# vmware/splinterdb

Hardware: AMD Instinct MI355X
Metric: routing_filter build Mkeys/s + probe Mkeys/s, device-resident, 24B keys (higher is better)
Workload: dtype u32; 1 GPU; C2: 64M x 24B keys per GPU = 8 filters x 8,000,000, build + full probe; filters_total=8, filters_per_gpu=8, keys_per_filter=8000000, key_len=24, fingerprint_size=26, log_index_size=8, seed=42, parallelism=key-range shards, 1 rank(s), no data-path collective

## Files before the change

### include/rf_amd_diag.h

```cpp
#ifndef RF_AMD_DIAG_H
#define RF_AMD_DIAG_H

#include "rf_amd.h"

#ifdef __cplusplus
extern "C" {
#endif

int rf_amd_debug_read_lines(rf_amd_batch *b, uint8_t *h_lines, uint64_t bytes, uint64_t *num_lines);
int rf_amd_debug_rebuild_lines(rf_amd_batch *b);

int rf_amd_debug_probe_floor(rf_amd_batch *b, const void *d_in, uint32_t key_len, const uint64_t *h_counts,
                             uint64_t *d_out, void *stream);

int rf_amd_debug_phase_buffer(void *d_buf, uint32_t kernel);

int rf_amd_diag_lookup_stats(uint64_t *out, int reset);

int rf_amd_diag_lookup_paths(uint64_t *out, int reset);

int rf_amd_lookup_server_stats(rf_amd_engine *e, uint64_t *out);

int rf_amd_diag_lookup_ring(rf_amd_engine *e);

int rf_amd_diag_lookup_server_kill(rf_amd_engine *e, int err, uint32_t gap_us);

uint64_t rf_amd_diag_k4_bitmap_builds(void);

uint64_t rf_amd_diag_part16_builds(void);

int rf_amd_diag_fanout_max_blocks(uint32_t blocks);

uint32_t rf_amd_diag_range_tile(void);
uint32_t rf_amd_diag_range_lds_ranges(void);

const char *rf_amd_build_id(void);

#ifdef __cplusplus
}
#endif
#endif
```

### splinterdb_amd/csrc/rf_batch_plan.h

```cpp
#pragma once
#include <math.h>
#include <string.h>

#include <algorithm>
#include <string>
#include <vector>

#include "../../include/rf_amd.h"
#include "rf_plan.h"

namespace rf {

inline uint64_t max_fingerprints(const rf_amd_config& cfg) {
  const uint64_t addrs_per_extent = (uint64_t)cfg.page_size * cfg.pages_per_extent / 8;
  return 2ull * addrs_per_extent * (1ull << cfg.log_index_size) - 1;
}

inline uint32_t vsize_of(uint32_t value) { return value == 0 ? 0 : 32 - __builtin_clz(value); }

inline uint32_t log_buckets_of(uint64_t nfp, uint32_t lis) {
  const uint32_t lnb = 63 - __builtin_clzll(nfp);
  return lnb < lis ? lis : lnb;
}
inline uint32_t num_indices_of(uint64_t nfp, uint32_t lis) { return 1u << (log_buckets_of(nfp, lis) - lis); }

inline uint32_t line_log_group(uint32_t lis, uint32_t rvs, double lam, double sigma) {
  if (rvs > 32) return 0;
  for (int g = (int)(lis < 6 ? lis : 6); g >= 0; g--) {
    const double G = (double)(1u << g), mean = lam * G;
    const double cap = rvs ? std::min(128.0 - G, 384.0 / rvs) : 128.0 - G;
    if (mean + sigma * sqrt(mean) + 2.0 <= cap) return (uint32_t)g + 1;
  }
  return 0;
}

inline int lines_in_assembly(uint32_t lis, uint32_t lg_line, uint32_t page_size) {
  const uint32_t IS = 1u << lis, L = IS >> (lg_line - 1);
  const uint32_t min_block = 2 + (IS - 1) / 8 + 4 + 3;
  const uint32_t maxb = page_size / min_block + 1;
  if (maxb > ASM_MAXB || L + 1 > ASM_GT) return 0;
  return (uint64_t)maxb * (L + 1) <= ASM_GT ? 1 : 2;
}

struct PlanKnobs {
  bool wide64 = false;
  bool old_decode = false;
  bool old_resplit_off = false;
  uint32_t layout_seg = LAYOUT_SEG_MAX;
  double line_sigma = 3.5;
};

struct OldFilter {
  bool present = false;
  const FilterPlan* plan = nullptr;
  uint32_t fingerprint_size = 0, log_index_size = 0;
  bool has_entries = false;
  bool wide = false;
  bool built = false;
  bool same_device = false;
};

struct BatchInput {
  const rf_amd_config* cfg = nullptr;
  uint32_t num_filters = 0;
  const uint32_t* num_new = nullptr;
  const uint16_t* value = nullptr;
  const uint32_t* num_runs = nullptr;
  const uint32_t* run_len = nullptr;
  const uint16_t* run_value = nullptr;
  const OldFilter* olds = nullptr;
};

enum { PRE_TILE, PRE_OTILE, PRE_CB, PRE_PG, PRE_IDX, PRE_OIDX, NUM_PRE };

struct BatchPlan {
  uint32_t F = 0;
  std::vector<FilterPlan> plans;
  std::vector<uint32_t> pre;
  uint32_t* pre_of(int k) { return pre.data() + (size_t)k * (F + 1); }
  const uint32_t* pre_of(int k) const { return pre.data() + (size_t)k * (F + 1); }
  bool wide = false;
  bool flag32 = false;
  bool chained = false;
  uint64_t old_total = 0;
  uint32_t num_tiles = 0, num_old_tiles = 0, num_old_idx = 0;
  uint64_t E = 0, keys_total = 0;
  uint32_t CB = 0, I = 0, PS = 0, PF = 0;
  uint64_t NL = 0;
  bool plines_needed = false;
  uint32_t line_lmax = 0;
  uint32_t lay_seg = 0, lay_grid = 0;
  bool lay_whole = true;
  std::vector<uint32_t> lay_wg;
  bool k4_bitmap = false;
  std::vector<uint32_t> tile_filter, tile_start, tile_value, tile_end;
  std::vector<uint4> pplans;
};

inline int plan_fail(std::string* err, int rc, const std::string& msg) {
  if (err) *err = msg;
  return rc;
}

inline int check_config(const rf_amd_config* cfg, std::string* err) {
  if (!cfg) return plan_fail(err, RF_AMD_EINVAL, "null config");
  if (cfg->page_size != MAX_PAGE || cfg->pages_per_extent != 32)
    return plan_fail(err, RF_AMD_EINVAL, "engine supports 4 KiB pages in 32-page extents");
  if (cfg->fingerprint_size == 0 || cfg->fingerprint_size > 32 || cfg->log_index_size > MAX_LIS ||
      cfg->log_index_size < 3)
    return plan_fail(err, RF_AMD_EINVAL, "unsupported fingerprint_size / log_index_size");
  return 0;
}

inline void probe_geometry(FilterPlan& p, const rf_amd_config& cfg, double sigma, uint64_t* line_total,
                           uint32_t* line_lmax) {
  const uint32_t lis = cfg.log_index_size;
  p.rem = cfg.fingerprint_size - p.lnb;
  p.rvs = p.rem + p.vs;
  p.lg_line = line_log_group(lis, p.rvs, (double)p.num_fp / (double)(1ull << p.lnb), sigma);
  p.line_base = (uint32_t)*line_total;
  if (p.lg_line) {
    *line_total += (uint64_t)p.num_indices << (lis - (p.lg_line - 1));
    *line_lmax = std::max(*line_lmax, (1u << lis) >> (p.lg_line - 1));
  }
}

inline uint32_t pplan_word(const FilterPlan& p) { return p.vs | (p.rem << 8) | (p.rvs << 16) | (p.lg_line << 24); }
inline uint4 pack_pplan(const FilterPlan& p) { return make_uint4(pplan_word(p), p.line_base, p.idx_base, 0); }

inline int check_runs(const BatchInput& in, std::vector<uint32_t>* run_first, std::vector<uint32_t>* run_total,
                      std::string* err) {
  const rf_amd_config& cfg = *in.cfg;
  run_first->assign(in.num_filters + 1, 0u);
  run_total->assign(in.num_filters, 0u);
  for (uint32_t f = 0; f < in.num_filters; f++) {
    if (in.num_runs[f] == 0) return plan_fail(err, RF_AMD_EINVAL, "a filter without runs");
    const uint32_t r0 = (*run_first)[f], r1 = r0 + in.num_runs[f];
    (*run_first)[f + 1] = r1;
    uint64_t tot = 0;
    for (uint32_t r = r0; r < r1; r++) {
      if (in.run_len[r] == 0) return plan_fail(err, RF_AMD_EINVAL, "zero-length run");
      if (r > r0 && in.run_value[r] <= in.run_value[r - 1])
        return plan_fail(err, RF_AMD_EINVAL, "run values of a filter must be strictly increasing");
      tot += in.run_len[r];
    }
    if (tot > max_fingerprints(cfg))
      return plan_fail(err, RF_AMD_EINVAL, "num_fingerprints over routing_filter_max_fingerprints (reference: UB)");
    if (cfg.fingerprint_size + vsize_of(in.run_value[r1 - 1]) > 32)
      return plan_fail(err, RF_AMD_EINVAL, "fp_size + value_size > 32");
    const OldFilter* o = in.olds && in.olds[f].present ? &in.olds[f] : nullptr;
    if (o && o->plan && vsize_of(in.run_value[r0]) < o->plan->vs)
      return plan_fail(err, RF_AMD_EINVAL, "first run's value narrower than the old filter's value_size");
    (*run_total)[f] = (uint32_t)tot;
  }
  return 0;
}

inline int filter_geometry(const rf_amd_config& cfg, uint32_t num_new, uint32_t v, const FilterPlan* op,
                           FilterPlan* out, std::string* err) {
  FilterPlan& p = *out;
  const uint32_t lis = cfg.log_index_size, fps = cfg.fingerprint_size, IS = 1u << lis;
  p.num_new = num_new;
  p.old_region = op ? op->num_fp : 0;
  const uint64_t nfp = (uint64_t)p.num_new + p.old_region;
  if (nfp > max_fingerprints(cfg))
    return plan_fail(err, RF_AMD_EINVAL, "num_fingerprints over routing_filter_max_fingerprints (reference: UB)");
  p.num_fp = (uint32_t)nfp;
  if (p.num_fp == 0) return plan_fail(err, RF_AMD_EINVAL, "routing_filter_add with zero fingerprints (reference: UB)");
  const uint32_t lnb = log_buckets_of(nfp, lis);
  p.vs = vsize_of(v);
  if (lnb > fps || (1u << (lnb - lis)) > MAX_INDICES || fps + p.vs > 32 || (op && p.vs < op->vs))
    return plan_fail(err, RF_AMD_EINVAL, "filter geometry out of range (over routing_filter_max_fingerprints, "
                                         "fp_size + value_size > 32, or value narrower than old filter)");
  p.lnb = lnb;
  p.value = v;
  p.num_indices = 1u << (lnb - lis);
// ... 94 lines not shown
      first = end;
    }
  }
}

inline int plan_batch(const BatchInput& in0, const PlanKnobs& knobs, BatchPlan* out, std::string* err) {
  BatchInput in = in0;
  if (in.num_runs && in.run_len && in.run_value) {
    bool single = true;
    for (uint32_t f = 0; f < in.num_filters && single; f++) single = in.num_runs[f] == 1;
    if (single) {
      for (uint32_t f = 0; f < in.num_filters; f++)
        if (in.run_len[f] == 0) return plan_fail(err, RF_AMD_EINVAL, "zero-length run");
      in.num_new = in.run_len;
      in.value = in.run_value;
      in.num_runs = nullptr;
    }
  }
  if (int rc = check_config(in.cfg, err)) return rc;
  if (in.num_filters == 0 || !(in.num_runs ? (in.run_len && in.run_value) : in.num_new != nullptr))
    return plan_fail(err, RF_AMD_EINVAL, "empty batch");
  const rf_amd_config& cfg = *in.cfg;
  const uint32_t F = in.num_filters;
  std::vector<uint32_t> run_first, run_total;
  if (in.num_runs) {
    if (int rc = check_runs(in, &run_first, &run_total, err)) return rc;
    in.num_new = run_total.data();
  }
  BatchPlan& b = *out;
  b = BatchPlan();
  b.F = F;
  b.chained = in.num_runs != nullptr;
  b.plans.resize(F);
  b.pre.assign((size_t)NUM_PRE * (F + 1), 0u);
  const uint32_t lis = cfg.log_index_size;
  for (uint32_t f = 0; f < F; f++) {
    FilterPlan& p = b.plans[f];
    memset(&p, 0, sizeof(p));
    const FilterPlan* op = nullptr;
    if (in.olds && in.olds[f].present) {
      const OldFilter& o = in.olds[f];
      if (!o.plan || !o.built || !o.same_device) return plan_fail(err, RF_AMD_EINVAL, "bad old filter reference");
      op = o.plan;
      b.wide = true;
    }
    const uint32_t v = b.chained ? in.run_value[run_first[f + 1] - 1] : in.value ? in.value[f] : 0;
    if (int rc = filter_geometry(cfg, in.num_new[f], v, op, &p, err)) return rc;
    p.e_first = b.E;
    p.key_first = b.keys_total;
    p.cb_base = b.CB;
    p.idx_base = b.I;
    p.page_base = b.PS;
    p.pf_base = b.PF;
    probe_geometry(p, cfg, knobs.line_sigma, &b.NL, &b.line_lmax);
    const int la = p.lg_line ? lines_in_assembly(lis, p.lg_line, cfg.page_size) : 0;
    p.lines_asm = la != 0;
    p.lines_flag = la == 2;
    if (p.lg_line && la != 1) b.plines_needed = true;
    uint32_t ntiles = (p.num_new + TILE_KEYS - 1) / TILE_KEYS;
    if (b.chained) {
      const uint64_t prev_fp = (uint64_t)p.num_fp - in.run_len[run_first[f + 1] - 1];
      p.npo = prev_fp ? p.num_indices / num_indices_of(prev_fp, lis) : 1u;
      ntiles = 0;
      for (uint32_t r = run_first[f]; r < run_first[f + 1]; r++) ntiles += (in.run_len[r] + TILE_KEYS - 1) / TILE_KEYS;
    }
    auto pre = [&](int k, uint32_t count) { b.pre_of(k)[f + 1] = b.pre_of(k)[f] + count; };
    pre(PRE_TILE, ntiles);
    pre(PRE_OTILE, (p.old_region + TILE_KEYS - 1) / TILE_KEYS);
    pre(PRE_CB, 1u << p.cbits);
    pre(PRE_PG, p.page_cap);
    pre(PRE_IDX, p.num_indices);
    b.E += p.num_fp;
    b.keys_total += p.num_new;
    b.CB += 1u << p.cbits;
    b.I += p.num_indices;
    b.PS += p.page_cap;
    b.PF += p.page_cap + 1;
  }
  if (b.wide) {
    b.flag32 = !knobs.wide64;
    for (const auto& p : b.plans) b.flag32 = b.flag32 && cfg.fingerprint_size + p.vs <= 31;
  }
  if (!b.wide || b.flag32) {
    b.E = 0;
    for (auto& p : b.plans) {
      p.e_first = b.E;
      b.E += (uint64_t)CB_REGION << p.cbits;
    }
  }
  if (b.wide) plan_old_filters(b, in, knobs);
  b.lay_seg = knobs.layout_seg;
  if (cfg.page_size > MAX_PAGE || F >= (1u << 26)) b.lay_seg = 0;
  assign_layout(b);
  b.k4_bitmap = k4_bitmap_batch(b, cfg);
  b.num_tiles = b.pre_of(PRE_TILE)[F];
  b.num_old_tiles = b.pre_of(PRE_OTILE)[F];
  if (b.NL > 0xffffffffull) return plan_fail(err, RF_AMD_EINVAL, "batch too large (probe lines > 2^32)");
  b.pplans.resize(F);
  for (uint32_t f = 0; f < F; f++) b.pplans[f] = pack_pplan(b.plans[f]);
  if (b.chained) cut_tiles(b, in, run_first);
  return 0;
}

inline int plan_import(const rf_amd_config* cfgp, uint32_t F, const rf_amd_filter_info* infos,
                       const PlanKnobs& knobs, BatchPlan* out, std::string* err) {
  if (int rc = check_config(cfgp, err)) return rc;
  if (F == 0 || !infos) return plan_fail(err, RF_AMD_EINVAL, "bad image");
  const rf_amd_config& cfg = *cfgp;
  const uint32_t lis = cfg.log_index_size;
  BatchPlan& b = *out;
  b = BatchPlan();
  b.F = F;
  b.plans.resize(F);
  b.pplans.resize(F);
  uint64_t pages_total = 0, idx_total = 0;
  for (uint32_t f = 0; f < F; f++) {
    const rf_amd_filter_info& in = infos[f];
    FilterPlan& p = b.plans[f];
    memset(&p, 0, sizeof(p));
    const uint32_t lnb = in.num_fingerprints ? log_buckets_of(in.num_fingerprints, lis) : lis;
    if (in.num_fingerprints == 0 || lnb > cfg.fingerprint_size || (1u << (lnb - lis)) > MAX_INDICES ||
        in.num_indices != (1u << (lnb - lis)) || in.value_size > 32 - cfg.fingerprint_size || in.error ||
        in.num_pages == 0)
      return plan_fail(err, RF_AMD_EINVAL, "image geometry out of range (filter " + std::to_string(f) + ")");
    p.num_fp = in.num_fingerprints;
    p.lnb = lnb;
    p.vs = in.value_size;
    p.num_indices = in.num_indices;
    p.page_cap = in.num_pages;
    p.page_base = (uint32_t)pages_total;
    p.idx_base = (uint32_t)idx_total;
    probe_geometry(p, cfg, knobs.line_sigma, &b.NL, &b.line_lmax);
    if (p.lg_line) b.plines_needed = true;
    b.pplans[f] = pack_pplan(p);
    pages_total += in.num_pages;
    idx_total += p.num_indices;
  }
  if (b.NL >= (1ull << 32) || pages_total >= (1ull << 32)) return plan_fail(err, RF_AMD_EINVAL, "import too large");
  b.PS = (uint32_t)pages_total;
  b.I = (uint32_t)idx_total;
  return 0;
}

}
```

### splinterdb_amd/csrc/rf_engine.cpp

```cpp
#include <hip/hip_runtime.h>
#include <hip/hip_ext.h>
#include <math.h>
#include <algorithm>
#include <stdio.h>
#include <stdlib.h>
#include <string.h>
#include <time.h>
#include <x86intrin.h>

#include <map>
#include <atomic>
#include <memory>
#include <mutex>
#include <string>
#include <vector>

#include "../../include/rf_amd.h"
#include "../../include/rf_amd_diag.h"
#include "rf_plan.h"
#include "rf_batch_plan.h"
#include "rf_set_plan.h"
#include "rf_launch.h"

using namespace rf;
// ... 223 lines not shown
}

#define RF_BATCH_DEVBUFS(X)                                                                        \
  X(d_runs) X(d_wave_tab)      \
  X(d_plans) X(d_outs) X(d_ent) X(d_part) X(d_sorted) X(d_cb_count) X(d_cb_start) X(d_cb_cursor)   \
  X(d_cb_filter) X(d_overflow) X(d_idx_cnt) X(d_idx_start) X(d_slots) X(d_page_first)              \
  X(d_pg_filter) X(d_pages) X(d_tile_filter) X(d_tile_start) X(d_old_tile_filter)                  \
  X(d_old_tile_start) X(d_old_cnt) X(d_old_pos) X(d_first_old) X(d_has_old) X(d_pplans) X(d_lines) \
  X(d_idx_filter) X(d_spill) X(d_old_idx_filter) X(d_old32) X(d_old_tot) X(d_ob_lo) X(d_ob_n)      \
  X(d_pg_noline) X(d_pre) X(d_cb_out) X(d_lay_wg) X(d_lay_hand)                                    \
  X(d_tile_value) X(d_tile_end)

struct rf_amd_batch : BatchPlan {
  rf_amd_engine* eng = nullptr;
  rf_amd_config cfg{};
#define X(name) DevBuf name;
  RF_BATCH_DEVBUFS(X)
#undef X
  std::vector<uint64_t> runs_host;
  uint32_t lay_seq = 0;
  bool counters_clean = false;
  bool built = false;
  bool has_entries = false;
  std::vector<uint32_t> err_host;
  std::atomic<bool> err_ready{false};
  std::mutex err_mu;
  hipEvent_t built_ev = nullptr;
  std::vector<hipEvent_t> events;
  uint32_t ev_sets = 0, ev_set = 0;
  uint32_t ev_mask = EV_MASK_ALL;
  ~rf_amd_batch() {
    if (built_ev) (void)hipEventDestroy(built_ev);
    for (auto ev : events) (void)hipEventDestroy(ev);
  }
  std::vector<DevBuf*> bufs() {
    return {
#define X(name) &name,
        RF_BATCH_DEVBUFS(X)
#undef X
    };
  }
};

static PlanKnobs plan_knobs_env() {
  PlanKnobs k;
  k.wide64 = getenv("RF_AMD_WIDE64") != nullptr;
  k.old_decode = getenv("RF_AMD_OLD_DECODE") != nullptr;
  k.old_resplit_off = getenv("RF_AMD_OLD_RESPLIT_OFF") != nullptr;
  if (const char* e = getenv("RF_AMD_LAYOUT_SEG"); e && *e) {
    const unsigned long v = strtoul(e, nullptr, 10);
    k.layout_seg = (v < LAYOUT_SEG_MIN || (v & (v - 1))) ? 0 : v > LAYOUT_SEG_MAX ? LAYOUT_SEG_MAX : (uint32_t)v;
  }
  if (const char* e = getenv("RF_AMD_LINE_SIGMA"); e && atof(e) > 0.0) k.line_sigma = atof(e);
  return k;
}

extern "C" const char* rf_amd_last_error(void) { return g_err.c_str(); }

static std::mutex g_live_mu;
static std::vector<rf_amd_engine*>* g_live = nullptr;
static bool engine_quiesce(rf_amd_engine* e, int budget_ms);
static void engine_destroy_now(rf_amd_engine* e, bool device_sync);
static void engines_at_exit() {
  std::vector<rf_amd_engine*> v;
  {
    std::lock_guard<std::mutex> g(g_live_mu);
    if (g_live) v.swap(*g_live);
  }
  for (rf_amd_engine* e : v) {
    if (engine_quiesce(e, 2000)) engine_destroy_now(e, false);
  }
}

extern "C" int rf_amd_engine_create(int device, rf_amd_engine** out) {
  int n = 0;
  if (hipGetDeviceCount(&n) != hipSuccess || n == 0)
    return fail(RF_AMD_ENODEV, "no HIP device: the routing-filter engine has no CPU fallback");
  if (device < 0 || device >= n) return fail(RF_AMD_EINVAL, "bad device ordinal");
  HIPCHK(hipSetDevice(device));
  auto* e = new rf_amd_engine();
  static std::atomic<uint64_t> next_uid{1};
  e->uid = next_uid.fetch_add(1);
  e->device = device;
  {
    const char* lim = getenv("RF_AMD_POOL_MIB");
    size_t free_b = 0, total_b = 0;
    (void)hipMemGetInfo(&free_b, &total_b);
    const size_t dflt = free_b / 4;
    e->pool.limit = lim ? (size_t)atoll(lim) << 20 : dflt;
  }
  if (hipStreamCreateWithFlags(&e->stream, hipStreamDefault) != hipSuccess) {
    delete e;
    return fail(RF_AMD_EINVAL, "hipStreamCreate failed");
  }
  {
    static std::once_flag at_exit_once;
    std::call_once(at_exit_once, [] { (void)atexit(engines_at_exit); });
    std::lock_guard<std::mutex> g(g_live_mu);
    if (!g_live) g_live = new std::vector<rf_amd_engine*>();
    g_live->push_back(e);
  }
  *out = e;
  return 0;
}

static void srv_stop(rf_amd_engine* e);
extern "C" void rf_amd_engine_destroy(rf_amd_engine* e) {
  if (!e) return;
  {
    std::lock_guard<std::mutex> g(g_live_mu);
// ... 439 lines not shown
  return rf_amd_engine_pool_trim(e, bytes);
}

extern "C" uint32_t rf_amd_batch_num_filters(const rf_amd_batch* b) { return b ? b->F : 0; }

static LaunchArgs make_args(rf_amd_batch* b, hipStream_t st) {
  LaunchArgs a;
  memset(&a, 0, sizeof(a));
  a.stream = st;
  a.wide = b->wide;
  a.plans = b->d_plans.as<FilterPlan>();
  a.pplans = b->d_pplans.as<uint4>();
  a.pplans_mut = b->d_pplans.as<uint4>();
  a.num_filters = b->F;
  a.tile_filter = b->d_tile_filter.as<uint32_t>();
  a.tile_start = b->d_tile_start.as<uint32_t>();
  a.num_tiles = b->num_tiles;
  a.tile_value = b->chained ? b->d_tile_value.as<uint32_t>() : nullptr;
  a.tile_end = b->chained ? b->d_tile_end.as<uint32_t>() : nullptr;
  a.old_tile_filter = b->d_old_tile_filter.as<uint32_t>();
  a.old_tile_start = b->d_old_tile_start.as<uint32_t>();
  a.num_old_tiles = b->num_old_tiles;
  a.old_idx_filter = b->d_old_idx_filter.as<uint32_t>();
  a.num_old_idx = b->num_old_idx;
  a.old_cnt = b->d_old_cnt.as<uint32_t>();
  a.old_pos = b->d_old_pos.as<uint32_t>();
  a.flag32 = b->flag32 ? 1u : 0u;
  a.old32 = b->d_old32.as<uint32_t>();
  a.old_tot = b->d_old_tot.as<uint32_t>();
  a.ob_lo = b->d_ob_lo.as<uint32_t>();
  a.ob_n = b->d_ob_n.as<uint32_t>();
  a.fp_size = b->cfg.fingerprint_size;
  a.seed = b->cfg.seed;
  a.lis = b->cfg.log_index_size;
  a.page_size = b->cfg.page_size;
  a.ent = b->d_ent.p;
  a.part = b->d_part.p;
  a.sorted32 = b->wide ? b->d_sorted.as<uint32_t>() : b->d_part.as<uint32_t>();
  a.cb_count = b->d_cb_count.as<uint32_t>();
  a.cb_start = b->d_cb_start.as<uint32_t>();
  a.cb_cursor = b->d_cb_cursor.as<uint32_t>();
  a.cb_filter = b->d_cb_filter.as<uint32_t>();
  a.num_cb = b->CB;
  a.overflow = b->d_overflow.as<uint32_t>();
  a.spill = b->d_spill.p ? b->d_spill.as<uint32_t>() : nullptr;
  a.cb_outs = b->d_cb_out.p ? b->d_cb_out.as<uint32_t>() : nullptr;
  a.idx_cnt = b->d_idx_cnt.as<uint32_t>();
  a.idx_start = b->d_idx_start.as<uint32_t>();
  a.first_old = b->d_first_old.as<uint32_t>();
  a.has_old = b->d_has_old.as<uint32_t>();
  a.slots = b->d_slots.as<uint64_t>();
  a.lines = b->d_lines.as<uint4>();
  a.line_lmax = b->line_lmax;
  a.plines_needed = b->plines_needed ? 1u : 0u;
  a.pg_noline = b->d_pg_noline.as<uint32_t>();
  a.idx_filter = b->d_idx_filter.as<uint32_t>();
  a.num_idx = b->I;
  a.page_first = b->d_page_first.as<uint32_t>();
  a.pg_filter = b->d_pg_filter.as<uint32_t>();
  a.num_page_slots = b->PS;
  a.pages = b->d_pages.as<uint8_t>();
  a.outs = b->d_outs.p ? b->d_outs.as<FilterOut>() : nullptr;
  a.lay_wg = b->d_lay_wg.as<uint32_t>();
  a.lay_grid = b->d_lay_wg.p && b->d_lay_hand.p ? b->lay_grid : 0;
  a.lay_hand = b->d_lay_hand.as<uint64_t>();
  a.lay_seq = b->lay_seq;
  a.lay_seg = b->lay_seg;
  a.lay_whole = b->lay_whole ? 1u : 0u;
  a.k4_bitmap = b->k4_bitmap ? 1u : 0u;
  a.events = b->events.empty() ? nullptr : reinterpret_cast<void**>(b->events.data() + (size_t)b->ev_set * NUM_EVENTS);
  a.ev_mask = b->ev_mask;
  return a;
}

static int do_probe(rf_amd_batch* b, int kind, const void* in0, const uint64_t* offs, uint32_t key_len,
                    const uint32_t* fid, uint64_t n, uint64_t* found, void* stream,
                    const uint64_t* d_runs = nullptr);

static int note_built(rf_amd_batch* b, hipStream_t st) {
  if (!b->built_ev) HIPCHK(hipEventCreateWithFlags(&b->built_ev, hipEventDisableTiming));
  HIPCHK(hipEventRecord(b->built_ev, st));
  return 0;
}
static int wait_built(rf_amd_batch* b) {
  if (b->built_ev) HIPCHK(hipEventSynchronize(b->built_ev));
  return 0;
}

static int do_build(rf_amd_batch* b, int kind, const void* in0, const uint64_t* offs, uint32_t key_len,
                    void* stream) {
  if (!b) return fail(RF_AMD_EINVAL, "null batch");
  if (b->keys_total && !in0) return fail(RF_AMD_EINVAL, "null input");
  HIPCHK(hipSetDevice(b->eng->device));
  hipStream_t st = stream_of(b->eng, stream);
  (void)hipGetLastError();
  if (b->ev_sets) b->ev_set = (b->ev_set + 1) % b->ev_sets;
  if (++b->lay_seq == 0) b->lay_seq = 1;
  LaunchArgs a = make_args(b, st);
  a.kind = kind;
  a.in0 = in0;
  a.offs = offs;
  a.key_len = key_len;
  if (a.events && (a.ev_mask >> EV_B_START & 1u)) HIPCHK(hipEventRecord(((hipEvent_t*)a.events)[EV_B_START], st));
  const char* sc = getenv("RF_AMD_SELF_CLEAN");
  a.self_clean = (!b->wide && !b->plines_needed && b->num_tiles && !(sc && sc[0] == '0') &&
                  !getenv("RF_AMD_DIAG_OVERFLOW")) ? 1u : 0u;
  a.zero_outs = (a.self_clean && b->counters_clean) ? 1u : 0u;
  b->counters_clean = false;
  if (!a.zero_outs &&
      rf_launch_build_init(st, b->d_cb_count.as<uint32_t>(), (b->wide && !b->flag32) ? nullptr : b->d_cb_cursor.as<uint32_t>(),
                           b->CB, b->d_outs.as<uint32_t>(), (uint32_t)(sizeof(FilterOut) / 4 * b->F),
                           b->d_overflow.as<uint32_t>(), (b->wide && !b->flag32) ? nullptr : b->d_spill.as<uint32_t>(),
                           b->d_pg_noline.as<uint32_t>()))
    return fail(RF_AMD_EINVAL, "init kernel launch failed");
  if (b->wide) {
    if (int rc = launch_rc("old decode", rf_launch_old_decode(&a))) return rc;
  }
  b->err_ready.store(false, std::memory_order_release);
  int rc = rf_launch_build(&a);
  if (st == b->eng->stream) b->eng->builds_issued.fetch_add(1, std::memory_order_acq_rel);
  if (rc) return launch_rc("build", rc);
  b->counters_clean = a.self_clean != 0;
  if (getenv("RF_AMD_DIAG_OVERFLOW") && b->d_overflow.p) {
    uint32_t nov = 0;
    if (hipMemcpyAsync(&nov, b->d_overflow.p, 4, hipMemcpyDeviceToHost, st) == hipSuccess &&
        hipStreamSynchronize(st) == hipSuccess)
      fprintf(stderr, "rf_amd: %u of %u coarse buckets handed back (K4b / list mode)\n", nov, b->CB);
  }
  if (int erc = note_built(b, st)) return erc;
  b->built = true;
  b->has_entries = true;
  return 0;
}

extern "C" int rf_amd_batch_build_keys(rf_amd_batch* b, const void* d_keys, uint32_t key_len, void* stream) {
  if (key_len == 0) return fail(RF_AMD_EINVAL, "key_len 0");
  return do_build(b, fixed_kind(d_keys, key_len), d_keys, nullptr, key_len, stream);
}
extern "C" int rf_amd_batch_build_var_keys(rf_amd_batch* b, const uint8_t* d_bytes, const uint64_t* d_offsets,
                                           void* stream) {
  if (!d_offsets) return fail(RF_AMD_EINVAL, "null offsets");
  return do_build(b, IN_VAR, d_bytes, d_offsets, 0, stream);
}
extern "C" int rf_amd_batch_build_hashes(rf_amd_batch* b, const uint32_t* d_hashes, void* stream) {
  return do_build(b, IN_HASH, d_hashes, nullptr, 4, stream);
}

static int stage_reserve(rf_amd_engine* e, size_t bytes) {
  HostStage& s = e->stage;
  if (s.cap >= bytes) return 0;
  if (s.h) (void)hipHostFree(s.h);
  if (s.d) (void)hipFree(s.d);
  s.h = s.d = nullptr;
  s.cap = 0;
  const size_t c = std::max<size_t>(bytes, (size_t)1 << 20);
  if (hipHostMalloc(&s.h, c, hipHostMallocDefault) != hipSuccess) {
    s.h = nullptr;
    return fail(RF_AMD_ENOMEM, "pinned staging allocation failed");
  }
  if (hipMalloc(&s.d, c) != hipSuccess) {
    (void)hipHostFree(s.h);
    s.h = nullptr;
    return fail(RF_AMD_ENOMEM, "device staging allocation failed");
  }
  s.cap = c;
  return 0;
}

extern "C" int rf_amd_batch_stage_begin(rf_amd_batch* b, uint32_t** h_stage) {
  if (!b || !h_stage) return fail(RF_AMD_EINVAL, "null batch / out-param");
  rf_amd_engine* e = b->eng;
// ... 570 lines not shown
  int z = 0;
  e->srv.dead.compare_exchange_strong(z, err);
  return 0;
}

extern "C" int rf_amd_lookup_server_error(rf_amd_engine* e) { return e ? e->srv.dead.load() : RF_AMD_ENODEV; }

extern "C" int rf_amd_lookup_server_set_times(rf_amd_engine* e, uint64_t idle_us, uint64_t life_us) {
  if (!e || !idle_us || !life_us) return fail(RF_AMD_EINVAL, "bad server times");
  e->srv.idle_ticks = idle_us * 100;
  e->srv.life_ticks = life_us * 100;
  return 0;
}

extern "C" int rf_amd_diag_lookup_ring(rf_amd_engine* e) {
  if (!e || !e->srv.ready.load(std::memory_order_acquire)) return -1;
  return e->srv.ring_dev ? 1 : 0;
}

extern "C" int rf_amd_lookup_server_stats(rf_amd_engine* e, uint64_t* out) {
  if (!e || !out) return fail(RF_AMD_EINVAL, "null argument");
  out[0] = e->srv.tail.load();
  out[1] = e->srv.launches.load();
  out[2] = e->srv.ctl ? __atomic_load_n(&e->srv.ctl->exit_head, __ATOMIC_ACQUIRE) : 0;
  return 0;
}

static std::atomic<uint64_t> g_lk_calls{0}, g_lk_prep_ns{0}, g_lk_launch_ns{0}, g_lk_wait_ns{0};
static std::atomic<uint64_t> g_lk_small{0}, g_lk_mapped{0}, g_lk_copy{0}, g_lk_sync{0};
static inline uint64_t mono_ns() {
  timespec ts;
  clock_gettime(CLOCK_MONOTONIC, &ts);
  return (uint64_t)ts.tv_sec * 1000000000ull + (uint64_t)ts.tv_nsec;
}
struct LookupClock {
  uint64_t t0 = mono_ns(), t1 = 0, t2 = 0;
  void launching() { t1 = mono_ns(); }
  void launched() { t2 = mono_ns(); }
  ~LookupClock() {
    if (!t2) return;
    const uint64_t t3 = mono_ns();
    g_lk_calls.fetch_add(1, std::memory_order_relaxed);
    g_lk_prep_ns.fetch_add(t1 - t0, std::memory_order_relaxed);
    g_lk_launch_ns.fetch_add(t2 - t1, std::memory_order_relaxed);
    g_lk_wait_ns.fetch_add(t3 - t2, std::memory_order_relaxed);
  }
};
#ifndef RF_AMD_SRC_ID
#define RF_AMD_SRC_ID "unknown"
#endif
extern "C" const char* rf_amd_build_id(void) { return RF_AMD_SRC_ID; }

extern "C" uint64_t rf_amd_diag_k4_bitmap_builds(void) { return rf_k4_bitmap_builds(); }
extern "C" uint64_t rf_amd_diag_part16_builds(void) { return rf_part16_builds(); }

extern "C" int rf_amd_diag_lookup_stats(uint64_t* out, int reset) {
  if (!out) return fail(RF_AMD_EINVAL, "null output");
  std::atomic<uint64_t>* c[4] = {&g_lk_calls, &g_lk_prep_ns, &g_lk_launch_ns, &g_lk_wait_ns};
  for (int k = 0; k < 4; k++) out[k] = reset ? c[k]->exchange(0) : c[k]->load();
  return 0;
}

extern "C" int rf_amd_diag_lookup_paths(uint64_t* out, int reset) {
  if (!out) return fail(RF_AMD_EINVAL, "null output");
  std::atomic<uint64_t>* c[4] = {&g_lk_small, &g_lk_mapped, &g_lk_copy, &g_lk_sync};
  for (int k = 0; k < 4; k++) out[k] = reset ? c[k]->exchange(0) : c[k]->load();
  return 0;
}

static int probe_groups_host(rf_amd_engine* e, const std::vector<ProbeGroup>& groups,
                             const uint32_t* h_hashes, const uint32_t* h_group, uint64_t n, uint64_t* h_found) {
  if (n == 0) return 0;
  LookupClock clk;
  static const int mode = env_mode("RF_AMD_PROBE_MODE", "mapped", "copy");
  static const int wait = env_mode("RF_AMD_PROBE_WAIT", "flag", "sync");
  static const bool small_ok = !getenv("RF_AMD_PROBE_SMALL") || atoi(getenv("RF_AMD_PROBE_SMALL")) != 0;
  const uint32_t ng = (uint32_t)groups.size();
  const size_t o_g = (8 * n + 15) & ~15ull, o_f = (o_g + sizeof(ProbeGroup) * ng + 63) & ~63ull;
  const bool small = small_ok && wait != 2 && n <= SMALL_PROBES && ng <= SMALL_GROUPS;
  const bool mapped = mode == 1 || (mode == 0 && n <= MAPPED_MAX_PROBES);
  (small ? g_lk_small : mapped ? g_lk_mapped : g_lk_copy).fetch_add(1, std::memory_order_relaxed);
  if (!small && wait == 2) g_lk_sync.fetch_add(1, std::memory_order_relaxed);
  ProbeSlot* s = slot_take(e);
  if (!s) return RF_AMD_ENOMEM;
  struct Give {
    rf_amd_engine* e;
    ProbeSlot* s;
    ~Give() { slot_give(e, s); }
  } give{e, s};
  if (int rc = slot_reserve(s, small ? 8 * n : o_f + 8 * n, (small || mapped) ? 0 : o_f)) return rc;
  const uint64_t issued = e->builds_issued.load(std::memory_order_acquire);
  if (issued != e->builds_seen_idle.load(std::memory_order_acquire)) {
    if (hipStreamQuery(e->stream) == hipErrorNotReady) {
      hipEvent_t ev;
      HIPCHK(hipEventCreateWithFlags(&ev, hipEventDisableTiming));
      HIPCHK(hipEventRecord(ev, e->stream));
      HIPCHK(hipStreamWaitEvent(s->st, ev, 0));
      (void)hipEventDestroy(ev);
    } else {
      e->builds_seen_idle.store(issued, std::memory_order_release);
    }
  }
  const uint32_t seq = ++s->seq ? s->seq : ++s->seq;
  (void)hipGetLastError();
  if (small) {
    SmallProbe sp;
// ... 627 lines not shown
  if (h_pages) {
    if (pages_bytes < need) return fail(RF_AMD_EINVAL, "pages buffer too small");
    HIPCHK(hipMemcpyAsync(h_pages, b->d_pages.as<uint8_t>() + (uint64_t)p.page_base * b->cfg.page_size, need,
                          hipMemcpyDeviceToHost, st));
  }
  if (h_slots) {
    if (num_slots < p.num_indices) return fail(RF_AMD_EINVAL, "slots buffer too small");
    HIPCHK(hipMemcpyAsync(h_slots, b->d_slots.as<uint64_t>() + p.idx_base, 8ull * p.num_indices,
                          hipMemcpyDeviceToHost, st));
  }
  HIPCHK(hipStreamSynchronize(st));
  return 0;
}

extern "C" int rf_amd_batch_read_image_async(rf_amd_batch* b, uint32_t f, void* h_pages, uint64_t pages_bytes,
                                             void* h_slots, uint32_t num_slots, void* stream) {
  if (!b || f >= b->F) return fail(RF_AMD_EINVAL, "bad batch/filter");
  const FilterPlan& p = b->plans[f];
  if (pages_bytes > (uint64_t)p.page_cap * b->cfg.page_size || num_slots > p.num_indices)
    return fail(RF_AMD_EINVAL, "copy larger than the filter's reservation");
  HIPCHK(hipSetDevice(b->eng->device));
  hipStream_t st = stream_of(b->eng, stream);
  if (h_pages && pages_bytes)
    HIPCHK(hipMemcpyAsync(h_pages, b->d_pages.as<uint8_t>() + (uint64_t)p.page_base * b->cfg.page_size,
                          pages_bytes, hipMemcpyDeviceToHost, st));
  if (h_slots && num_slots)
    HIPCHK(hipMemcpyAsync(h_slots, b->d_slots.as<uint64_t>() + p.idx_base, 8ull * num_slots,
                          hipMemcpyDeviceToHost, st));
  return 0;
}

extern "C" int rf_amd_batch_image_ptrs(rf_amd_batch* b, uint32_t f, void** d_pages, void** d_slots) {
  if (!b || f >= b->F) return fail(RF_AMD_EINVAL, "bad batch/filter");
  const FilterPlan& p = b->plans[f];
  if (d_pages) *d_pages = b->d_pages.as<uint8_t>() + (uint64_t)p.page_base * b->cfg.page_size;
  if (d_slots) *d_slots = b->d_slots.as<uint64_t>() + p.idx_base;
  return 0;
}

static int import_enqueue(rf_amd_batch* b, const std::vector<FilterOut>& outs, const std::vector<uint32_t>& idx_filter,
                          const void* pages, const uint64_t* slots, hipMemcpyKind kind) {
  const uint32_t F = b->F;
  const size_t page_bytes = (size_t)b->PS * b->cfg.page_size;
  hipStream_t st = b->eng->stream;
  HIPCHK(hipMemcpyAsync(b->d_outs.p, outs.data(), sizeof(FilterOut) * F, hipMemcpyHostToDevice, st));
  HIPCHK(hipMemsetAsync(b->d_pages.as<uint8_t>() + page_bytes, 0, 256, st));
  HIPCHK(hipMemcpyAsync(b->d_pages.p, pages, page_bytes, kind, st));
  HIPCHK(hipMemcpyAsync(b->d_slots.p, slots, 8ull * b->I, kind, st));
  HIPCHK(hipMemcpyAsync(b->d_idx_filter.p, idx_filter.data(), 4ull * b->I, hipMemcpyHostToDevice, st));
  HIPCHK(hipMemcpyAsync(b->d_plans.p, b->plans.data(), sizeof(FilterPlan) * F, hipMemcpyHostToDevice, st));
  HIPCHK(hipMemcpyAsync(b->d_pplans.p, b->pplans.data(), 16ull * F, hipMemcpyHostToDevice, st));
  {
    LaunchArgs a = make_args(b, st);
    if (int lrc = launch_rc("probe-line", rf_launch_plines(&a))) return lrc;
  }
  HIPCHK(hipStreamSynchronize(st));
  return note_built(b, st);
}

static int batch_import(rf_amd_engine* e, const rf_amd_config* cfg, uint32_t F, const rf_amd_filter_info* infos,
                        const void* pages, const uint64_t* slots, hipMemcpyKind kind, rf_amd_batch** out) {
  if (int rc = check_cfg(cfg)) return rc;
  if (F == 0 || !infos || !pages || !slots) return fail(RF_AMD_EINVAL, "bad image");
  auto b = std::make_unique<rf_amd_batch>();
  std::string msg;
  if (int rc = plan_import(cfg, F, infos, plan_knobs_env(), b.get(), &msg)) return fail(rc, msg);
  b->eng = e;
  b->cfg = *cfg;

  HIPCHK(hipSetDevice(e->device));
  DevPool* pool = &e->pool;
  int rc = b->d_plans.alloc(sizeof(FilterPlan) * F, pool);
  rc |= b->d_pplans.alloc(16ull * F, pool);
  rc |= b->d_pages.alloc((size_t)b->PS * cfg->page_size + 256, pool);
  rc |= b->d_slots.alloc(8ull * b->I, pool);
  rc |= b->d_lines.alloc(64ull * b->NL + 64, pool);
  rc |= b->d_idx_filter.alloc(4ull * b->I, pool);
  rc |= b->d_outs.alloc(sizeof(FilterOut) * F, pool);
  if (rc) return fail(RF_AMD_ENOMEM, "device allocation failed");

  std::vector<FilterOut> outs(F);
  std::vector<uint32_t> idx_filter;
  idx_filter.reserve(b->I);
  for (uint32_t f = 0; f < F; f++) {
    outs[f] = FilterOut{infos[f].num_unique, infos[f].num_pages, 0u, 0u};
    idx_filter.insert(idx_filter.end(), b->plans[f].num_indices, f);
  }
  if (int erc = import_enqueue(b.get(), outs, idx_filter, pages, slots, kind)) {
    (void)hipStreamSynchronize(e->stream);
    return erc;
  }
  b->err_host.assign(F, 0u);
  b->err_ready.store(true, std::memory_order_release);
  b->built = true;
  *out = b.release();
  return 0;
}

static int batch_from_image(rf_amd_engine* e, const rf_amd_config* cfg, const rf_amd_image* img,
                            rf_amd_batch** out) {
  if (!img || !img->pages || !img->slots || img->info.num_fingerprints == 0)
    return fail(RF_AMD_EINVAL, "bad image");
  return batch_import(e, cfg, 1, &img->info, img->pages, img->slots, hipMemcpyHostToDevice, out);
}

extern "C" int rf_amd_batch_export(rf_amd_batch* b, void* d_pages, uint64_t pages_bytes, uint64_t* d_slots,
// ... 611 lines not shown
```

### splinterdb_amd/csrc/rf_kernels.hip

```cpp
#include <hip/hip_runtime.h>
#include <stdint.h>

#include <atomic>

#include "rf_device.h"
#include "rf_plan.h"
#include "rf_launch.h"

using namespace rf;

typedef unsigned int v4u __attribute__((ext_vector_type(4)));
typedef unsigned int v2u __attribute__((ext_vector_type(2)));

template <int KIND, bool NT = false>
__device__ __forceinline__ uint32_t hash_key(const void* __restrict__ in0, const uint64_t* __restrict__ offs,
                                             uint32_t key_len, uint32_t seed, uint64_t k) {
  if constexpr (KIND == IN_KEYS24) {
    const v2u* kp = reinterpret_cast<const v2u*>(static_cast<const uint8_t*>(in0) + k * 24);
    v2u a, b, c;
    if constexpr (NT) {
      a = __builtin_nontemporal_load(kp);
      b = __builtin_nontemporal_load(kp + 1);
      c = __builtin_nontemporal_load(kp + 2);
    } else {
// ... 2052 lines not shown
  const uint64_t v = (uint64_t)(nbits >= 32 ? val : (val & ((1u << nbits) - 1))) << sh;
  if ((uint32_t)v) atomicOr(&s[w], (uint32_t)v);
  if ((uint32_t)(v >> 32)) atomicOr(&s[w + 1], (uint32_t)(v >> 32));
}

__device__ __forceinline__ void assemble_atomic(const FilterPlan& P, uint32_t p, uint32_t slot, uint32_t b0,
                                                uint32_t b1, const uint32_t* __restrict__ idx_cnt,
                                                const uint32_t* __restrict__ idx_start,
                                                const uint32_t* __restrict__ sorted32,
                                                const uint64_t* __restrict__ slots, uint8_t* __restrict__ pages,
                                                uint32_t lis, uint32_t page_size, uint32_t* s_pg) {
  const uint32_t nwords = page_size / 4;
  for (uint32_t i = threadIdx.x; i < nwords + 4; i += ASM_NT) s_pg[i] = 0;
  const uint32_t index_size = 1u << lis;
  __syncthreads();
  for (uint32_t b = b0; b < b1; b++) {
    const uint32_t g = P.idx_base + b;
    const uint32_t off = (uint32_t)(slots[g] - (uint64_t)p * page_size);
    const uint32_t c = idx_cnt[g];
    const uint32_t enc = (c + index_size - 1) / 8 + 4;
    if (threadIdx.x == 0) lds_or_bits(s_pg, (uint64_t)off * 8, c & 0xffffu, 16);
    const uint32_t e0 = off + 2, e1 = off + 2 + enc;
    for (uint32_t w = (e0 >> 2) + threadIdx.x; w <= ((e1 - 1) >> 2); w += ASM_NT) {
      const uint32_t lo = max(e0, w * 4), hi = min(e1, w * 4 + 4);
      const uint32_t m = (hi - lo == 4) ? 0xffffffffu : (((1u << ((hi - lo) * 8)) - 1) << ((lo & 3) * 8));
      atomicOr(&s_pg[w], m);
    }
  }
  __syncthreads();
  const uint32_t remmask = P.rem >= 32 ? 0xffffffffu : ((1u << P.rem) - 1);
  for (uint32_t b = b0; b < b1; b++) {
    const uint32_t g = P.idx_base + b;
    const uint32_t off = (uint32_t)(slots[g] - (uint64_t)p * page_size);
    const uint32_t c = idx_cnt[g];
    const uint32_t enc = (c + index_size - 1) / 8 + 4;
    const uint32_t* ent = sorted32 + P.e_first + idx_start[g];
    const uint64_t ebit = (uint64_t)(off + 2) * 8;
    const uint64_t rbit = (uint64_t)(off + 2 + enc) * 8;
    for (uint32_t k = threadIdx.x; k < c; k += ASM_NT) {
      const uint32_t e = ent[k];
      const uint32_t fp = e >> P.vs;
      const uint32_t bucket_off = (P.rem >= 32 ? 0u : (fp >> P.rem)) & (index_size - 1);
      const uint64_t hb = ebit + k + bucket_off;
      atomicAnd(&s_pg[hb >> 5], ~(1u << (hb & 31)));
      const uint32_t rv = ((fp & remmask) << P.vs) | (e & ((1u << P.vs) - 1));
      lds_or_bits(s_pg, rbit + (uint64_t)k * P.rvs, rv, P.rvs);
    }
  }
}

constexpr uint32_t ASM_RUN = 16;
constexpr uint32_t ASM_MAXE = 16384;

__device__ __forceinline__ uint64_t lds_bits64(const uint32_t* s_pg, uint32_t bitpos) {
  const uint32_t w = bitpos >> 5, sh = bitpos & 31;
  const uint64_t lo = ((uint64_t)s_pg[w + 1] << 32) | s_pg[w];
  return (lo >> sh) | (sh ? (uint64_t)s_pg[w + 2] << (64 - sh) : 0ull);
}

__global__ __launch_bounds__(ASM_NT) __attribute__((amdgpu_waves_per_eu(8))) void k_assemble(const FilterPlan* __restrict__ plans,
                                                     const uint32_t* __restrict__ pg_filter,
                                                     const uint32_t* __restrict__ idx_cnt,
                                                     const uint32_t* __restrict__ idx_start,
                                                     const uint32_t* __restrict__ sorted32,
                                                     const uint64_t* __restrict__ slots,
                                                     const uint32_t* __restrict__ page_first,
                                                     const FilterOut* __restrict__ outs,
                                                     uint8_t* __restrict__ pages, uint4* __restrict__ lines,
                                                     uint32_t* __restrict__ pg_noline,
                                                     uint32_t lis, uint32_t page_size) {
  __shared__ __attribute__((aligned(16))) uint32_t s_pg[MAX_PAGE / 4 + 4];
  __shared__ uint32_t s_wpre[ASM_MAXB];
  __shared__ uint32_t s_off[ASM_MAXB + 1];
  __shared__ uint32_t s_c[ASM_MAXB];
  __shared__ uint32_t s_est[ASM_MAXB + 1];
  __shared__ uint32_t s_src[ASM_MAXB];
  __shared__ uint8_t s_rblk[ASM_MAXE / ASM_RUN + ASM_MAXB];
  __shared__ __attribute__((aligned(16))) uint32_t s_wmgs[MAX_PAGE / 16 > ASM_GT / 2 ? MAX_PAGE / 16 : ASM_GT / 2];
  uint32_t* const s_wm = s_wmgs;
  uint16_t* const s_gs = reinterpret_cast<uint16_t*>(s_wmgs);
  __shared__ uint32_t s_tmp[ASM_NT / WAVE + 1];
  DBG_PHASE_K(3, 15);
  const uint32_t slot = xcd_chunk(blockIdx.x, gridDim.x);
  const uint32_t f = pg_filter[slot];
  const FilterPlan& P = plans[f];
  const uint32_t p = slot - P.page_base;
  if (outs[f].error || p >= outs[f].num_pages) return;
  if (!P.lines_asm && P.lg_line && threadIdx.x == 0) pg_noline[1 + atomicAdd(&pg_noline[0], 1u)] = slot;
  const uint32_t* pf = page_first + P.pf_base;
  const uint32_t b0 = pf[p], b1 = pf[p + 1], nb = b1 - b0;
  uint4* dst = reinterpret_cast<uint4*>(pages + (uint64_t)slot * page_size);
  if (nb > ASM_MAXB) {
    assemble_atomic(P, p, slot, b0, b1, idx_cnt, idx_start, sorted32, slots, pages, lis, page_size, s_pg);
    __syncthreads();
    for (uint32_t i = threadIdx.x; i < page_size / 16; i += ASM_NT) dst[i] = reinterpret_cast<const uint4*>(s_pg)[i];
    return;
  }
  const uint32_t IS = 1u << lis, rvs = P.rvs;
  const uint32_t lgG = P.lines_asm ? P.lg_line - 1 : 0u, G = 1u << lgG, L = IS >> lgG;
  const bool cut = P.lines_asm && !(P.lines_flag && nb * (L + 1) > ASM_GT);
  uint32_t cj[2], oj[2], sj[2], sum = 0;
  uint64_t sl[2];
#pragma unroll
  for (int q = 0; q < 2; q++) {
    const uint32_t g = P.idx_base + b0 + min(threadIdx.x * 2 + q, nb - 1);
    cj[q] = idx_cnt[g];
    sl[q] = slots[g];
    sj[q] = idx_start[g];
  }
  for (uint32_t i = threadIdx.x; i < MAX_PAGE / 16; i += ASM_NT) s_wm[i] = 0;
#pragma unroll
  for (int q = 0; q < 2; q++) {
    const uint32_t j = threadIdx.x * 2 + q;
    oj[q] = 0;
    if (j < nb) {
      oj[q] = (uint32_t)(sl[q] - (uint64_t)p * page_size);
      s_off[j] = oj[q];
      s_c[j] = cj[q];
      s_src[j] = sj[q];
    } else {
      cj[q] = 0;
    }
    sum += cj[q];
  }
  uint32_t tot;
  uint32_t run = block_excl_scan<ASM_NT>(sum + (((cj[0] + ASM_RUN - 1) / ASM_RUN + (cj[1] + ASM_RUN - 1) / ASM_RUN) << 20),
                                         s_tmp, &tot);
  const uint32_t ne = tot & 0xfffffu, nruns = tot >> 20;
#pragma unroll
  for (int q = 0; q < 2; q++) {
    const uint32_t j = threadIdx.x * 2 + q;
    if (j < nb) s_est[j] = run >> 20;
    run += cj[q] + (((cj[q] + ASM_RUN - 1) / ASM_RUN) << 20);
  }
  if (threadIdx.x == 0) { s_est[nb] = nruns; s_off[nb] = page_size; }
  DBG_PHASE_K(3, 0);
  if (ne > ASM_MAXE) {
    __syncthreads();
    assemble_atomic(P, p, slot, b0, b1, idx_cnt, idx_start, sorted32, slots, pages, lis, page_size, s_pg);
  } else {
  __syncthreads();
#pragma unroll
  for (int q = 0; q < 2; q++) {
    const uint32_t j = threadIdx.x * 2 + q;
    if (j < nb) {
      for (uint32_t r = s_est[j]; r < s_est[j + 1]; r++) s_rblk[r] = (uint8_t)j;
    }
    if (j < nb && j > 0) reinterpret_cast<uint8_t*>(s_wm)[(oj[q] + 3) / 4] = 1;
  }
  __syncthreads();
  const uint32_t nwp = page_size / 4;
  constexpr uint32_t QPT = (MAX_PAGE / 16 + ASM_NT - 1) / ASM_NT;
// ... 24 lines not shown
#pragma unroll
      for (uint32_t i = 0; i < ASM_RUN; i++) ev[i] = src[min(i, last)];
    }
  };
  uint32_t ev0[ASM_RUN], pv0 = 0;
  if (threadIdx.x < nruns) load_run(threadIdx.x, ev0, pv0);
  uint32_t jw = jw0;
#pragma unroll
  for (uint32_t q = 0; q < QPT; q++) {
  const uint32_t qd = threadIdx.x * QPT + q;
  const uint32_t mw = mwq[q];
  if (4 * qd < nwp) {
    const uint32_t ja = jw + (mw & 0xffu);
    jw += (mw & 0xffu) + ((mw >> 8) & 0xffu) + ((mw >> 16) & 0xffu) + (mw >> 24);
    const uint32_t jb = min(ja + 1, nb - 1), jc = min(ja + 2, nb - 1);
    const uint32_t o0 = s_off[ja], c0 = s_c[ja];
    const uint32_t o1 = ja + 1 < nb ? s_off[jb] : 0xffffffffu, c1 = s_c[jb];
    const uint32_t o2 = ja + 2 < nb ? s_off[jc] : 0xffffffffu, c2 = s_c[jc];
    const uint32_t n0 = o0 + 2 + (c0 + IS - 1) / 8 + 4;
    const uint32_t n1 = o1 + 2 + (c1 + IS - 1) / 8 + 4;
    const uint32_t n2 = o2 + 2 + (c2 + IS - 1) / 8 + 4;
    uint32_t x4[4];
#pragma unroll
    for (int k = 0; k < 4; k++) {
      uint32_t x = 0;
#pragma unroll
      for (int i = 0; i < 4; i++) {
        const uint32_t B = 16 * qd + 4 * k + i;
        const bool s2 = B >= o2, s1 = B >= o1;
        const uint32_t o = s2 ? o2 : (s1 ? o1 : o0), c = s2 ? c2 : (s1 ? c1 : c0);
        const uint32_t en = s2 ? n2 : (s1 ? n1 : n0);
        const uint32_t rel = B - o;
        const uint32_t byte = rel < 2 ? ((c >> (8 * rel)) & 0xffu) : (B < en ? 0xffu : 0u);
        x |= byte << (8 * i);
      }
      x4[k] = x;
    }
    reinterpret_cast<v4u*>(s_pg)[qd] = v4u{x4[0], x4[1], x4[2], x4[3]};
  }
  }
  if (threadIdx.x < 4) s_pg[page_size / 4 + threadIdx.x] = 0;
  __syncthreads();
  DBG_PHASE_K(3, 1);
  const uint32_t rmask = rvs >= 32 ? 0xffffffffu : ((1u << rvs) - 1);
  const uint32_t bsh = rvs >= 32 ? 0u : rvs, bmask = rvs >= 32 ? 0u : IS - 1;
  for (uint32_t r = threadIdx.x; r < nruns; r += ASM_NT) {
    const uint32_t j = s_rblk[r], k0 = (r - s_est[j]) * ASM_RUN, c = s_c[j];
    const uint32_t len = min((uint32_t)ASM_RUN, c - k0);
    uint32_t (&ev)[ASM_RUN] = ev0;
    uint32_t& pv = pv0;
    if (r != threadIdx.x) load_run(r, ev, pv);
    if (cut) {
      const uint32_t gb = j * (L + 1);
      const uint32_t gp = k0 ? ((pv >> bsh) & bmask) >> lgG : 0u;
      uint32_t last = ev[0];
#pragma unroll
      for (uint32_t i = 1; i < ASM_RUN; i++) last = i < len ? ev[i] : last;
      const uint32_t gl = ((last >> bsh) & bmask) >> lgG;
      const uint32_t hi = bsh + lis >= 32 ? 0u : ev[0] & ~((IS << bsh) - 1u);
#pragma unroll 1
      for (uint32_t g = gp + 1; g <= gl; g++) {
        const uint32_t lim = hi | ((g * G) << bsh);
        uint32_t before = 0;
#pragma unroll
        for (uint32_t i = 0; i < ASM_RUN; i++) before += (i < len && ev[i] < lim) ? 1u : 0u;
        s_gs[gb + g] = (uint16_t)(g * G + k0 + before);
      }
      if (k0 + len == c)
#pragma unroll 1
        for (uint32_t g = gl + 1; g < L; g++) s_gs[gb + g] = (uint16_t)(g * G + c);
    }
    const uint32_t eb0 = (s_off[j] + 2) * 8 + k0;
    const uint32_t rb0 = (s_off[j] + 2 + (c + IS - 1) / 8 + 4) * 8 + k0 * rvs;
    uint32_t wb = (eb0 + ((ev[0] >> bsh) & bmask)) & ~31u;
    uint64_t m = 0;
#pragma unroll
    for (uint32_t i = 0; i < ASM_RUN; i++) {
      const uint32_t hb = eb0 + i + ((ev[i] >> bsh) & bmask);
      const bool live = i < len;
      if (live && hb - wb >= 64) {
        if ((uint32_t)m) atomicAnd(&s_pg[wb >> 5], ~(uint32_t)m);
        if ((uint32_t)(m >> 32)) atomicAnd(&s_pg[(wb >> 5) + 1], ~(uint32_t)(m >> 32));
        m = 0;
        wb = hb & ~31u;
      }
      m |= (uint64_t)(live ? 1u : 0u) << ((hb - wb) & 63);
    }
    if ((uint32_t)m) atomicAnd(&s_pg[wb >> 5], ~(uint32_t)m);
    if ((uint32_t)(m >> 32)) atomicAnd(&s_pg[(wb >> 5) + 1], ~(uint32_t)(m >> 32));
    if (rvs >= 32) {
#pragma unroll
      for (uint32_t i = 0; i < ASM_RUN; i++)
        if (i < len) lds_or_bits(s_pg, rb0 + i * rvs, ev[i], rvs);
    } else if (rvs) {
      const uint32_t per = 32u / rvs;
      uint32_t w = rb0 >> 5, nbit = rb0 & 31, since = 0;
      uint64_t acc = 0;
#pragma unroll
      for (uint32_t i = 0; i < ASM_RUN; i++) {
        const bool live = i < len;
        acc |= (uint64_t)(live ? ev[i] & rmask : 0u) << nbit;
        nbit += live ? rvs : 0u;
        if (++since == per) {
          since = 0;
          if (nbit >= 32) {
            atomicOr(&s_pg[w], (uint32_t)acc);
            acc >>= 32;
            nbit -= 32;
            w++;
          }
        }
// ... 28 lines not shown
        s_gs[j * (L + 1) + L] = (uint16_t)(c + IS);
        if (c == 0)
          for (uint32_t g = 1; g < L; g++) s_gs[j * (L + 1) + g] = (uint16_t)(g * G);
      }
    }
    __syncthreads();
  } else {
  uint32_t wc[2], wsum = 0;
#pragma unroll
  for (int q = 0; q < 2; q++) {
    const uint32_t j = threadIdx.x * 2 + q;
    wc[q] = j < nb ? (s_c[j] + IS + 63) / 64 : 0u;
    wsum += wc[q];
  }
  uint32_t nw;
  uint32_t wrun = block_excl_scan<ASM_NT>(wsum, s_tmp, &nw);
#pragma unroll
  for (int q = 0; q < 2; q++) {
    const uint32_t j = threadIdx.x * 2 + q;
    if (j < nb) {
      s_est[j] = wrun;
      s_gs[j * (L + 1)] = 0;
      s_gs[j * (L + 1) + L] = (uint16_t)(s_c[j] + IS);
    }
    wrun += wc[q];
  }
  if (threadIdx.x == 0) s_est[nb] = nw;
  __syncthreads();
  uint32_t carry = 0;
  for (uint32_t base = 0; base < nw; base += ASM_NT) {
    const uint32_t it = base + threadIdx.x;
    uint32_t j = 0, w = 0, ones = 0;
    uint64_t x = 0;
    if (it < nw) {
      uint32_t lo = 0, hi = nb;
      while (hi - lo > 1) {
        const uint32_t mid = (lo + hi) >> 1;
        if (s_est[mid] <= it) lo = mid; else hi = mid;
      }
      j = lo;
      w = it - s_est[j];
      const uint32_t nbits = s_c[j] + IS, b = w * 64;
      x = lds_bits64(s_pg, (s_off[j] + 2) * 8 + b);
      if (nbits - b < 64) x &= (1ull << (nbits - b)) - 1;
      ones = __popcll(x);
    }
    uint32_t tot;
    const uint32_t ex_all = block_excl_scan<ASM_NT>(ones, s_tmp, &tot) + carry;
    carry += tot;
    if (it < nw && w == 0) s_wpre[j] = ex_all;
    __syncthreads();
    if (it < nw) {
      const uint32_t ex = ex_all - s_wpre[j];
      for (uint32_t k = (ex + G) >> lgG; k < L && k * G - 1 < ex + ones; k++)
        s_gs[j * (L + 1) + k] = (uint16_t)(w * 64 + select64_fast(x, k * G - 1 - ex) + 1);
    }
    __syncthreads();
  }
  }
  DBG_PHASE_K(3, 4);
  const uint32_t nt = nb * L * 4;
  for (uint32_t u = threadIdx.x; u < nt; u += ASM_NT) {
    const uint32_t j = u >> (lis - lgG + 2), rest = u & (4 * L - 1), gl = rest >> 2, qq = rest & 3;
    const uint32_t c = s_c[j];
    const uint32_t ebit = (s_off[j] + 2) * 8, rbit = (s_off[j] + 2 + (c + IS - 1) / 8 + 4) * 8;
    const uint32_t a = s_gs[j * (L + 1) + gl], ne2 = s_gs[j * (L + 1) + gl + 1] - a;
    const uint32_t n = ne2 - G, E = a - gl * G;
    const bool ovf = ne2 > 128 || n * rvs > 384;
    uint64_t wv[2];
#pragma unroll
    for (int h = 0; h < 2; h++) {
      const uint32_t o = qq * 128 + h * 64;
      uint64_t x = 0;
      if (ovf) {
        x = o < 128 ? ~0ull : 0ull;
      } else if (o < 128) {
        const uint32_t hi = min(o + 64, ne2);
        if (o < hi) x = lds_bits64(s_pg, ebit + a + o) & lowmask64(hi - o);
      } else {
        const uint32_t ro = o - 128, hi = min(ro + 64, n * rvs);
        if (ro < hi) x = lds_bits64(s_pg, rbit + E * rvs + ro) & lowmask64(hi - ro);
      }
      wv[h] = x;
    }
    const uint64_t line = (uint64_t)P.line_base + (uint64_t)(b0 + j) * L + gl;
    lines[line * 4 + qq] = make_uint4((uint32_t)wv[0], (uint32_t)(wv[0] >> 32), (uint32_t)wv[1], (uint32_t)(wv[1] >> 32));
  }
  DBG_PHASE_K(3, 8);
}

__global__ void k_old_counts(const FilterPlan* __restrict__ plans, const uint32_t* __restrict__ old_idx_filter,
                             uint32_t num_old_idx, uint32_t* __restrict__ cnt) {
  const uint32_t g = blockIdx.x * blockDim.x + threadIdx.x;
  if (g >= num_old_idx) return;
  const FilterPlan& P = plans[old_idx_filter[g]];
  if (old_error(P)) {
    cnt[g] = 0;
    return;
  }
  const uint64_t s = P.old_slots[g - P.old_idx_base];
  cnt[g] = (uint32_t)P.old_pages[s] | ((uint32_t)P.old_pages[s + 1] << 8);
}

__global__ __launch_bounds__(LAYOUT_NT) void k_old_scan(const FilterPlan* __restrict__ plans,
                                                        const uint32_t* __restrict__ cnt,
                                                        uint32_t* __restrict__ pos, uint64_t* __restrict__ ent,
                                                        uint32_t* __restrict__ old_tot) {
  __shared__ uint32_t s_tmp[LAYOUT_NT / WAVE + 1];
  const FilterPlan& P = plans[blockIdx.x];
  const uint32_t n = P.old_direct ? 0u : P.old_num_indices;
  if (n == 0) return;
  constexpr int PER = MAX_INDICES / LAYOUT_NT;
  uint32_t v[PER], sum = 0;
#pragma unroll
  for (int k = 0; k < PER; k++) {
    const uint32_t i = threadIdx.x * PER + k;
    v[k] = i < n ? cnt[P.old_idx_base + i] : 0u;
    sum += v[k];
  }
  uint32_t total;
  uint32_t run = block_excl_scan<LAYOUT_NT>(sum, s_tmp, &total);
#pragma unroll
  for (int k = 0; k < PER; k++) {
    const uint32_t i = threadIdx.x * PER + k;
    if (i < n) pos[P.old_idx_base + i] = run;
    run += v[k];
  }
  if (old_tot && threadIdx.x == 0) old_tot[blockIdx.x] = total;
  if (!ent) return;
  uint64_t* tail = ent + P.e_first + P.num_new;
  for (uint32_t j = total + threadIdx.x; j < P.old_region; j += LAYOUT_NT) tail[j] = ~0ull;
}

__global__ __launch_bounds__(256) void k_old_decode(const FilterPlan* __restrict__ plans,
                                                    const uint32_t* __restrict__ old_idx_filter,
                                                    uint32_t num_old_idx, const uint32_t* __restrict__ pos,
                                                    uint64_t* __restrict__ ent, uint32_t* __restrict__ old32,
// ... 432 lines not shown
__device__ __forceinline__ uint64_t probe_stream(uint32_t bo, uint32_t remainder, uint32_t vs, uint32_t rvs,
                                                 const uint8_t* pg, uint64_t hdr, uint32_t lis) {
  const uint32_t index_size = 1u << lis;
  const uint32_t c = (uint32_t)pg[hdr] | ((uint32_t)pg[hdr + 1] << 8);
  const uint32_t enc = (c + index_size - 1) / 8 + 4;
  const uint64_t a0 = (hdr + 2) & ~15ull;
  const uint32_t e0 = (uint32_t)((hdr + 2 - a0) * 8);
  const uint32_t target_lo = bo ? bo - 1 : 0;
  uint32_t start = 0, end = 0, cum = 0;
  bool have_start = (bo == 0);
  const uint32_t nwin = (e0 + c + index_size + 127) / 128 + 1;
  for (uint32_t k = 0;; k++) {
    if (k > nwin) return 0;
    uint64_t lo, hi;
    ld_win(pg, a0 + 16ull * k, lo, hi);
    if (k == 0 && e0) {
      if (e0 >= 64) { lo = 0; hi = (hi >> (e0 - 64)) << (e0 - 64); }
      else { lo = (lo >> e0) << e0; }
    }
    const uint32_t pc = __popcll(lo) + __popcll(hi);
    const uint32_t base = 128u * k - e0;
    if (!have_start && cum + pc > target_lo) {
      start = base + select128(lo, hi, target_lo - cum) + 1 - bo;
      have_start = true;
    }
    if (cum + pc > bo) {
      end = base + select128(lo, hi, bo - cum) - bo;
      break;
    }
    cum += pc;
  }
  if (start >= end) return 0;
  const uint64_t rbit0 = (hdr + 2 + enc) * 8;
  const uint32_t vmask = (uint32_t)((1ull << vs) - 1);
  uint64_t found = 0;
  for (uint32_t pos = start; pos < end; pos++) {
    const uint32_t rv = ld_bits(pg, rbit0 + (uint64_t)pos * rvs, rvs);
    if ((rv >> vs) == remainder) {
      const uint32_t v = rv & vmask;
      if (v < 64) found |= 1ull << v;
    }
  }
  return found;
}

__device__ __forceinline__ uint64_t bits64_at(const uint8_t* pg, uint64_t bitpos) {
  const uint64_t by = bitpos >> 3;
  const uint32_t sh = (uint32_t)(bitpos & 7);
  uint64_t x = ld_u64_unaligned(pg, by) >> sh;
  if (sh) x |= (uint64_t)pg[by + 8] << (64 - sh);
  return x;
}

__device__ __forceinline__ void plines_index(const FilterPlan& P, uint32_t g, const uint64_t* __restrict__ slots,
                                             const uint8_t* __restrict__ pages, uint4* __restrict__ lines,
                                             uint8_t* blk, uint32_t* s_a, uint32_t lane, uint32_t lis,
                                             uint32_t page_size) {
  constexpr uint32_t SLICE = MAX_PAGE + 64;
  const uint32_t IS = 1u << lis;
  const uint32_t lgG = P.lg_line - 1, G = 1u << lgG, L = IS >> lgG;
  const uint8_t* pg = blk;
  const uint8_t* gp = pages + (uint64_t)P.page_base * page_size;
  const uint64_t rel_g = slots[g];
  const uint32_t c = (uint32_t)gp[rel_g] | ((uint32_t)gp[rel_g + 1] << 8);
  const uint64_t a0 = rel_g & ~15ull;
  const uint32_t used = (uint32_t)(rel_g - a0) + 2 + (c + IS - 1) / 8 + 4 +
                        (uint32_t)(((uint64_t)c * P.rvs + 7) / 8) + 12;
  const uint32_t nq = min((used + 15) / 16, SLICE / 16);
  for (uint32_t q = lane; q < nq; q += WAVE)
    reinterpret_cast<v4u*>(blk)[q] = *reinterpret_cast<const v4u*>(gp + a0 + 16ull * q);
  __builtin_amdgcn_fence(__ATOMIC_RELEASE, "wavefront");
  __builtin_amdgcn_wave_barrier();
  __builtin_amdgcn_fence(__ATOMIC_ACQUIRE, "wavefront");
  const uint64_t rel = rel_g - a0;
  {
    const uint64_t ebit = (rel + 2) * 8;
    const uint32_t nbits = c + IS;
    if (lane == 0) { s_a[0] = 0; s_a[L] = nbits; }
    uint32_t ones_before = 0;
    for (uint32_t base = 0; base < nbits; base += 64 * WAVE) {
      const uint32_t b0 = base + lane * 64;
      uint64_t x = 0;
      if (b0 < nbits) {
        x = bits64_at(pg, ebit + b0);
        const uint32_t nb = min(64u, nbits - b0);
        x &= lowmask64(nb);
      }
      const uint32_t ones = __popcll(x);
      const uint32_t ex = wave_incl_scan(ones) - ones + ones_before;
      for (uint32_t k = (ex + G) >> lgG; k < L && k * G - 1 < ex + ones; k++)
        s_a[k] = b0 + select64_fast(x, k * G - 1 - ex) + 1;
      ones_before = __shfl(ex + ones, WAVE - 1, WAVE);
    }
  }
  __builtin_amdgcn_fence(__ATOMIC_RELEASE, "wavefront");
  __builtin_amdgcn_wave_barrier();
  __builtin_amdgcn_fence(__ATOMIC_ACQUIRE, "wavefront");
  const uint32_t rvs = P.rvs;
  const uint64_t ebit = (rel + 2) * 8;
  const uint32_t enc = (c + IS - 1) / 8 + 4;
  const uint64_t rbit0 = (rel + 2 + enc) * 8;
  const uint64_t line0 = (uint64_t)P.line_base + (uint64_t)(g - P.idx_base) * L;
  for (uint32_t u = lane; u < 4 * L; u += WAVE) {
    const uint32_t gl = u >> 2, qq = u & 3;
    const uint32_t a = s_a[gl], ne = s_a[gl + 1] - a;
    const uint32_t n = ne - G, E = a - gl * G;
    const bool ovf = ne > 128 || (uint64_t)n * rvs > 384;
    uint64_t w[2];
#pragma unroll
    for (int h = 0; h < 2; h++) {
      const uint32_t o = qq * 128 + h * 64;
      uint64_t x = 0;
      if (ovf) {
        x = o < 128 ? ~0ull : 0ull;
      } else if (o < 128) {
        const uint32_t hi = min(o + 64, ne);
        if (o < hi) x = bits64_at(pg, ebit + a + o) & lowmask64(hi - o);
      } else {
        const uint32_t ro = o - 128, hi = min(ro + 64, n * rvs);
        if (ro < hi) x = bits64_at(pg, rbit0 + (uint64_t)E * rvs + ro) & lowmask64(hi - ro);
      }
      w[h] = x;
    }
    lines[(line0 + gl) * 4 + qq] =
        make_uint4((uint32_t)w[0], (uint32_t)(w[0] >> 32), (uint32_t)w[1], (uint32_t)(w[1] >> 32));
  }
}


__global__ __launch_bounds__(256) void k_plines(const FilterPlan* __restrict__ plans,
                                                const uint32_t* __restrict__ idx_filter,
                                                const uint64_t* __restrict__ slots,
                                                const uint8_t* __restrict__ pages,
                                                const FilterOut* __restrict__ outs,
                                                uint4* __restrict__ lines, uint32_t num_idx,
                                                uint32_t lmax, uint32_t lis, uint32_t page_size,
                                                uint32_t force) {
  constexpr uint32_t SLICE = MAX_PAGE + 64;
  __shared__ __attribute__((aligned(16))) uint8_t s_blk[256 / WAVE][SLICE];
  extern __shared__ uint32_t s_dyn[];
  const uint32_t wv = threadIdx.x / WAVE, lane = threadIdx.x & (WAVE - 1);
  const uint32_t g = blockIdx.x * (blockDim.x / WAVE) + wv;
  if (g >= num_idx) return;
  const uint32_t f = idx_filter[g];
  const FilterPlan& P = plans[f];
  if (P.lg_line == 0 || (outs && outs[f].error) || g - P.idx_base >= P.num_indices) return;
  if (!force && P.lines_asm) return;
  plines_index(P, g, slots, pages, lines, s_blk[wv], s_dyn + wv * (lmax + 1), lane, lis, page_size);
}

__global__ __launch_bounds__(256) void k_plines_list(const FilterPlan* __restrict__ plans,
                                                     const uint32_t* __restrict__ pg_filter,
                                                     const uint32_t* __restrict__ page_first,
                                                     const uint64_t* __restrict__ slots,
                                                     const uint8_t* __restrict__ pages,
                                                     const uint32_t* __restrict__ plist,
                                                     uint4* __restrict__ lines, uint32_t lmax, uint32_t lis,
                                                     uint32_t page_size) {
  constexpr uint32_t SLICE = MAX_PAGE + 64;
  __shared__ __attribute__((aligned(16))) uint8_t s_blk[256 / WAVE][SLICE];
  extern __shared__ uint32_t s_dyn[];
  const uint32_t wv = threadIdx.x / WAVE, lane = threadIdx.x & (WAVE - 1);
  const uint32_t n = plist[0];
  for (uint32_t e = blockIdx.x; e < n; e += gridDim.x) {
    const uint32_t slot = plist[1 + e];
    const FilterPlan& P = plans[pg_filter[slot]];
    const uint32_t* pf = page_first + P.pf_base;
    const uint32_t p = slot - P.page_base, b1 = pf[p + 1];
    for (uint32_t b = pf[p] + wv; b < b1; b += 256 / WAVE)
      plines_index(P, P.idx_base + b, slots, pages, lines, s_blk[wv], s_dyn + wv * (lmax + 1), lane, lis,
                   page_size);
  }
}

__device__ __forceinline__ uint32_t select32(uint32_t x, uint32_t r) {
  uint32_t pos = 0;
#pragma unroll
  for (uint32_t w = 16; w >= 1; w >>= 1) {
    const uint32_t c = __popc(x & ((1u << w) - 1));
    const bool up = r >= c;
    r = up ? r - c : r;
    x = up ? x >> w : x;
    pos = up ? pos + w : pos;
  }
  return pos;
}

__device__ __forceinline__ uint64_t field_ones64(uint32_t rvs) {
  uint64_t L = 1;
  uint32_t w = rvs;
#pragma unroll
  for (int i = 0; i < 6; i++) {
    if (w < 64) {
      L |= L << w;
      w <<= 1;
    }
  }
  return L;
}

__device__ __forceinline__ bool line_bounds(const v4u& E, uint32_t j, uint32_t& p1, uint32_t& c) {
  const uint32_t d0 = E.x, d1 = E.y, d2 = E.z, d3 = E.w;
  if ((d0 & d1 & d2 & d3) == 0xffffffffu) return false;
  p1 = 0;
  if (j) {
    const uint32_t r = j - 1, c0 = __popc(d0), c1 = c0 + __popc(d1), c2 = c1 + __popc(d2);
    const uint32_t x = r >= c2 ? d3 : (r >= c1 ? d2 : (r >= c0 ? d1 : d0));
    const uint32_t base = r >= c2 ? 96u : (r >= c1 ? 64u : (r >= c0 ? 32u : 0u));
    const uint32_t rr = r - (r >= c2 ? c2 : (r >= c1 ? c1 : (r >= c0 ? c0 : 0u)));
    p1 = base + select32(x, rr) + 1;
  }
  const uint64_t e0 = (uint64_t)d1 << 32 | d0, e1 = (uint64_t)d3 << 32 | d2;
  const uint64_t y = p1 >= 128 ? 0ull
                     : (p1 >= 64 ? e1 >> (p1 - 64) : (e0 >> p1) | (p1 ? e1 << (64 - p1) : 0ull));
  if (y == 0) return false;
  c = (uint32_t)__builtin_ctzll(y);
  return true;
}

__device__ __forceinline__ uint64_t emit_matches(uint64_t Z, uint64_t W, uint32_t rvs, uint32_t vs) {
  if (vs == 0) return Z ? 1ull : 0ull;
  const uint32_t vmask = (1u << vs) - 1;
  uint64_t found = 0;
  while (Z) {
    const uint32_t p = (uint32_t)__builtin_ctzll(Z) + 1 - rvs;
    const uint32_t val = (uint32_t)(W >> p) & vmask;
    if (val < 64) found |= 1ull << val;
    Z &= Z - 1;
  }
  return found;
}

template <typename Win>
__device__ __forceinline__ bool line_decode_w(const v4u& E, Win win, uint32_t j, uint32_t remainder, uint32_t vs,
                                              uint32_t rvs, uint64_t& found) {
  uint32_t p1, c;
  if (!line_bounds(E, j, p1, c)) return false;
  const uint32_t s = p1 - j;
  found = 0;
  if (c == 0 || rvs == 0) {
    if (c && remainder == 0) found = 1;
    return true;
  }
  const uint32_t b = s * rvs, wi = b >> 5, off = b & 31;
  if (off + c * rvs > 96 || b + c * rvs > 384) return false;
  uint32_t w0, w1, w2;
  win(wi, w0, w1, w2);
  const uint64_t wl = (uint64_t)w1 << 32 | w0;
  const uint32_t vmask = (uint32_t)((1ull << vs) - 1);
  const uint32_t nb = c * rvs, rem = rvs - vs;
  if (nb <= 64 && rem > 0) {
    const uint64_t W = off ? (wl >> off) | ((uint64_t)w2 << (64 - off)) : wl;
    const uint64_t L = field_ones64(rvs);
    const uint64_t valid = nb == 64 ? ~0ull : (1ull << nb) - 1;
    const uint64_t M = ((L << rvs) - (L << vs)) & valid;
    const uint64_t H = (L << (rvs - 1)) & valid;
    const uint64_t MH = M & ~H;
    const uint64_t Y = (W ^ ((uint64_t)(remainder << vs) * L)) & M;
    const uint64_t Z = H & ~((((Y & MH) + MH) | Y) & H);
    found = emit_matches(Z, W, rvs, vs);
    return true;
  }
  const uint32_t rvmask = rvs >= 32 ? 0xffffffffu : ((1u << rvs) - 1);
  for (uint32_t k = 0; k < c; k++) {
    const uint32_t qb = off + k * rvs;
    const uint64_t v = qb < 64 ? ((wl >> qb) | (qb ? (uint64_t)w2 << (64 - qb) : 0ull)) : (uint64_t)(w2 >> (qb - 64));
    const uint32_t rv = (uint32_t)v & rvmask;
    if ((rv >> vs) == remainder) {
      const uint32_t val = rv & vmask;
      if (val < 64) found |= 1ull << val;
    }
  }
  return true;
}

__device__ __forceinline__ bool line_decode(const v4u (&Q)[4], uint32_t j, uint32_t remainder, uint32_t vs,
                                            uint32_t rvs, uint64_t& found) {
  auto win = [&](uint32_t wi, uint32_t& w0, uint32_t& w1, uint32_t& w2) {
    const uint32_t R[14] = {Q[1].x, Q[1].y, Q[1].z, Q[1].w, Q[2].x, Q[2].y, Q[2].z,
                            Q[2].w, Q[3].x, Q[3].y, Q[3].z, Q[3].w, 0u, 0u};
    const uint32_t g = wi >> 2, o = wi & 3;
    uint32_t W[6];
#pragma unroll
    for (int k = 0; k < 6; k++) W[k] = g == 0 ? R[k] : (g == 1 ? R[4 + k] : R[8 + k]);
    w0 = o == 0 ? W[0] : (o == 1 ? W[1] : (o == 2 ? W[2] : W[3]));
    w1 = o == 0 ? W[1] : (o == 1 ? W[2] : (o == 2 ? W[3] : W[4]));
    w2 = o == 0 ? W[2] : (o == 1 ? W[3] : (o == 2 ? W[4] : W[5]));
  };
  return line_decode_w(Q[0], win, j, remainder, vs, rvs, found);
}

#ifndef RF_PROBE_NT
#define RF_PROBE_NT 1024
#endif
constexpr int PROBE_NT = RF_PROBE_NT;
constexpr int PROBE_NT_VAR = 256;
__host__ __device__ constexpr int probe_nt(int kind) { return kind == IN_VAR ? PROBE_NT_VAR : PROBE_NT; }

__global__ __launch_bounds__(256) void k_wave_tab(const uint64_t* __restrict__ runs, uint32_t nf, uint64_t n,
                                                  uint32_t* __restrict__ tab) {
  const uint64_t w = (uint64_t)blockIdx.x * blockDim.x + threadIdx.x;
  const uint64_t i = w * WAVE;
  if (i >= n) return;
  uint32_t lo = 0, hi = nf;
  while (hi - lo > 1) {
    const uint32_t mid = (lo + hi) >> 1;
    if (runs[mid] <= i) lo = mid; else hi = mid;
  }
  const uint64_t left = runs[lo + 1] - i;
  tab[w] = lo << 7 | (uint32_t)min<uint64_t>(left, WAVE);
}

__device__ __forceinline__ uint32_t tab_filter(const uint32_t* __restrict__ tab, const uint64_t* __restrict__ runs,
                                               uint32_t nf, uint64_t i) {
  const uint64_t w = i / WAVE;
  const uint64_t wu = ((uint64_t)__builtin_amdgcn_readfirstlane((uint32_t)(w >> 32)) << 32) |
                      __builtin_amdgcn_readfirstlane((uint32_t)w);
  const uint32_t t = tab[wu];
  uint32_t lo = t >> 7;
  if ((uint32_t)(i & (WAVE - 1)) >= (t & 127u))
    while (lo + 1 < nf && runs[lo + 1] <= i) lo++;
  return lo;
}

__device__ __forceinline__ uint4 load_pplan(const uint4* __restrict__ pplans, uint32_t fid, uint32_t nf) {
  const uint32_t fs = __builtin_amdgcn_readfirstlane(fid);
  if (__builtin_amdgcn_ballot_w64(fid != fs) == 0) {
    if (fs >= nf) return make_uint4(0, 0, 0, 1);
#if __HIP_DEVICE_COMPILE__
    typedef __attribute__((address_space(4))) const uint32_t cu32;
    const cu32* c = reinterpret_cast<const cu32*>(reinterpret_cast<uintptr_t>(pplans + fs));
    return make_uint4(c[0], c[1], c[2], c[3]);
#else
    return pplans[fs];
#endif
  }
  return fid < nf ? pplans[fid] : make_uint4(0, 0, 0, 1);
}

__device__ __forceinline__ void split_fp(uint32_t h, uint32_t fp_size, uint32_t rem, uint32_t& bucket,
                                         uint32_t& remainder) {
  const uint32_t fp = h >> (32 - fp_size);
  bucket = rem >= 32 ? 0u : fp >> rem;
  remainder = fp & (rem >= 32 ? 0xffffffffu : ((1u << rem) - 1));
}

__device__ __forceinline__ bool probe_line(const uint4 P, uint32_t h, const uint4* __restrict__ lines,
                                           uint32_t fp_size, uint64_t& r) {
  const uint32_t vs = P.x & 0xff, rem = (P.x >> 8) & 0xff, rvs = (P.x >> 16) & 0xff, lgl = P.x >> 24;
  r = 0;
  if (P.w) return true;
  if (!lgl) return false;
  uint32_t bucket, remainder;
  split_fp(h, fp_size, rem, bucket, remainder);
  const v4u* lp = reinterpret_cast<const v4u*>(lines + ((uint64_t)P.y + (bucket >> (lgl - 1))) * 4);
  v4u Q[4];
#pragma unroll
  for (int k = 0; k < 4; k++) Q[k] = lp[k];
  return line_decode(Q, bucket & ((1u << (lgl - 1)) - 1), remainder, vs, rvs, r);
}

__device__ __forceinline__ uint64_t probe_walk(const uint4 P, uint32_t h, uint32_t fid,
                                               const FilterPlan* __restrict__ plans,
                                               const uint8_t* __restrict__ pages, const uint64_t* __restrict__ slots,
                                               uint32_t fp_size, uint32_t lis, uint32_t page_size) {
  const uint32_t vs = P.x & 0xff, rem = (P.x >> 8) & 0xff, rvs = (P.x >> 16) & 0xff;
  uint32_t bucket, remainder;
  split_fp(h, fp_size, rem, bucket, remainder);
  const uint64_t hdr = slots[P.z + (bucket >> lis)];
  const uint8_t* pg = pages + (uint64_t)plans[fid].page_base * page_size;
  return probe_stream(bucket & ((1u << lis) - 1), remainder, vs, rvs, pg, hdr, lis);
}

struct FieldOnes {
  uint64_t v[33];
  constexpr FieldOnes() : v() {
    for (uint32_t r = 1; r <= 32; r++) {
      uint64_t L = 0;
      for (uint32_t k = 0; k < 64; k += r) L |= 1ull << k;
      v[r] = L;
    }
  }
};
__constant__ FieldOnes c_field_ones = FieldOnes();

__device__ __forceinline__ uint32_t sload32(const void* p) {
#if __HIP_DEVICE_COMPILE__
  typedef __attribute__((address_space(4))) const uint32_t cu32;
  return *reinterpret_cast<const cu32*>(reinterpret_cast<uintptr_t>(p));
#else
  return *static_cast<const uint32_t*>(p);
#endif
}
__device__ __forceinline__ uint64_t sload64(const void* p) {
  return (uint64_t)sload32(p) | (uint64_t)sload32(static_cast<const uint32_t*>(p) + 1) << 32;
}

__device__ __forceinline__ bool line_decode_u(const uint32_t* Lw, uint32_t j, uint32_t remainder, uint32_t vs,
                                              uint32_t rvs, uint64_t L, uint64_t& found) {
  uint32_t p1, c;
  if (!line_bounds(*reinterpret_cast<const v4u*>(Lw), j, p1, c)) return false;
  found = 0;
  if (c == 0) return true;
  const uint32_t b = (p1 - j) * rvs, nb = c * rvs, wi = b >> 5, off = b & 31;
  if (off + nb > 96 || b + nb > 384 || nb > 64) return false;
  const uint64_t M = (L << rvs) - (L << vs);
  const uint64_t H = L << (rvs - 1);
  const uint64_t MH = M & ~H;
  const uint32_t w0 = Lw[4 + wi], w1 = Lw[5 + wi], w2 = Lw[6 + wi];
  const uint64_t W = (uint64_t)__builtin_amdgcn_alignbit(w2, w1, off) << 32 | __builtin_amdgcn_alignbit(w1, w0, off);
  const uint64_t Y = W ^ ((uint64_t)(remainder << vs) * L);
  const uint64_t valid = nb == 64 ? ~0ull : (1ull << nb) - 1;
  const uint64_t Z = H & valid & ~(((Y & MH) + MH) | Y);
  found = emit_matches(Z, W, rvs, vs);
  return true;
}

#ifndef RF_FAST_KSTRIDE
#define RF_FAST_KSTRIDE 1040
#endif
constexpr uint32_t FAST_KSTRIDE = RF_FAST_KSTRIDE;
constexpr int FAST_WBUF = (3 * FAST_KSTRIDE + 1024) / 16 + 1;

__device__ __forceinline__ void keys24_issue_dma(const uint8_t* kb, v4u* sw, uint32_t lane) {
  __builtin_amdgcn_global_load_lds((const __attribute__((address_space(1))) void*)(kb + lane * 16),
                                   (__attribute__((address_space(3))) void*)sw, 16, 0, 2);
  if (lane < 32)
    __builtin_amdgcn_global_load_lds((const __attribute__((address_space(1))) void*)(kb + 1024 + lane * 16),
                                     (__attribute__((address_space(3))) void*)(sw + WAVE), 16, 0, 2);
}
__device__ __forceinline__ void keys24_stage_partial(const uint8_t* kb, uint32_t bytes, v4u* sw, uint32_t lane) {
  const v4u* src = reinterpret_cast<const v4u*>(kb);
#pragma unroll
  for (uint32_t j = lane; j < 96; j += WAVE) {
    if ((j + 1) * 16 <= bytes) {
      sw[j] = __builtin_nontemporal_load(src + j);
    } else if (j * 16 < bytes) {
      const uint64_t t = __builtin_nontemporal_load(reinterpret_cast<const uint64_t*>(src + j));
      sw[j] = v4u{(uint32_t)t, (uint32_t)(t >> 32), 0u, 0u};
    }
  }
}
__device__ __forceinline__ uint32_t keys24_hash_lds(const v4u* sw, uint32_t lane, uint32_t seed) {
  const uint2* k2 = reinterpret_cast<const uint2*>(sw) + 3 * lane;
  const uint2 a = k2[0], b = k2[1], c = k2[2];
  const uint32_t w[6] = {a.x, a.y, b.x, b.y, c.x, c.y};
  return xxh32_24(w, seed);
}

template <int K, uint32_t STRIDE, bool ROT>
__device__ __forceinline__ void quad_gather_k(const uint8_t* fb, uint32_t lo, uint32_t q, uint32_t q16, uint8_t* sb) {
  const uint32_t lk = (uint32_t)__builtin_amdgcn_mov_dpp((int)lo, K * 0x55, 0xf, 0xf, false);
  const uint8_t* src;
  if constexpr (ROT) src = fb + lk + (((q + K) & 3u) << 4);
  else src = fb + (lk + q16);
  __builtin_amdgcn_global_load_lds((const __attribute__((address_space(1))) void*)src,
                                   (__attribute__((address_space(3))) void*)(sb + K * STRIDE), 16, 0, 0);
}
template <uint32_t STRIDE, bool ROT>
__device__ __forceinline__ void quad_gather(const uint8_t* fb, uint32_t lo, uint32_t q, uint8_t* sb) {
  const uint32_t q16 = q << 4;
  quad_gather_k<0, STRIDE, ROT>(fb, lo, q, q16, sb);
  quad_gather_k<1, STRIDE, ROT>(fb, lo, q, q16, sb);
  quad_gather_k<2, STRIDE, ROT>(fb, lo, q, q16, sb);
  quad_gather_k<3, STRIDE, ROT>(fb, lo, q, q16, sb);
}

template <int KIND>
__device__ __forceinline__ bool probe_fast(const uint4* __restrict__ pplans, const FilterPlan* __restrict__ plans,
                                           const uint8_t* __restrict__ pages, const uint64_t* __restrict__ slots,
                                           const uint4* __restrict__ lines, const void* __restrict__ in0,
                                           const uint32_t* __restrict__ wave_tab, uint64_t n,
                                           uint64_t* __restrict__ found, uint32_t fp_size, uint32_t seed, uint32_t lis,
                                           uint32_t page_size, uint32_t nf, uint64_t wf, v4u* sw) {
  if (wf + WAVE > n) return false;
  if (KIND == IN_KEYS24 && ((uintptr_t)in0 & 15)) return false;
  const uint32_t lane = threadIdx.x & (WAVE - 1);
  uint32_t h = 0;
  if constexpr (KIND == IN_KEYS24) {
    keys24_issue_dma(static_cast<const uint8_t*>(in0) + wf * 24, sw, lane);
  } else {
    h = __builtin_nontemporal_load(static_cast<const uint32_t*>(in0) + wf + lane);
  }
  const uint32_t t = sload32(wave_tab + wf / WAVE);
  if ((t & 127u) != WAVE) return false;
  const uint32_t fs = t >> 7;
  if (fs >= nf) return false;
  const uint4 U = make_uint4(sload32(&pplans[fs].x), sload32(&pplans[fs].y), sload32(&pplans[fs].z),
                             sload32(&pplans[fs].w));
  const uint32_t vs = U.x & 0xff, rem = (U.x >> 8) & 0xff, rvs = (U.x >> 16) & 0xff, lgl = U.x >> 24;
  if (U.w || !lgl || rem == 0 || rem >= 32 || rvs > 32) return false;
  if constexpr (KIND == IN_KEYS24) {
    asm volatile("s_waitcnt vmcnt(0)" ::: "memory");
    wave_sync_lds();
    h = keys24_hash_lds(sw, lane, seed);
  }
  const uint32_t lgG = lgl - 1;
  const uint32_t fp = h >> (32 - fp_size);
  const uint32_t bucket = fp >> rem;
  const uint32_t remainder = fp & ((1u << rem) - 1);
  const uint8_t* fb = reinterpret_cast<const uint8_t*>(lines) + ((uint64_t)U.y << 6);
  uint8_t* sb = reinterpret_cast<uint8_t*>(sw);
  quad_gather<FAST_KSTRIDE, false>(fb, (bucket >> lgG) << 6, lane & 3, sb);
  asm volatile("s_waitcnt vmcnt(0)" ::: "memory");
  wave_sync_lds();
  const uint32_t* Lw = reinterpret_cast<const uint32_t*>(sb + (lane & 3) * FAST_KSTRIDE + (lane >> 2) * 64);
  const uint64_t L = sload64(&c_field_ones.v[rvs]);
  uint64_t r;
  if (!line_decode_u(Lw, bucket & ((1u << lgG) - 1), remainder, vs, rvs, L, r))
    r = probe_walk(U, h, fs, plans, pages, slots, fp_size, lis, page_size);
  __builtin_nontemporal_store(r, found + wf + lane);
  return true;
}

template <int KIND>
__global__ __launch_bounds__(probe_nt(KIND)) void k_probe(const uint4* __restrict__ pplans,
                                                    const FilterPlan* __restrict__ plans,
                                                    const uint8_t* __restrict__ pages,
                                                    const uint64_t* __restrict__ slots,
                                                    const uint4* __restrict__ lines,
                                                    const void* __restrict__ in0,
                                                    const uint64_t* __restrict__ offs, uint32_t key_len,
                                                    const uint32_t* __restrict__ filter_id,
                                                    const uint64_t* __restrict__ runs,
                                                    const uint32_t* __restrict__ wave_tab, uint64_t n,
                                                    uint64_t* __restrict__ found, uint32_t fp_size,
                                                    uint32_t seed, uint32_t lis, uint32_t page_size,
                                                    uint32_t num_filters) {
  constexpr int NT = probe_nt(KIND);
  const uint64_t i0 = (uint64_t)xcd_chunk(blockIdx.x, gridDim.x) * NT + threadIdx.x;
  uint32_t h = 0, fid = 0xffffffffu;
  uint4 pp = make_uint4(0, 0, 0, 1);
  constexpr bool WAVE_KEYS = KIND == IN_KEYS24;
  constexpr bool WAVE_VAR = KIND == IN_VAR;
  constexpr int WBUF = WAVE_VAR ? 1 : FAST_WBUF;
  __shared__ v4u s_wbuf[NT / WAVE][WBUF];
  constexpr uint32_t VCAP = 4096;
  __shared__ __attribute__((aligned(16))) uint32_t s_vk[WAVE_VAR ? NT / WAVE : 1][WAVE_VAR ? VCAP / 4 + 4 : 1];
  const uint32_t lane = threadIdx.x & (WAVE - 1);
  const uint64_t wf = i0 - lane;
  if constexpr (KIND == IN_KEYS24 || KIND == IN_HASH) {
    if (runs) {
      const uint32_t wv = __builtin_amdgcn_readfirstlane(threadIdx.x) / WAVE;
      const uint64_t wfs = (uint64_t)xcd_chunk(blockIdx.x, gridDim.x) * NT + wv * WAVE;
      if (wfs < n && probe_fast<KIND>(pplans, plans, pages, slots, lines, in0, wave_tab, n, found, fp_size, seed,
                                      lis, page_size, num_filters, wfs, s_wbuf[wv]))
        return;
    }
  }
  if constexpr (WAVE_KEYS) {
    if (wf < n) {
      if (i0 < n) fid = runs ? tab_filter(wave_tab, runs, num_filters, i0) : __builtin_nontemporal_load(filter_id + i0);
      pp = load_pplan(pplans, fid, num_filters);
      if (((uintptr_t)in0 & 15) == 0) {
        v4u* sw = s_wbuf[threadIdx.x / WAVE];
        const uint32_t bytes = (uint32_t)min<uint64_t>(WAVE, n - wf) * 24;
        const uint8_t* kb = static_cast<const uint8_t*>(in0) + wf * 24;
        if (bytes == WAVE * 24) {
          keys24_issue_dma(kb, sw, lane);
          asm volatile("s_waitcnt vmcnt(0)" ::: "memory");
        } else {
          keys24_stage_partial(kb, bytes, sw, lane);
        }
        wave_sync_lds();
        if (i0 < n) h = keys24_hash_lds(sw, lane, seed);
      } else if (i0 < n) {
        h = hash_key<KIND, true>(in0, offs, key_len, seed, i0);
      }
    }
  } else if constexpr (WAVE_VAR) {
    uint64_t o0 = 0, o1 = 0;
    if (i0 < n) {
      fid = runs ? tab_filter(wave_tab, runs, num_filters, i0) : __builtin_nontemporal_load(filter_id + i0);
      o0 = offs[i0];
      o1 = offs[i0 + 1];
    }
    pp = load_pplan(pplans, fid, num_filters);
    uint64_t w0 = 0, w1 = 0;
    h = wave_hash_var<VCAP, true>(static_cast<const uint8_t*>(in0), o0, o1, i0 < n, s_vk[threadIdx.x / WAVE], seed,
                                  &w0, &w1);
  } else {
    if (i0 < n) {
      if constexpr (KIND == IN_PAIR) {
        const uint64_t pr = __builtin_nontemporal_load(static_cast<const uint64_t*>(in0) + i0);
        fid = (uint32_t)(pr >> 32);
        h = (uint32_t)pr;
      } else {
        fid = runs ? tab_filter(wave_tab, runs, num_filters, i0) : __builtin_nontemporal_load(filter_id + i0);
        h = hash_key<KIND, true>(in0, offs, key_len, seed, i0);
      }
    }
    pp = load_pplan(pplans, fid, num_filters);
  }
  const uint32_t fs = __builtin_amdgcn_readfirstlane(fid);
  const bool uniform = __builtin_amdgcn_ballot_w64(fid != fs) == 0;
  if (wf + WAVE <= n && uniform) {
    const uint4 U = make_uint4(__builtin_amdgcn_readfirstlane(pp.x), __builtin_amdgcn_readfirstlane(pp.y),
                               __builtin_amdgcn_readfirstlane(pp.z), __builtin_amdgcn_readfirstlane(pp.w));
    const uint32_t vs = U.x & 0xff, rem = (U.x >> 8) & 0xff, rvs = (U.x >> 16) & 0xff, lgl = U.x >> 24;
    if (!U.w && lgl) {
      uint32_t bucket, remainder;
      split_fp(h, fp_size, rem, bucket, remainder);
      const uint8_t* fb = reinterpret_cast<const uint8_t*>(lines) + ((uint64_t)U.y << 6);
      const uint32_t lo = (bucket >> (lgl - 1)) << 6;
      v4u* sw;
      if constexpr (WAVE_VAR) sw = reinterpret_cast<v4u*>(s_vk[threadIdx.x / WAVE]);
      else sw = s_wbuf[threadIdx.x / WAVE];
      quad_gather<WAVE * 16, true>(fb, lo, lane & 3, reinterpret_cast<uint8_t*>(sw));
      asm volatile("s_waitcnt vmcnt(0)" ::: "memory");
      wave_sync_lds();
      const uint32_t* L32 = reinterpret_cast<const uint32_t*>(sw + (lane & 3) * WAVE + (lane >> 2) * 4);
      const v4u E = *reinterpret_cast<const v4u*>(L32 + ((0u - lane) & 3u) * 4);
      auto win = [&](uint32_t wi, uint32_t& w0, uint32_t& w1, uint32_t& w2) {
        auto dw = [&](uint32_t d) -> uint32_t { d &= 15u; return L32[(((d >> 2) - lane) & 3u) * 4 + (d & 3u)]; };
        w0 = dw(4 + wi);
        w1 = dw(5 + wi);
        w2 = dw(6 + wi);
      };
      uint64_t r;
      if (!line_decode_w(E, win, bucket & ((1u << (lgl - 1)) - 1), remainder, vs, rvs, r))
        r = probe_walk(U, h, fs, plans, pages, slots, fp_size, lis, page_size);
      __builtin_nontemporal_store(r, found + i0);
      return;
    }
  }
  if (i0 >= n) return;
  uint64_t r;
  bool ok;
  if (uniform) {
    const uint4 U = make_uint4(__builtin_amdgcn_readfirstlane(pp.x), __builtin_amdgcn_readfirstlane(pp.y),
                               __builtin_amdgcn_readfirstlane(pp.z), __builtin_amdgcn_readfirstlane(pp.w));
    ok = probe_line(U, h, lines, fp_size, r);
  } else {
    ok = probe_line(pp, h, lines, fp_size, r);
  }
  if (!ok) r = probe_walk(pp, h, fid, plans, pages, slots, fp_size, lis, page_size);
  __builtin_nontemporal_store(r, found + i0);
}

template <int KIND>
__global__ __launch_bounds__(probe_nt(KIND)) void k_probe_floor(const uint4* __restrict__ pplans,
                                                          const uint4* __restrict__ lines,
                                                          const void* __restrict__ in0,
                                                          const uint32_t* __restrict__ wave_tab, uint64_t n,
                                                          uint64_t* __restrict__ found, uint32_t fp_size,
                                                          uint32_t nf) {
  constexpr int NT = probe_nt(KIND);
  __shared__ v4u s_wbuf[NT / WAVE][FAST_WBUF];
  const uint32_t wv = __builtin_amdgcn_readfirstlane(threadIdx.x) / WAVE;
  const uint64_t wf = (uint64_t)xcd_chunk(blockIdx.x, gridDim.x) * NT + wv * WAVE;
  const uint32_t lane = threadIdx.x & (WAVE - 1);
  if (wf >= n) return;
  v4u* sw = s_wbuf[wv];
  uint32_t h = 0;
  const bool full = wf + WAVE <= n;
  if constexpr (KIND == IN_KEYS24) {
    if (full) keys24_issue_dma(static_cast<const uint8_t*>(in0) + wf * 24, sw, lane);
  } else {
    if (full) h = __builtin_nontemporal_load(static_cast<const uint32_t*>(in0) + wf + lane);
  }
  const uint32_t t = sload32(wave_tab + wf / WAVE);
  const uint32_t fs = t >> 7;
  uint32_t lgl = 0, rem = 0, base = 0;
  if ((t & 127u) == WAVE && fs < nf && full) {
    const uint32_t x = sload32(&pplans[fs].x);
    lgl = x >> 24;
    rem = (x >> 8) & 0xff;
    base = sload32(&pplans[fs].y);
  }
  if (!lgl || rem == 0 || rem >= 32) {
    asm volatile("s_waitcnt vmcnt(0)" ::: "memory");
    if (wf + lane < n) found[wf + lane] = 0;
    return;
  }
  if constexpr (KIND == IN_KEYS24) {
    asm volatile("s_waitcnt vmcnt(0)" ::: "memory");
    wave_sync_lds();
    const uint2* k2 = reinterpret_cast<const uint2*>(sw) + 3 * lane;
    const uint2 a = k2[0], b = k2[1], c = k2[2];
    h = (a.x ^ a.y ^ b.x ^ b.y ^ c.x ^ c.y) * 0x9e3779b1u;
    h ^= h >> 15;
    h *= 0x85ebca77u;
  }
  const uint32_t bucket = (h >> (32 - fp_size)) >> rem;
  const uint8_t* fb = reinterpret_cast<const uint8_t*>(lines) + ((uint64_t)base << 6);
  uint8_t* sb = reinterpret_cast<uint8_t*>(sw);
  quad_gather<FAST_KSTRIDE, false>(fb, (bucket >> (lgl - 1)) << 6, lane & 3, sb);
  asm volatile("s_waitcnt vmcnt(0)" ::: "memory");
  wave_sync_lds();
  const v4u E = *reinterpret_cast<const v4u*>(sb + (lane & 3) * FAST_KSTRIDE + (lane >> 2) * 64);
  __builtin_nontemporal_store((uint64_t)(E[0] ^ E[1] ^ E[2] ^ E[3]), found + wf + lane);
}

__device__ __forceinline__ uint64_t probe_group(const ProbeGroup& G, uint32_t h) {
  const uint32_t fp_size = G.fpl & 0xff, lis = (G.fpl >> 8) & 0xff;
  const uint4 P = make_uint4(G.x, 0u, 0u, G.err);
  uint64_t r = 0;
  if (!probe_line(P, h, G.lines, fp_size, r)) {
    const uint32_t vs = G.x & 0xff, rem = (G.x >> 8) & 0xff, rvs = (G.x >> 16) & 0xff;
    uint32_t bucket, remainder;
    split_fp(h, fp_size, rem, bucket, remainder);
    r = probe_stream(bucket & ((1u << lis) - 1), remainder, vs, rvs, G.pages, G.slots[bucket >> lis], lis);
  }
  return r;
}

__global__ __launch_bounds__(256) void k_probe_groups(const uint32_t* __restrict__ in,
                                                      const ProbeGroup* __restrict__ groups, uint32_t ng,
                                                      uint64_t n, uint64_t* __restrict__ found,
                                                      uint32_t* __restrict__ counter,
                                                      uint32_t* __restrict__ done_flag, uint32_t seq) {
  const uint64_t i = (uint64_t)blockIdx.x * 256 + threadIdx.x;
  if (i < n) {
    const uint32_t h = in[i], g = in[n + i];
    uint64_t r = 0;
    if (g < ng) r = probe_group(groups[g], h);
    found[i] = r;
  }
  if (done_flag) {
    asm volatile("s_waitcnt vmcnt(0)" ::: "memory");
    __syncthreads();
    if (threadIdx.x == 0) {
      __threadfence_system();
      asm volatile("s_waitcnt vmcnt(0)" ::: "memory");
      const uint32_t last = gridDim.x - 1;
      if (last == 0 || __hip_atomic_fetch_add(counter, 1u, __ATOMIC_ACQ_REL, __HIP_MEMORY_SCOPE_AGENT) == last) {
        if (last) atomicExch(counter, 0u);
        __hip_atomic_store(done_flag, seq, __ATOMIC_RELEASE, __HIP_MEMORY_SCOPE_SYSTEM);
      }
    }
  }
}

__global__ __launch_bounds__(WAVE) void k_probe_small(SmallProbe a) {
  const uint32_t lane = threadIdx.x;
  if (lane < a.n) {
    const uint32_t h = a.h[lane], g = a.g[lane];
    uint64_t r = 0;
    if (g < a.ng) r = probe_group(a.groups[g], h);
    a.found[lane] = r;
  }
  asm volatile("s_waitcnt vmcnt(0)" ::: "memory");
  __builtin_amdgcn_wave_barrier();
  if (lane == 0) {
    __threadfence_system();
    asm volatile("s_waitcnt vmcnt(0)" ::: "memory");
    __hip_atomic_store(a.done_flag, a.seq, __ATOMIC_RELEASE, __HIP_MEMORY_SCOPE_SYSTEM);
  }
}

constexpr int FAN_NT = 256;
#ifndef RF_FAN_U
#define RF_FAN_U 2
#endif
constexpr int FAN_U = RF_FAN_U;
#ifndef RF_FAN_VCAP
#define RF_FAN_VCAP 4096
#endif
constexpr uint32_t FAN_VCAP = RF_FAN_VCAP;

template <int KIND>
__device__ __forceinline__ uint32_t fan_hash_chunk(const void* __restrict__ in0, const uint64_t* __restrict__ offs,
                                                   uint32_t key_len, uint32_t seed, uint64_t wf, uint32_t nk,
                                                   uint32_t lane, v4u* sw, uint32_t* svk) {
  constexpr bool WAVE_KEYS = KIND == IN_KEYS24;
  constexpr bool WAVE_VAR = KIND == IN_VAR;
  uint32_t h = 0;
  if constexpr (WAVE_KEYS) {
    if (((uintptr_t)in0 & 15) == 0) {
      const uint8_t* kb = static_cast<const uint8_t*>(in0) + wf * 24;
      if (nk == WAVE) {
        keys24_issue_dma(kb, sw, lane);
        asm volatile("s_waitcnt vmcnt(0)" ::: "memory");
      } else {
        keys24_stage_partial(kb, nk * 24, sw, lane);
      }
      wave_sync_lds();
      if (lane < nk) h = keys24_hash_lds(sw, lane, seed);
    } else if (lane < nk) {
      h = hash_key<KIND, true>(in0, nullptr, key_len, seed, wf + lane);
    }
  } else if constexpr (WAVE_VAR) {
    uint64_t o0 = 0, o1 = 0;
    if (lane < nk) {
      o0 = offs[wf + lane];
      o1 = offs[wf + lane + 1];
    }
    uint64_t win0 = 0, win1 = 0;
    h = wave_hash_var<FAN_VCAP, true>(static_cast<const uint8_t*>(in0), o0, o1, lane < nk, svk, seed, &win0,
                                      &win1);
  } else {
    if (lane < nk) h = hash_key<KIND, true>(in0, nullptr, key_len, seed, wf + lane);
  }
  return h;
}

template <int KIND>
__global__ __launch_bounds__(FAN_NT) void k_probe_fanout(const void* __restrict__ in0,
                                                         const uint64_t* __restrict__ offs, uint32_t key_len,
                                                         uint32_t seed, const ProbeGroup* __restrict__ groups,
                                                         uint32_t ng, const uint32_t* __restrict__ member,
                                                         uint32_t K, uint64_t n, uint64_t* __restrict__ found) {
  constexpr bool WAVE_KEYS = KIND == IN_KEYS24;
  constexpr bool WAVE_VAR = KIND == IN_VAR;
  constexpr int NW = FAN_NT / WAVE;
  __shared__ v4u s_keys[NW][WAVE_KEYS ? 96 : 1];
  constexpr uint32_t VCAP = FAN_VCAP;
  __shared__ __attribute__((aligned(16))) uint32_t s_vk[WAVE_VAR ? NW : 1][WAVE_VAR ? VCAP / 4 + 4 : 1];
  __shared__ uint32_t s_h[NW][WAVE];
  const uint32_t lane = threadIdx.x & (WAVE - 1);
  const uint32_t wv = __builtin_amdgcn_readfirstlane(threadIdx.x) / WAVE;
  const uint64_t nwaves = (n + WAVE - 1) / WAVE;
  const uint32_t q64 = WAVE / K, r64 = WAVE % K;
  for (uint64_t wc = (uint64_t)blockIdx.x * NW + wv; wc < nwaves; wc += (uint64_t)gridDim.x * NW) {
    const uint64_t wf = wc * WAVE;
    const uint32_t nk = (uint32_t)min<uint64_t>(WAVE, n - wf);
    const uint32_t h = fan_hash_chunk<KIND>(in0, offs, key_len, seed, wf, nk, lane, s_keys[wv], s_vk[wv]);
    s_h[wv][lane] = h;
    wave_sync_lds();
    const uint64_t pbase = wf * K;
    const uint64_t np = (uint64_t)nk * K;
    uint32_t key = lane / K, slot = lane % K;
    for (uint64_t p0 = lane; p0 < np + lane; p0 += (uint64_t)WAVE * FAN_U) {
      uint32_t kk[FAN_U], g[FAN_U], st[FAN_U], px[FAN_U], pf[FAN_U], hh[FAN_U], pj[FAN_U], pr[FAN_U];
      v4u Q[FAN_U][4];
#pragma unroll
      for (int u = 0; u < FAN_U; u++) {
        kk[u] = key;
        g[u] = 0xffffffffu;
        if (key < nk) g[u] = member ? __builtin_nontemporal_load(member + pbase + p0 + (uint64_t)u * WAVE) : slot;
        const uint64_t s2 = (uint64_t)slot + r64;
        key += q64 + (s2 >= K ? 1u : 0u);
        slot = (uint32_t)(s2 >= K ? s2 - K : s2);
      }
      uint64_t pl[FAN_U];
#pragma unroll
      for (int u = 0; u < FAN_U; u++) {
        if (g[u] >= ng) g[u] = 0xffffffffu;
        const uint32_t gs = __builtin_amdgcn_readfirstlane(g[u]);
        uint32_t err = 1;
        px[u] = pf[u] = 0;
        pl[u] = 0;
        if (__builtin_amdgcn_ballot_w64(g[u] != gs) == 0) {
          if (gs != 0xffffffffu) {
            const ProbeGroup* G = groups + gs;
            px[u] = sload32(&G->x);
            err = sload32(&G->err);
            pf[u] = sload32(&G->fpl);
            pl[u] = sload64(&G->lines);
          }
        } else if (g[u] != 0xffffffffu) {
          const ProbeGroup* G = groups + g[u];
          px[u] = G->x;
          err = G->err;
          pf[u] = G->fpl;
          pl[u] = (uint64_t)(uintptr_t)G->lines;
        }
        st[u] = err ? 0u : ((px[u] >> 24) ? 1u : 2u);
      }
#pragma unroll
      for (int u = 0; u < FAN_U; u++) {
        hh[u] = s_h[wv][kk[u] & (WAVE - 1)];
        pj[u] = pr[u] = 0;
        if (st[u] == 1) {
          const uint32_t rem = (px[u] >> 8) & 0xff, lgl = px[u] >> 24, fp_size = pf[u] & 0xff;
          uint32_t bucket, remainder;
          split_fp(hh[u], fp_size, rem, bucket, remainder);
          pr[u] = remainder;
          pj[u] = bucket & ((1u << (lgl - 1)) - 1);
          const v4u* lp = reinterpret_cast<const v4u*>((uintptr_t)pl[u]) + (uint64_t)(bucket >> (lgl - 1)) * 4;
#pragma unroll
          for (int k = 0; k < 4; k++) Q[u][k] = lp[k];
        }
      }
#pragma unroll
      for (int u = 0; u < FAN_U; u++) {
        uint64_t r = 0;
        bool walk = st[u] == 2;
        if (st[u] == 1) walk = !line_decode(Q[u], pj[u], pr[u], px[u] & 0xff, (px[u] >> 16) & 0xff, r);
        if (walk) r = probe_group(groups[g[u]], hh[u]);
        if (kk[u] < nk) __builtin_nontemporal_store(r, found + pbase + p0 + (uint64_t)u * WAVE);
      }
    }
    wave_sync_lds();
  }
}

template <int KIND>
__global__ __launch_bounds__(FAN_NT) void k_probe_fanout_ragged(const void* __restrict__ in0,
                                                                const uint64_t* __restrict__ offs,
                                                                uint32_t key_len, uint32_t seed,
                                                                const ProbeGroup* __restrict__ groups, uint32_t ng,
                                                                const uint32_t* __restrict__ member,
                                                                const uint64_t* __restrict__ moff, uint64_t n,
                                                                uint64_t* __restrict__ found) {
  constexpr bool WAVE_KEYS = KIND == IN_KEYS24;
  constexpr bool WAVE_VAR = KIND == IN_VAR;
  constexpr int NW = FAN_NT / WAVE;
  __shared__ v4u s_keys[NW][WAVE_KEYS ? 96 : 1];
  __shared__ __attribute__((aligned(16))) uint32_t s_vk[WAVE_VAR ? NW : 1][WAVE_VAR ? FAN_VCAP / 4 + 4 : 1];
  __shared__ uint32_t s_h[NW][WAVE];
  __shared__ uint32_t s_off[NW][WAVE];
  const uint32_t lane = threadIdx.x & (WAVE - 1);
  const uint32_t wv = __builtin_amdgcn_readfirstlane(threadIdx.x) / WAVE;
  const uint64_t nwaves = (n + WAVE - 1) / WAVE;
  for (uint64_t wc = (uint64_t)blockIdx.x * NW + wv; wc < nwaves; wc += (uint64_t)gridDim.x * NW) {
    const uint64_t wf = wc * WAVE;
    const uint32_t nk = (uint32_t)min<uint64_t>(WAVE, n - wf);
    const uint64_t pbase = moff[wf];
    const uint32_t np = (uint32_t)(moff[wf + nk] - pbase);
    if (np == 0) continue;
    s_off[wv][lane] = lane < nk ? (uint32_t)(moff[wf + lane] - pbase) : np;
    const uint32_t h = fan_hash_chunk<KIND>(in0, offs, key_len, seed, wf, nk, lane, s_keys[wv], s_vk[wv]);
    s_h[wv][lane] = h;
    wave_sync_lds();
    for (uint32_t p0 = lane; p0 < np + lane; p0 += (uint32_t)WAVE * FAN_U) {
      uint32_t g[FAN_U], st[FAN_U], px[FAN_U], pf[FAN_U], hh[FAN_U], pj[FAN_U], pr[FAN_U];
      v4u Q[FAN_U][4];
#pragma unroll
      for (int u = 0; u < FAN_U; u++) {
        const uint32_t p = p0 + (uint32_t)u * WAVE;
        g[u] = 0xffffffffu;
        if (p < np) g[u] = __builtin_nontemporal_load(member + pbase + p);
      }
#pragma unroll
      for (int u = 0; u < FAN_U; u++) {
        hh[u] = s_h[wv][wave_owner_of(s_off[wv], p0 + (uint32_t)u * WAVE)];
      }
      uint64_t pl[FAN_U];
#pragma unroll
      for (int u = 0; u < FAN_U; u++) {
        if (g[u] >= ng) g[u] = 0xffffffffu;
        const uint32_t gs = __builtin_amdgcn_readfirstlane(g[u]);
        uint32_t err = 1;
        px[u] = pf[u] = 0;
        pl[u] = 0;
        if (__builtin_amdgcn_ballot_w64(g[u] != gs) == 0) {
          if (gs != 0xffffffffu) {
            const ProbeGroup* G = groups + gs;
            px[u] = sload32(&G->x);
            err = sload32(&G->err);
            pf[u] = sload32(&G->fpl);
            pl[u] = sload64(&G->lines);
          }
        } else if (g[u] != 0xffffffffu) {
          const ProbeGroup* G = groups + g[u];
          px[u] = G->x;
          err = G->err;
          pf[u] = G->fpl;
          pl[u] = (uint64_t)(uintptr_t)G->lines;
        }
        st[u] = err ? 0u : ((px[u] >> 24) ? 1u : 2u);
      }
#pragma unroll
      for (int u = 0; u < FAN_U; u++) {
        pj[u] = pr[u] = 0;
        if (st[u] == 1) {
          const uint32_t rem = (px[u] >> 8) & 0xff, lgl = px[u] >> 24, fp_size = pf[u] & 0xff;
          uint32_t bucket, remainder;
          split_fp(hh[u], fp_size, rem, bucket, remainder);
          pr[u] = remainder;
          pj[u] = bucket & ((1u << (lgl - 1)) - 1);
          const v4u* lp = reinterpret_cast<const v4u*>((uintptr_t)pl[u]) + (uint64_t)(bucket >> (lgl - 1)) * 4;
#pragma unroll
          for (int k = 0; k < 4; k++) Q[u][k] = lp[k];
        }
      }
#pragma unroll
      for (int u = 0; u < FAN_U; u++) {
        const uint32_t p = p0 + (uint32_t)u * WAVE;
        uint64_t r = 0;
        bool walk = st[u] == 2;
        if (st[u] == 1) walk = !line_decode(Q[u], pj[u], pr[u], px[u] & 0xff, (px[u] >> 16) & 0xff, r);
        if (walk) r = probe_group(groups[g[u]], hh[u]);
        if (p < np) __builtin_nontemporal_store(r, found + pbase + p);
      }
    }
    wave_sync_lds();
  }
}

constexpr int FC_NT = 256;
constexpr int FC_PER = 16;
constexpr uint32_t FC_TILE = FC_NT * FC_PER;
constexpr uint32_t FC_MAX_GRID = 1u << 20;

__global__ __launch_bounds__(FC_NT) void k_found_count(const uint64_t* __restrict__ found, uint64_t m,
                                                       uint64_t ntiles, uint32_t* __restrict__ cnt) {
  __shared__ uint32_t s_c[FC_NT / WAVE];
  for (uint64_t t = blockIdx.x; t < ntiles; t += gridDim.x) {
    const uint64_t t0 = t * FC_TILE;
    uint32_t c = 0;
#pragma unroll
    for (int k = 0; k < FC_PER; k++) {
      const uint64_t i = t0 + (uint64_t)k * FC_NT + threadIdx.x;
      if (i < m) c += (uint32_t)__popcll(found[i]);
    }
    const uint32_t s = block_sum<FC_NT>(c, s_c);
    if (threadIdx.x == 0) cnt[t] = s;
  }
}

__global__ __launch_bounds__(1024) void k_found_scan(const uint32_t* __restrict__ cnt, uint64_t ntiles,
                                                     uint64_t* __restrict__ off, uint64_t* __restrict__ count) {
  __shared__ uint32_t s_tmp[1024 / WAVE + 1];
// ... 335 lines not shown
  if (v < 0) {
    const char* e = getenv("RF_AMD_K4_BITMAP");
    v = (e && e[0] == '0') ? 0 : 1;
  }
  return v != 0;
}
static std::atomic<uint64_t> g_k4_bitmap_builds{0};
extern "C" uint64_t rf_k4_bitmap_builds(void) { return g_k4_bitmap_builds.load(std::memory_order_relaxed); }
static std::atomic<uint64_t> g_part16_builds{0};
extern "C" uint64_t rf_part16_builds(void) { return g_part16_builds.load(std::memory_order_relaxed); }

template <typename EntT, bool FL = (sizeof(EntT) == 8), bool DUAL = false, bool RUNS = false>
static int launch_sort_t(const LaunchArgs& a, EntT* ent, EntT* part, const uint32_t* spill, bool bitmap = false) {
  if constexpr (DUAL) {
    hipLaunchKernelGGL((k_cb_merge<RUNS>), dim3(a.num_cb), dim3(SORT_NT), 0, (hipStream_t)a.stream, a.plans, a.cb_filter,
                     a.cb_count, a.cb_start, (const uint32_t*)part, a.old32, a.ob_lo, a.ob_n, a.sorted32, a.idx_cnt,
                     a.idx_start, a.outs, a.overflow, a.lis, a.first_old, a.has_old, spill, a.cb_outs);
    CHECK_LAUNCH();
    hipLaunchKernelGGL((k_cb_sort<EntT, FL, true, true, RUNS>), dim3(a.num_cb), dim3(SORT_NT), 0, (hipStream_t)a.stream,
                       a.plans, a.cb_filter, a.cb_count, a.cb_start, part, a.old32, a.ob_lo, a.ob_n, a.sorted32,
                       a.idx_cnt, a.idx_start, a.outs, a.overflow, a.lis, a.first_old, a.has_old, spill, a.cb_outs,
                       a.overflow);
  } else {
    bool launched = false;
    if constexpr (sizeof(EntT) == 4 && !FL && !RUNS) {
      if (bitmap) {
        launched = true;
        hipLaunchKernelGGL(k_cb_bitmap, dim3(a.num_cb), dim3(SORT_NT), 0, (hipStream_t)a.stream, a.plans, a.cb_filter,
                           a.cb_count, a.cb_start, part, a.sorted32, a.idx_cnt, a.idx_start, a.outs, a.overflow, a.lis,
                           spill);
        g_k4_bitmap_builds.fetch_add(1, std::memory_order_relaxed);
      }
    }
    if (!launched) {
      hipLaunchKernelGGL((k_cb_sort<EntT, FL, false, false, RUNS>), dim3(a.num_cb), dim3(SORT_NT), 0, (hipStream_t)a.stream, a.plans,
                         a.cb_filter, a.cb_count, a.cb_start, part, a.old32, a.ob_lo, a.ob_n, a.sorted32, a.idx_cnt,
                         a.idx_start, a.outs, a.overflow, a.lis, a.first_old, a.has_old, spill, a.cb_outs, nullptr);
    }
  }
  CHECK_LAUNCH();
  REC(EV_B_SORT);
  hipLaunchKernelGGL((k_cb_sort_big<EntT, FL, DUAL, RUNS>), dim3(BIG_GRID), dim3(BIG_NT), 0, (hipStream_t)a.stream, a.plans,
                     a.cb_filter, a.cb_count, a.cb_start, part, a.old32, a.ob_lo, a.ob_n, ent, a.sorted32, a.idx_cnt, a.idx_start, a.outs,
                     a.overflow, a.lis, a.first_old, a.has_old, spill, a.cb_outs);
  CHECK_LAUNCH();
  REC(EV_B_SORT_BIG);
  return 0;
}

static int launch_plines_list(const LaunchArgs& a) {
  if (!a.line_lmax || !a.num_page_slots) return 0;
  const size_t lds = 4ull * (256 / WAVE) * (a.line_lmax + 1);
  const uint32_t grid = a.num_page_slots < 1024 ? a.num_page_slots : 1024;
  hipLaunchKernelGGL(k_plines_list, dim3(grid), dim3(256), lds, (hipStream_t)a.stream, a.plans, a.pg_filter,
                     a.page_first, a.slots, a.pages, a.pg_noline, a.lines, a.line_lmax, a.lis, a.page_size);
  CHECK_LAUNCH();
  return 0;
}

template <bool RUNS>
static int launch_build_t(const LaunchArgs& a) {
  const TileRuns runs{a.tile_value, a.tile_end};
  if (a.wide && a.flag32) {
    uint32_t* ent = (uint32_t*)a.ent;
    uint32_t* part = (uint32_t*)a.part;
    if (a.num_tiles) {
#define L(K) hipLaunchKernelGGL((k_hash_scatter<K, true, RUNS>), dim3(a.num_tiles), dim3(SCAT_NT), 0, (hipStream_t)a.stream, \
                                a.plans, a.tile_filter, a.tile_start, a.in0, a.offs, a.key_len, a.fp_size, a.seed, \
                                part, a.cb_count, a.spill, runs)
      KIND_SWITCH(a.kind, L);
#undef L
      CHECK_LAUNCH();
    }
    if (a.num_tiles) {
      const CountFold fold{nullptr, 0, a.spill + 1, a.cb_count, a.cb_start, a.num_filters};
      if (int rc = launch_hash_count_t<uint32_t, true, RUNS>(a, ent, a.cb_cursor, a.spill, fold)) return rc;
    }
    if (int rc = launch_scatter_t<uint32_t, true, RUNS>(a, ent, part, a.spill)) return rc;
    if (a.num_cb) {
      hipLaunchKernelGGL(k_old_cb_bounds, dim3((a.num_cb + 255) / 256), dim3(256), 0, (hipStream_t)a.stream, a.plans,
                         a.cb_filter, a.num_cb, a.old32, a.old_tot, a.fp_size, a.lis, a.ob_lo, a.ob_n, a.cb_count);
      CHECK_LAUNCH();
    }
    REC(EV_B_HASH);
    hipLaunchKernelGGL(k_cb_scan, dim3(a.num_filters), dim3(256), 0, (hipStream_t)a.stream, a.plans, a.cb_count,
                       a.cb_count, a.cb_outs, a.cb_outs, nullptr);
    CHECK_LAUNCH();
    REC(EV_B_SCAN);
    REC(EV_B_SCATTER);
    if (int rc = launch_sort_t<uint32_t, true, true, RUNS>(a, ent, part, a.spill)) return rc;
  } else if (a.wide) {
    uint64_t* ent = (uint64_t*)a.ent;
    uint64_t* part = (uint64_t*)a.part;
    if (a.num_old_tiles) {
      hipLaunchKernelGGL(k_old_count, dim3(a.num_old_tiles), dim3(TILE_NT), 0, (hipStream_t)a.stream, a.plans,
                         a.old_tile_filter, a.old_tile_start, a.fp_size, ent, a.cb_count);
      CHECK_LAUNCH();
    }
    if (a.num_tiles) { int rc = launch_hash_count_t<uint64_t, true, RUNS>(a, ent, a.cb_count, nullptr, CountFold{}); if (rc) return rc; }
    REC(EV_B_HASH);
    hipLaunchKernelGGL(k_cb_scan, dim3(a.num_filters), dim3(256), 0, (hipStream_t)a.stream, a.plans, a.cb_count,
                       a.cb_count, a.cb_start, a.cb_cursor, nullptr);
    CHECK_LAUNCH();
    REC(EV_B_SCAN);
    if (int rc = launch_scatter_t<uint64_t, true, RUNS>(a, ent, part, nullptr)) return rc;
    REC(EV_B_SCATTER);
    if (int rc = launch_sort_t<uint64_t, true, false, RUNS>(a, ent, part, nullptr)) return rc;
  } else {
    uint32_t* ent = (uint32_t*)a.ent;
    uint32_t* part = (uint32_t*)a.part;
    bool bitmap = false;
    if constexpr (!RUNS) bitmap = a.k4_bitmap && k4_bitmap_enabled();
    if (a.num_tiles) {
#define L(K) hipLaunchKernelGGL((k_hash_scatter<K, false, RUNS, P16>), dim3(a.num_tiles), dim3(SCAT_NT), 0, (hipStream_t)a.stream, \
                                a.plans, a.tile_filter, a.tile_start, a.in0, a.offs, a.key_len, a.fp_size, a.seed, \
                                part, a.cb_count, a.spill, runs)
      if constexpr (!RUNS) {
        if (bitmap) {
          constexpr bool P16 = true;
          KIND_SWITCH(a.kind, L);
        }
      }
      if (!bitmap) {
        constexpr bool P16 = false;
        KIND_SWITCH(a.kind, L);
      }
#undef L
      CHECK_LAUNCH();
    }
    if (bitmap) g_part16_builds.fetch_add(1, std::memory_order_relaxed);
    REC(EV_B_HASH);
    if (a.num_tiles) {
      const CountFold fold{a.zero_outs ? (uint32_t*)a.outs : nullptr, (uint32_t)(sizeof(FilterOut) / 4) * a.num_filters,
                           a.spill + 1, a.cb_count, a.cb_start, a.num_filters};
      if (int rc = launch_hash_count_t<uint32_t, false, RUNS>(a, ent, a.cb_cursor, a.spill, fold)) return rc;
    }
    REC(EV_B_SCAN);
    if (int rc = launch_scatter_t<uint32_t, false, RUNS>(a, ent, part, a.spill)) return rc;
    REC(EV_B_SCATTER);
    if (int rc = launch_sort_t<uint32_t, false, false, RUNS>(a, ent, part, a.spill, bitmap)) return rc;
  }
  const BuildClean clean = a.self_clean ? BuildClean{a.cb_count, a.cb_cursor, a.overflow, a.spill}
                                        : BuildClean{nullptr, nullptr, nullptr, nullptr};
  if (a.lay_whole || !a.lay_grid) {
    hipLaunchKernelGGL(k_layout, dim3(a.num_filters), dim3(LAYOUT_NT), 0, (hipStream_t)a.stream, a.plans, a.idx_cnt,
                       a.idx_start, a.sorted32, a.first_old, a.has_old, a.pplans_mut, a.slots, a.page_first, a.outs,
                       a.lis, a.page_size, a.lay_grid ? a.lay_seg : 0u, clean);
    CHECK_LAUNCH();
  }
  if (a.lay_grid) {
    hipLaunchKernelGGL(k_layout_seg, dim3(a.lay_grid), dim3(LAYOUT_NT), 0, (hipStream_t)a.stream, a.plans, a.lay_wg,
                       a.lay_hand, a.lay_seq, a.lay_seg, a.idx_cnt, a.idx_start, a.sorted32, a.first_old, a.has_old,
                       a.pplans_mut, a.slots, a.page_first, a.outs, a.lis, a.page_size, clean);
    CHECK_LAUNCH();
  }
  REC(EV_B_LAYOUT);
  hipLaunchKernelGGL(k_assemble, dim3(a.num_page_slots), dim3(ASM_NT), 0, (hipStream_t)a.stream, a.plans, a.pg_filter,
                     a.idx_cnt, a.idx_start, a.sorted32, a.slots, a.page_first, a.outs, a.pages, a.lines,
                     a.pg_noline, a.lis, a.page_size);
  CHECK_LAUNCH();
  if (a.plines_needed)
    if (int rc = launch_plines_list(a)) return rc;
  REC(EV_B_ASSEMBLE);
  return 0;
}

extern "C" int rf_launch_build(const LaunchArgs* pa) {
  return pa->tile_value ? launch_build_t<true>(*pa) : launch_build_t<false>(*pa);
}

extern "C" int rf_launch_plines(const LaunchArgs* pa) {
  const LaunchArgs& a = *pa;
  if (!a.line_lmax) return 0;
  const size_t lds = 4ull * (256 / WAVE) * (a.line_lmax + 1);
  hipLaunchKernelGGL(k_plines, dim3((a.num_idx + 3) / 4), dim3(256), lds, (hipStream_t)a.stream, a.plans,
                     a.idx_filter, a.slots, a.pages, a.outs, a.lines, a.num_idx, a.line_lmax, a.lis,
                     a.page_size, a.plines_force);
  CHECK_LAUNCH();
  return 0;
}

extern "C" int rf_launch_old_decode(const LaunchArgs* pa) {
  const LaunchArgs& a = *pa;
  if (a.num_old_idx == 0) return 0;
  hipLaunchKernelGGL(k_old_counts, dim3((a.num_old_idx + 255) / 256), dim3(256), 0, (hipStream_t)a.stream, a.plans,
                     a.old_idx_filter, a.num_old_idx, a.old_cnt);
  CHECK_LAUNCH();
  hipLaunchKernelGGL(k_old_scan, dim3(a.num_filters), dim3(LAYOUT_NT), 0, (hipStream_t)a.stream, a.plans, a.old_cnt,
                     a.old_pos, a.flag32 ? nullptr : (uint64_t*)a.ent, a.old_tot);
  CHECK_LAUNCH();
  const uint32_t waves_per_block = 256 / WAVE;
  hipLaunchKernelGGL(k_old_decode, dim3((a.num_old_idx + waves_per_block - 1) / waves_per_block), dim3(256), 0,
                     (hipStream_t)a.stream, a.plans, a.old_idx_filter, a.num_old_idx, a.old_pos,
                     a.flag32 ? nullptr : (uint64_t*)a.ent, a.flag32 ? a.old32 : nullptr, a.lis, a.fp_size);
  CHECK_LAUNCH();
  return 0;
}

__global__ __launch_bounds__(256) void k_seg_fill(const uint32_t* __restrict__ pre, uint32_t nf, uint32_t n,
                                                  uint32_t* __restrict__ fof, uint32_t* __restrict__ start,
                                                  uint32_t mul) {
  const uint32_t i = blockIdx.x * blockDim.x + threadIdx.x;
  if (i >= n) return;
  uint32_t lo = 0, hi = nf;
  while (hi - lo > 1) {
    const uint32_t mid = (lo + hi) >> 1;
    if (pre[mid] <= i) lo = mid; else hi = mid;
  }
  fof[i] = lo;
  if (start) start[i] = (i - pre[lo]) * mul;
}

extern "C" int rf_launch_seg_fill(void* stream, const uint32_t* pre, uint32_t nf, uint32_t n, uint32_t* fof,
                                  uint32_t* start, uint32_t mul) {
  if (n == 0) return 0;
  hipLaunchKernelGGL(k_seg_fill, dim3((n + 255) / 256), dim3(256), 0, (hipStream_t)stream, pre, nf, n, fof, start, mul);
  CHECK_LAUNCH();
  return 0;
}

extern "C" int rf_launch_wave_tab(void* stream, const uint64_t* runs, uint32_t nf, uint64_t n, uint32_t* tab) {
  const uint64_t nw = (n + WAVE - 1) / WAVE;
  if (nw == 0) return 0;
  hipLaunchKernelGGL(k_wave_tab, dim3((uint32_t)((nw + 255) / 256)), dim3(256), 0, (hipStream_t)stream, runs, nf, n, tab);
  CHECK_LAUNCH();
  return 0;
}

extern "C" int rf_launch_probe_floor(const LaunchArgs* pa, int kind, const void* in0, uint64_t n, uint64_t* found) {
  const LaunchArgs& a = *pa;
  if (n == 0) return 0;
  if (!a.wave_tab || (kind != IN_KEYS24 && kind != IN_HASH)) return (int)hipErrorInvalidValue;
  const int nt = probe_nt(kind);
  dim3 g((uint32_t)((n + nt - 1) / nt)), b(nt);
  if (kind == IN_KEYS24)
    hipLaunchKernelGGL((k_probe_floor<IN_KEYS24>), g, b, 0, (hipStream_t)a.stream, a.pplans, a.lines, in0, a.wave_tab, n,
                       found, a.fp_size, a.num_filters);
  else
    hipLaunchKernelGGL((k_probe_floor<IN_HASH>), g, b, 0, (hipStream_t)a.stream, a.pplans, a.lines, in0, a.wave_tab, n,
                       found, a.fp_size, a.num_filters);
  CHECK_LAUNCH();
  return 0;
}

extern "C" int rf_launch_probe(const LaunchArgs* pa, int kind, const void* in0, const uint64_t* offs,
                               uint32_t key_len, const uint32_t* filter_id, uint64_t n, uint64_t* found) {
  const LaunchArgs& a = *pa;
  if (n == 0) return 0;
  const int nt = probe_nt(kind);
  dim3 g((uint32_t)((n + nt - 1) / nt)), b(nt);
  REC(EV_P_START);
#define PK(K) hipLaunchKernelGGL((k_probe<K>), g, b, 0, (hipStream_t)a.stream, a.pplans, a.plans, a.pages, a.slots, a.lines, in0, offs, key_len, filter_id, a.probe_runs, a.wave_tab, n, found, a.fp_size, a.seed, a.lis, a.page_size, a.num_filters)
  switch (kind) {
    KEY_KIND_CASES(PK)
    case IN_PAIR: PK(IN_PAIR); break;
    default: PK(IN_HASH); break;
  }
#undef PK
  CHECK_LAUNCH();
  REC(EV_P_END);
  return 0;
}
```

### splinterdb_amd/csrc/rf_plan.h

```cpp
#pragma once
#include <hip/hip_runtime.h>
#include <stdint.h>

namespace rf {

constexpr uint32_t MAX_PAGE = 4096;
constexpr uint32_t MAX_INDICES = 16384;
constexpr uint32_t MAX_LIS = 12;
constexpr uint32_t CB_LOG_MEAN = 12;
constexpr uint32_t MAX_CB = 2048;
constexpr uint32_t MAX_BINS = 4096;
constexpr uint32_t MAX_IPC = 512;

constexpr int TILE_NT = 256;
#ifndef RF_TILE_KEYS
#define RF_TILE_KEYS 16384
#endif
constexpr int TILE_KEYS = RF_TILE_KEYS;
constexpr int SCAT_NT = 512;
constexpr int SORT_NT = 512;
constexpr int SORT_CAP = 9216;
#ifndef RF_REGION_PAD
#define RF_REGION_PAD 0
#endif
// ... 3 lines not shown
constexpr int BIG_NT = 1024;
constexpr int BIG_GRID = 64;
constexpr int LAYOUT_NT = 1024;
constexpr int ASM_NT = 128;
constexpr uint32_t ASM_MAXB = 128;
constexpr uint32_t ASM_GT = 1024;

enum InputKind { IN_KEYS24 = 0, IN_KEYS_W = 1, IN_KEYS_B = 2, IN_VAR = 3, IN_HASH = 4, IN_PAIR = 5 };

inline int fixed_kind(const void* p, uint32_t key_len) {
  const uintptr_t u = (uintptr_t)p;
  if (key_len == 24 && (u & 7) == 0) return IN_KEYS24;
  if ((key_len & 3) == 0 && (u & 3) == 0) return IN_KEYS_W;
  return IN_KEYS_B;
}

constexpr uint32_t ERR_INDEX_OVERFLOW = 1u, ERR_BLOCK_TOO_BIG = 2u, ERR_PAGE_CAP = 4u,
                   ERR_GEOMETRY = 8u;

struct FilterOut {
  uint32_t num_unique;
  uint32_t num_pages;
  uint32_t error;
  uint32_t pad;
};

struct FilterPlan {
  uint64_t e_first;
  uint64_t key_first;
  uint64_t old_first;
  uint32_t num_new;
  uint32_t old_region;
  uint32_t num_fp;
  uint32_t value;
  uint32_t vs, rem, rvs, lnb;
  uint32_t num_indices;
  uint32_t cbits, bbits;
  uint32_t binsh;
  uint32_t cb_base, idx_base, page_base, page_cap, pf_base;
  uint32_t lg_line, line_base;
  uint32_t lines_asm;
  uint32_t old_num_indices, old_vs, old_rvs, npo;
  uint32_t old_idx_base;
  uint32_t lines_flag;
  const uint8_t* old_pages;
  const uint64_t* old_slots;
  uint32_t old_direct;
  uint32_t old_cbits, old_bbits;
  const uint32_t* old_entries;
  const uint32_t* old_idx_start;
  const uint32_t* old_idx_cnt;
  const FilterOut* old_out;
};
__host__ __device__ inline uint32_t old_error(const FilterPlan& P) { return P.old_out ? P.old_out->error : 0u; }

constexpr uint32_t LAYOUT_SEG_MAX = 4096, LAYOUT_SEG_MIN = 256;
constexpr uint32_t LAYOUT_MAX_GROUPS = MAX_INDICES / LAYOUT_SEG_MIN;
__host__ __device__ inline uint32_t layout_groups(const FilterPlan& p, uint32_t seg) {
  return (seg && p.num_indices > seg && p.npo <= seg) ? p.num_indices / seg : 1u;
}

struct EstFilter {
  const uint8_t* pages;
  const uint64_t* slots;
  uint32_t vs, rvs;
  uint32_t num_idx;
  uint32_t idx_first;
};

struct ProbeGroup {
  uint32_t x;
  uint32_t err;
  uint32_t fpl;
  uint32_t pad;
  const uint4* lines;
  const uint8_t* pages;
  const uint64_t* slots;
};

constexpr uint32_t SRV_RING = 4096;
constexpr uint32_t SRV_REQ_WORDS = 16;
struct SrvReq {
  uint64_t w[SRV_REQ_WORDS];
};
static_assert(sizeof(SrvReq) == 128, "one request per two 64-byte lines");
struct SrvRes {
  uint64_t w[4];
};
static_assert(sizeof(SrvRes) == 32, "two answers per 64-byte line");
__host__ __device__ inline uint32_t srv_check(uint64_t t) { return (uint32_t)(t / SRV_RING) + 1u; }
struct SrvCtl {
  uint64_t unused;
  uint64_t exit_head;
  uint64_t exit_gen;
  uint64_t served;
  uint64_t prof[6];
};

constexpr uint32_t SMALL_PROBES = 64, SMALL_GROUPS = 8;
struct SmallProbe {
  uint32_t n, ng, seq;
  uint32_t h[SMALL_PROBES];
  uint8_t g[SMALL_PROBES];
  ProbeGroup groups[SMALL_GROUPS];
  uint64_t* found;
  uint32_t* done_flag;
// ... 13 lines not shown
  SetUpdEntry e[SET_UPD_PER_LAUNCH];
};
static_assert(sizeof(SetUpdEntry) == 56, "40 bytes of ProbeGroup, the id, the error word's address");
static_assert(sizeof(SetUpdate) == 16 + 56 * SET_UPD_PER_LAUNCH && sizeof(SetUpdate) <= 4096,
              "one launch's entries fit HIP's 4,096 bytes of kernel arguments");

struct LaunchArgs {
  void* stream;
  int kind;
  int wide;
  const FilterPlan* plans;
  const uint4* pplans;
  uint4* pplans_mut;
  uint32_t num_filters;
  const uint32_t* tile_filter;
  const uint32_t* tile_start;
  uint32_t num_tiles;
  const uint32_t* tile_value;
  const uint32_t* tile_end;
  const uint32_t* old_tile_filter;
  const uint32_t* old_tile_start;
  uint32_t num_old_tiles;
  const uint32_t* old_idx_filter;
  uint32_t num_old_idx;
  uint32_t* old_cnt;
  uint32_t* old_pos;
  uint32_t flag32;
  uint32_t* old32;
  uint32_t* old_tot;
  uint32_t* ob_lo;
  uint32_t* ob_n;
  const void* in0;
  const uint64_t* offs;
  uint32_t key_len, fp_size, seed, lis, page_size;
  void* ent;
  void* part;
  uint32_t* sorted32;
  uint32_t* cb_count;
  uint32_t* cb_start;
  uint32_t* cb_cursor;
  const uint32_t* cb_filter;
  uint32_t num_cb;
  uint32_t* overflow;
  uint32_t* spill;
  uint32_t* idx_cnt;
  uint32_t* idx_start;
  uint32_t* first_old;
  uint32_t* has_old;
  uint64_t* slots;
  uint4* lines;
  uint32_t line_lmax;
  uint32_t plines_needed;
  uint32_t plines_force;
  const uint32_t* idx_filter;
  uint32_t num_idx;
  uint32_t* page_first;
  uint32_t* pg_noline;
  uint32_t* cb_outs;
  const uint32_t* pg_filter;
  uint32_t num_page_slots;
  uint8_t* pages;
  FilterOut* outs;
  const uint32_t* lay_wg;
  uint32_t lay_grid;
  uint64_t* lay_hand;
  uint32_t lay_seq;
  uint32_t lay_seg;
  uint32_t lay_whole;
  uint32_t k4_bitmap;
  uint32_t self_clean;
  uint32_t zero_outs;
  const uint64_t* probe_runs;
  const uint32_t* wave_tab;
  void** events;
  uint32_t ev_mask;
};

enum EventSlot { EV_B_START = 0, EV_B_HASH, EV_B_SCAN, EV_B_SCATTER, EV_B_SORT, EV_B_SORT_BIG,
                 EV_B_LAYOUT, EV_B_ASSEMBLE, EV_P_START, EV_P_END, NUM_EVENTS };
constexpr uint32_t EV_MASK_ALL = (1u << NUM_EVENTS) - 1;
constexpr uint32_t EV_MASK_PROBE = 1u << EV_P_START | 1u << EV_P_END;

}
```

### splinterdb_amd/engine.py

```python
import ctypes
import os
from dataclasses import dataclass

import numpy as np

HERE = os.path.dirname(os.path.abspath(__file__))
LIB_PATH = os.path.join(HERE, "librf_amd.so")

STATUS_OK = 0
STATUS_NO_MEMORY = 12
STATUS_NO_DEVICE = 19
STATUS_BAD_PARAM = 22
MAX_FILTERS = 32
ROUTING_NOT_FOUND = 0xFFFF

EXPORTED = [
    "rf_amd_engine_create", "rf_amd_engine_destroy", "rf_amd_last_error",
    "rf_amd_batch_create", "rf_amd_batch_destroy", "rf_amd_batch_build_keys",
    "rf_amd_batch_build_var_keys", "rf_amd_batch_build_hashes", "rf_amd_batch_probe_keys",
    "rf_amd_batch_probe_var_keys", "rf_amd_batch_probe_hashes", "rf_amd_batch_info",
    "rf_amd_batch_probe_keys_runs", "rf_amd_batch_probe_hashes_runs",
    "rf_amd_batch_read_image", "rf_amd_batch_read_image_async", "rf_amd_batch_image_ptrs", "rf_amd_batch_num_filters",
    "rf_amd_batch_set_timing", "rf_amd_batch_timings", "rf_amd_batch_timings_back", 
    "rf_amd_debug_read_lines", "rf_amd_debug_rebuild_lines", "rf_amd_debug_phase_buffer", "rf_amd_diag_lookup_stats",
    "rf_amd_debug_probe_floor",
    "rf_amd_host_alloc", "rf_amd_host_free", "rf_amd_engine_fence", "rf_amd_engine_fence_wait",
    "rf_amd_host_register", "rf_amd_host_unregister", "rf_amd_batch_place_image", "rf_amd_engine_set_pool_limit",
    "rf_amd_lookup_submit", "rf_amd_lookup_wait", "rf_amd_lookup_reap", "rf_amd_lookup_server_stats",
    "rf_amd_build_id",
    "rf_amd_filter_add", "rf_amd_filter_lookup_hashes", "rf_amd_filter_lookup_keys",
    "rf_amd_image_free",
    "rf_amd_max_fingerprints", "rf_amd_estimate_unique_keys_from_count",
    "rf_amd_space_use_bytes",
    "rf_amd_estimate_unique_fp", "rf_amd_batch_estimate_unique_fp", "rf_amd_estimate_unique_keys",
    "rf_amd_lookup_async", "rf_amd_lookup_async_poll", "rf_amd_lookup_async_wait",
    "rf_amd_lookup_async_free", "rf_amd_filter_verify", "rf_amd_filter_print",
    "rf_amd_hash_keys", "rf_amd_hash_var_keys",
    "rf_amd_batch_export", "rf_amd_batch_import", "rf_amd_route_scratch_bytes", "rf_amd_route_probes", "rf_amd_batch_probe_pairs", "rf_amd_unroute_found",
    "rf_amd_batch_build_hashes_host", "rf_amd_batch_probe_hashes_host", "rf_amd_engine_pool_stats",
    "rf_amd_filter_print_abs", "rf_amd_batch_infos", "rf_amd_batch_destroy_on", "rf_amd_probe_many_hashes_host",
    "rf_amd_probe_filters_host", "rf_amd_engine_pool_trim", "rf_amd_engine_stream", "rf_amd_engine_sync",
    "rf_amd_batch_device_bytes", "rf_amd_batch_trim", "rf_amd_batch_stage_begin", "rf_amd_batch_stage_build",
    "rf_amd_batch_stage_abort", "rf_amd_lookup_server_error", "rf_amd_lookup_server_failed",
    "rf_amd_lookup_server_set_times", "rf_amd_diag_lookup_server_kill", "rf_amd_diag_lookup_ring",
    "rf_amd_batch_create_runs", "rf_amd_filter_add_runs", "rf_amd_diag_k4_bitmap_builds",
    "rf_amd_filter_set_create", "rf_amd_filter_set_destroy", "rf_amd_filter_set_num_members",
    "rf_amd_filter_set_probe_keys", "rf_amd_filter_set_probe_hashes",
    "rf_amd_found_compact_scratch_bytes", "rf_amd_found_compact",
    "rf_amd_filter_set_probe_var_keys", "rf_amd_batch_probe_var_keys_runs", "rf_amd_filter_lookup_var_keys",
    "rf_amd_diag_fanout_max_blocks", "rf_amd_diag_lookup_paths", "rf_amd_diag_part16_builds",
    "rf_amd_filter_set_probe_keys_ragged", "rf_amd_filter_set_probe_var_keys_ragged",
    "rf_amd_filter_set_probe_hashes_ragged",
    "rf_amd_filter_set_create_cap", "rf_amd_filter_set_capacity", "rf_amd_filter_set_update",
    "rf_amd_filter_set_destroy_on",
    "rf_amd_range_map_create", "rf_amd_range_map_destroy", "rf_amd_range_map_destroy_on",
    "rf_amd_range_map_num_ranges", "rf_amd_range_map_max_list", "rf_amd_range_route_scratch_bytes",
    "rf_amd_range_map_route_keys", "rf_amd_range_map_route_var_keys",
    "rf_amd_diag_range_tile", "rf_amd_diag_range_lds_ranges",
]
ROUTE_MAX_WORLD = 16
FOUND_COMPACT_TILE = 4096
ASYNC_STATUS_RUNNING = 0
ASYNC_STATUS_DONE = 1
CALLBACK_FN = ctypes.CFUNCTYPE(None, ctypes.c_void_p)


class PlatformStatusError(RuntimeError):
    def __init__(self, code, msg):
        super().__init__(f"platform_status {code}: {msg}")
        self.code = code


class RfConfig(ctypes.Structure):
    _fields_ = [("fingerprint_size", ctypes.c_uint32), ("log_index_size", ctypes.c_uint32),
                ("seed", ctypes.c_uint32), ("page_size", ctypes.c_uint32),
                ("pages_per_extent", ctypes.c_uint32)]


class RfFilterInfo(ctypes.Structure):
    _fields_ = [("num_fingerprints", ctypes.c_uint32), ("num_unique", ctypes.c_uint32),
                ("value_size", ctypes.c_uint32), ("num_indices", ctypes.c_uint32),
                ("num_pages", ctypes.c_uint32), ("error", ctypes.c_uint32)]


class RfImage(ctypes.Structure):
    _fields_ = [("info", RfFilterInfo), ("pages", ctypes.POINTER(ctypes.c_uint8)),
                ("slots", ctypes.POINTER(ctypes.c_uint64))]


_lib = None


def check_build_id(L, path):
    from . import build as _b
    L.rf_amd_build_id.restype = ctypes.c_char_p
    got = L.rf_amd_build_id().decode()
    try:
        want = _b.source_id()
    except OSError:
        return
    if got != want:
        raise RuntimeError(f"{path} was built from other sources (build id {got}, tree {want}): "
                           "rebuild it (python -c 'import __graft_entry__ as g; g.build()')")
# ... 6 lines not shown
    path = os.environ.get("RF_AMD_LIB", LIB_PATH)
    if not os.path.exists(path):
        if not build_if_missing or path != LIB_PATH:
            raise PlatformStatusError(STATUS_NO_DEVICE, f"{path} missing (run build)")
        from . import build as _b
        _b.build()
    L = ctypes.CDLL(path)
    check_build_id(L, path)
    vp, u32, u64, i32 = ctypes.c_void_p, ctypes.c_uint32, ctypes.c_uint64, ctypes.c_int
    L.rf_amd_last_error.restype = ctypes.c_char_p
    L.rf_amd_engine_create.argtypes = [i32, ctypes.POINTER(vp)]
    L.rf_amd_engine_destroy.argtypes = [vp]
    L.rf_amd_engine_destroy.restype = None
    L.rf_amd_batch_create.argtypes = [vp, ctypes.POINTER(RfConfig), u32, vp, vp, vp, vp,
                                      ctypes.POINTER(vp)]
    L.rf_amd_batch_create_runs.argtypes = [vp, ctypes.POINTER(RfConfig), u32, vp, vp, vp, vp, vp,
                                           ctypes.POINTER(vp)]
    L.rf_amd_batch_destroy.argtypes = [vp]
    L.rf_amd_batch_destroy.restype = None
    L.rf_amd_batch_build_keys.argtypes = [vp, vp, u32, vp]
    L.rf_amd_batch_build_var_keys.argtypes = [vp, vp, vp, vp]
    L.rf_amd_batch_build_hashes.argtypes = [vp, vp, vp]
    L.rf_amd_batch_probe_keys.argtypes = [vp, vp, u32, vp, u64, vp, vp]
    L.rf_amd_batch_probe_var_keys.argtypes = [vp, vp, vp, vp, u64, vp, vp]
    L.rf_amd_batch_probe_hashes.argtypes = [vp, vp, vp, u64, vp, vp]
    L.rf_amd_batch_probe_keys_runs.argtypes = [vp, vp, u32, ctypes.POINTER(u64), vp, vp]
    L.rf_amd_batch_probe_hashes_runs.argtypes = [vp, vp, ctypes.POINTER(u64), vp, vp]
    L.rf_amd_batch_info.argtypes = [vp, u32, ctypes.POINTER(RfFilterInfo)]
    L.rf_amd_batch_read_image.argtypes = [vp, u32, vp, u64, vp, u32]
    L.rf_amd_batch_read_image_async.argtypes = [vp, u32, vp, u64, vp, u32, vp]
    L.rf_amd_batch_image_ptrs.argtypes = [vp, u32, ctypes.POINTER(vp), ctypes.POINTER(vp)]
    L.rf_amd_batch_set_timing.argtypes = [vp, i32]
    L.rf_amd_batch_timings.argtypes = [vp, ctypes.POINTER(ctypes.c_float), u32]
    L.rf_amd_batch_timings_back.argtypes = [vp, u32, ctypes.POINTER(ctypes.c_float), u32]
    L.rf_amd_debug_read_lines.argtypes = [vp, vp, u64, ctypes.POINTER(u64)]
    L.rf_amd_debug_rebuild_lines.argtypes = [vp]
    L.rf_amd_debug_phase_buffer.argtypes = [vp, u32]
    L.rf_amd_debug_probe_floor.argtypes = [vp, vp, u32, vp, vp, vp]
    L.rf_amd_diag_lookup_stats.argtypes = [vp, ctypes.c_int]
    L.rf_amd_diag_lookup_paths.argtypes = [vp, ctypes.c_int]
    L.rf_amd_lookup_submit.argtypes = [vp, vp, u32, u32, vp, ctypes.POINTER(u64)]
    L.rf_amd_lookup_wait.argtypes = [vp, u64, ctypes.POINTER(u64)]
    L.rf_amd_lookup_reap.argtypes = [vp, vp, vp, u64]
    L.rf_amd_lookup_reap.restype = u64
    L.rf_amd_lookup_server_stats.argtypes = [vp, vp]
    L.rf_amd_lookup_server_error.argtypes = [vp]
    L.rf_amd_lookup_server_failed.argtypes = [vp, vp, u64]
    L.rf_amd_lookup_server_failed.restype = u64
    L.rf_amd_lookup_server_set_times.argtypes = [vp, u64, u64]
    L.rf_amd_diag_lookup_server_kill.argtypes = [vp, i32, u32]
    L.rf_amd_diag_lookup_ring.argtypes = [vp]
    L.rf_amd_diag_k4_bitmap_builds.argtypes = []
    L.rf_amd_diag_k4_bitmap_builds.restype = u64
    L.rf_amd_diag_part16_builds.argtypes = []
    L.rf_amd_diag_part16_builds.restype = u64
    L.rf_amd_batch_num_filters.argtypes = [vp]
    L.rf_amd_batch_num_filters.restype = u32
    L.rf_amd_filter_add.argtypes = [vp, ctypes.POINTER(RfConfig), ctypes.POINTER(RfImage),
                                    ctypes.POINTER(RfImage), vp, u64, ctypes.c_uint16]
    L.rf_amd_filter_add_runs.argtypes = [vp, ctypes.POINTER(RfConfig), ctypes.POINTER(RfImage),
                                         ctypes.POINTER(RfImage), vp, vp, vp, u32]
    L.rf_amd_filter_lookup_hashes.argtypes = [vp, ctypes.POINTER(RfConfig),
                                              ctypes.POINTER(RfImage), vp, u64, vp]
    L.rf_amd_filter_lookup_keys.argtypes = [vp, ctypes.POINTER(RfConfig), ctypes.POINTER(RfImage),
                                            vp, u32, u64, vp]
    L.rf_amd_image_free.argtypes = [ctypes.POINTER(RfImage)]
    L.rf_amd_image_free.restype = None
    L.rf_amd_max_fingerprints.argtypes = [ctypes.POINTER(RfConfig)]
    L.rf_amd_max_fingerprints.restype = u64
    L.rf_amd_estimate_unique_keys_from_count.argtypes = [ctypes.POINTER(RfConfig), u64]
    L.rf_amd_estimate_unique_keys_from_count.restype = u32
    L.rf_amd_space_use_bytes.argtypes = [ctypes.POINTER(RfConfig), u32]
    L.rf_amd_space_use_bytes.restype = u64
    L.rf_amd_estimate_unique_fp.argtypes = [vp, ctypes.POINTER(RfConfig), vp, u64,
                                            ctypes.POINTER(u32)]
    L.rf_amd_batch_estimate_unique_fp.argtypes = [vp, vp, u64, ctypes.POINTER(u32)]
    L.rf_amd_estimate_unique_keys.argtypes = [ctypes.POINTER(RfFilterInfo), ctypes.POINTER(RfConfig)]
    L.rf_amd_estimate_unique_keys.restype = u32
    L.rf_amd_lookup_async.argtypes = [vp, vp, u32, vp, u64, vp, CALLBACK_FN, vp, vp,
                                      ctypes.POINTER(vp)]
    L.rf_amd_lookup_async_poll.argtypes = [vp]
    L.rf_amd_lookup_async_wait.argtypes = [vp]
    L.rf_amd_lookup_async_free.argtypes = [vp]
    L.rf_amd_lookup_async_free.restype = None
    L.rf_amd_filter_verify.argtypes = [vp, ctypes.POINTER(RfConfig), ctypes.POINTER(RfImage), vp, u32,
                                       u64, ctypes.c_uint16, ctypes.POINTER(u64)]
    L.rf_amd_filter_print.argtypes = [ctypes.POINTER(RfConfig), ctypes.POINTER(RfImage), vp]
    L.rf_amd_hash_keys.argtypes = [vp, ctypes.POINTER(RfConfig), vp, u32, u64, vp, vp]
    L.rf_amd_hash_var_keys.argtypes = [vp, ctypes.POINTER(RfConfig), vp, vp, u64, vp, vp]
    L.rf_amd_batch_export.argtypes = [vp, vp, u64, vp, u64, vp]
    L.rf_amd_batch_import.argtypes = [vp, ctypes.POINTER(RfConfig), u32, ctypes.POINTER(RfFilterInfo), vp, vp,
                                      i32, ctypes.POINTER(vp)]
    L.rf_amd_route_scratch_bytes.argtypes = [u64, u32]
    L.rf_amd_route_scratch_bytes.restype = u64
    L.rf_amd_route_probes.argtypes = [vp, vp, vp, u64, vp, u32, u32, vp, vp, vp, ctypes.POINTER(u64), vp]
    L.rf_amd_batch_probe_pairs.argtypes = [vp, vp, u64, vp, vp]
    L.rf_amd_unroute_found.argtypes = [vp, vp, vp, u64, vp, vp]
    L.rf_amd_batch_build_hashes_host.argtypes = [vp, vp]
    L.rf_amd_batch_probe_hashes_host.argtypes = [vp, vp, vp, u64, vp]
    L.rf_amd_engine_pool_stats.argtypes = [vp, ctypes.POINTER(u64), ctypes.POINTER(u64), ctypes.POINTER(u64)]
    L.rf_amd_filter_print_abs.argtypes = [ctypes.POINTER(RfConfig), ctypes.POINTER(RfImage), u64, vp, vp]
    L.rf_amd_batch_infos.argtypes = [vp, ctypes.POINTER(RfFilterInfo), vp]
    L.rf_amd_batch_destroy_on.argtypes = [vp, vp]
    L.rf_amd_probe_many_hashes_host.argtypes = [vp, vp, vp, vp, u32, vp, vp]
    L.rf_amd_probe_filters_host.argtypes = [vp, vp, vp, u32, vp, vp, u64, vp]
    L.rf_amd_engine_pool_trim.argtypes = [vp, u64]
# ... 936 lines not shown
```

Baseline: 45890 Mkeys/s.

## Add dense non-power-of-two line groups for probe lines on large fresh filters

Introduces a dense line layout in which each 512-bit probe line covers an arbitrary group size G rather than a power of two. G is chosen as the largest group whose expected occupancy fits a tighter unary budget, and the layout is enabled by default for fresh filters whose line table exceeds 4 MiB. Fewer lines shrink the line table, which is meant to cut memory traffic and cache pressure during probe. In exchange the kernels pick up float-reciprocal division and extra template variants, and the change also adds a waves-per-EU occupancy hint to the fanout probe kernels.

```diff
diff --git a/include/rf_amd_diag.h b/include/rf_amd_diag.h
--- a/include/rf_amd_diag.h
+++ b/include/rf_amd_diag.h
@@ -27,6 +27,8 @@
 
 uint64_t rf_amd_diag_k4_bitmap_builds(void);
 
+uint64_t rf_amd_diag_dense_line_filters(void);
+
 uint64_t rf_amd_diag_part16_builds(void);
 
 int rf_amd_diag_fanout_max_blocks(uint32_t blocks);
diff --git a/splinterdb_amd/csrc/rf_batch_plan.h b/splinterdb_amd/csrc/rf_batch_plan.h
--- a/splinterdb_amd/csrc/rf_batch_plan.h
+++ b/splinterdb_amd/csrc/rf_batch_plan.h
@@ -34,8 +34,21 @@
   return 0;
 }
 
+inline uint32_t line_dense_group(uint32_t lis, uint32_t rvs, double lam, double sigma, uint32_t L_now) {
+  if (rvs > 32) return 0;
+  const uint32_t IS = 1u << lis;
+  for (uint32_t L = 1; L < L_now && L <= 256; L++) {
+    const uint32_t G = (IS + L - 1) / L;
+    if (G > 64) continue;
+    const double mean = lam * G, cap = (double)(line_unary_bits(G, rvs) - G);
+    if (mean + sigma * sqrt(mean) + 2.0 <= cap) return G;
+  }
+  return 0;
+}
+constexpr uint64_t LINE_DENSE_MIN_TABLE = 4ull << 20;
+
 inline int lines_in_assembly(uint32_t lis, uint32_t lg_line, uint32_t page_size) {
-  const uint32_t IS = 1u << lis, L = IS >> (lg_line - 1);
+  const uint32_t IS = 1u << lis, L = lines_per_index(lis, lg_line);
   const uint32_t min_block = 2 + (IS - 1) / 8 + 4 + 3;
   const uint32_t maxb = page_size / min_block + 1;
   if (maxb > ASM_MAXB || L + 1 > ASM_GT) return 0;
@@ -48,6 +61,8 @@
   bool old_resplit_off = false;
   uint32_t layout_seg = LAYOUT_SEG_MAX;
   double line_sigma = 3.5;
+  int lines_dense = -1;
+  double dense_sigma = 2.5;
 };
 
 struct OldFilter {
@@ -89,6 +104,7 @@
   uint64_t NL = 0;
   bool plines_needed = false;
   uint32_t line_lmax = 0;
+  bool lines_dense = false;
   uint32_t lay_seg = 0, lay_grid = 0;
   bool lay_whole = true;
   std::vector<uint32_t> lay_wg;
@@ -112,16 +128,24 @@
   return 0;
 }
 
-inline void probe_geometry(FilterPlan& p, const rf_amd_config& cfg, double sigma, uint64_t* line_total,
-                           uint32_t* line_lmax) {
+inline void probe_geometry(FilterPlan& p, const rf_amd_config& cfg, const PlanKnobs& knobs, bool fresh,
+                           uint64_t* line_total, uint32_t* line_lmax, bool* any_dense) {
   const uint32_t lis = cfg.log_index_size;
+  const double lam = (double)p.num_fp / (double)(1ull << p.lnb);
   p.rem = cfg.fingerprint_size - p.lnb;
   p.rvs = p.rem + p.vs;
-  p.lg_line = line_log_group(lis, p.rvs, (double)p.num_fp / (double)(1ull << p.lnb), sigma);
+  p.lg_line = line_log_group(lis, p.rvs, lam, knobs.line_sigma);
+  if (p.lg_line && knobs.lines_dense != 0) {
+    const uint32_t L = lines_per_index(lis, p.lg_line);
+    if (knobs.lines_dense > 0 || (fresh && (uint64_t)p.num_indices * L * 64 > LINE_DENSE_MIN_TABLE))
+      if (const uint32_t G = line_dense_group(lis, p.rvs, lam, knobs.dense_sigma, L)) p.lg_line = LINE_DENSE | (G - 1);
+  }
   p.line_base = (uint32_t)*line_total;
   if (p.lg_line) {
-    *line_total += (uint64_t)p.num_indices << (lis - (p.lg_line - 1));
-    *line_lmax = std::max(*line_lmax, (1u << lis) >> (p.lg_line - 1));
+    const uint32_t L = lines_per_index(lis, p.lg_line);
+    if (line_is_dense(p.lg_line)) *any_dense = true;
+    *line_total += (uint64_t)p.num_indices * L;
+    *line_lmax = std::max(*line_lmax, L);
   }
 }
 
@@ -322,7 +346,7 @@
     p.idx_base = b.I;
     p.page_base = b.PS;
     p.pf_base = b.PF;
-    probe_geometry(p, cfg, knobs.line_sigma, &b.NL, &b.line_lmax);
+    probe_geometry(p, cfg, knobs, !op && !b.chained, &b.NL, &b.line_lmax, &b.lines_dense);
     const int la = p.lg_line ? lines_in_assembly(lis, p.lg_line, cfg.page_size) : 0;
     p.lines_asm = la != 0;
     p.lines_flag = la == 2;
@@ -400,7 +424,7 @@
     p.page_cap = in.num_pages;
     p.page_base = (uint32_t)pages_total;
     p.idx_base = (uint32_t)idx_total;
-    probe_geometry(p, cfg, knobs.line_sigma, &b.NL, &b.line_lmax);
+    probe_geometry(p, cfg, knobs, true, &b.NL, &b.line_lmax, &b.lines_dense);
     if (p.lg_line) b.plines_needed = true;
     b.pplans[f] = pack_pplan(p);
     pages_total += in.num_pages;
diff --git a/splinterdb_amd/csrc/rf_engine.cpp b/splinterdb_amd/csrc/rf_engine.cpp
--- a/splinterdb_amd/csrc/rf_engine.cpp
+++ b/splinterdb_amd/csrc/rf_engine.cpp
@@ -299,10 +299,20 @@
     k.layout_seg = (v < LAYOUT_SEG_MIN || (v & (v - 1))) ? 0 : v > LAYOUT_SEG_MAX ? LAYOUT_SEG_MAX : (uint32_t)v;
   }
   if (const char* e = getenv("RF_AMD_LINE_SIGMA"); e && atof(e) > 0.0) k.line_sigma = atof(e);
+  if (const char* e = getenv("RF_AMD_LINES_DENSE"); e && *e) k.lines_dense = e[0] == '0' ? 0 : 1;
+  if (const char* e = getenv("RF_AMD_DENSE_SIGMA"); e && atof(e) > 0.0) k.dense_sigma = atof(e);
   return k;
 }
 
 extern "C" const char* rf_amd_last_error(void) { return g_err.c_str(); }
+
+static std::atomic<uint64_t> g_dense_line_filters{0};
+template <typename Batch>
+static void note_dense_lines(const Batch* b) {
+  uint64_t n = 0;
+  for (const FilterPlan& p : b->plans) n += line_is_dense(p.lg_line) ? 1 : 0;
+  if (n) g_dense_line_filters.fetch_add(n, std::memory_order_relaxed);
+}
 
 static std::mutex g_live_mu;
 static std::vector<rf_amd_engine*>* g_live = nullptr;
@@ -848,6 +858,7 @@
   a.slots = b->d_slots.as<uint64_t>();
   a.lines = b->d_lines.as<uint4>();
   a.line_lmax = b->line_lmax;
+  a.lines_dense = b->lines_dense ? 1u : 0u;
   a.plines_needed = b->plines_needed ? 1u : 0u;
   a.pg_noline = b->d_pg_noline.as<uint32_t>();
   a.idx_filter = b->d_idx_filter.as<uint32_t>();
@@ -913,6 +924,7 @@
     if (int rc = launch_rc("old decode", rf_launch_old_decode(&a))) return rc;
   }
   b->err_ready.store(false, std::memory_order_release);
+  note_dense_lines(b);
   int rc = rf_launch_build(&a);
   if (st == b->eng->stream) b->eng->builds_issued.fetch_add(1, std::memory_order_acq_rel);
   if (rc) return launch_rc("build", rc);
@@ -1589,6 +1601,7 @@
 extern "C" const char* rf_amd_build_id(void) { return RF_AMD_SRC_ID; }
 
 extern "C" uint64_t rf_amd_diag_k4_bitmap_builds(void) { return rf_k4_bitmap_builds(); }
+extern "C" uint64_t rf_amd_diag_dense_line_filters(void) { return g_dense_line_filters.load(std::memory_order_relaxed); }
 extern "C" uint64_t rf_amd_diag_part16_builds(void) { return rf_part16_builds(); }
 
 extern "C" int rf_amd_diag_lookup_stats(uint64_t* out, int reset) {
@@ -2322,6 +2335,7 @@
   HIPCHK(hipMemcpyAsync(b->d_pplans.p, b->pplans.data(), 16ull * F, hipMemcpyHostToDevice, st));
   {
     LaunchArgs a = make_args(b, st);
+    note_dense_lines(b);
     if (int lrc = launch_rc("probe-line", rf_launch_plines(&a))) return lrc;
   }
   HIPCHK(hipStreamSynchronize(st));
diff --git a/splinterdb_amd/csrc/rf_kernels.hip b/splinterdb_amd/csrc/rf_kernels.hip
--- a/splinterdb_amd/csrc/rf_kernels.hip
+++ b/splinterdb_amd/csrc/rf_kernels.hip
@@ -2128,12 +2128,88 @@
 constexpr uint32_t ASM_RUN = 16;
 constexpr uint32_t ASM_MAXE = 16384;
 
+__device__ __forceinline__ float rcp_small(uint32_t d) { return __builtin_amdgcn_rcpf((float)d); }
+__device__ __forceinline__ uint32_t div_small(uint32_t x, float r) { return (uint32_t)(((float)x + 0.5f) * r); }
+
+struct LineGeo {
+  uint32_t G, L, U, lgG;
+  float rG;
+  bool dense;
+  __device__ __forceinline__ uint32_t group(uint32_t b) const { return dense ? div_small(b, rG) : b >> lgG; }
+};
+template <bool DENSE>
+__device__ __forceinline__ LineGeo line_geo(uint32_t lg_line, uint32_t rvs, uint32_t lis) {
+  LineGeo g;
+  g.dense = DENSE && line_is_dense(lg_line);
+  g.lgG = g.dense ? 0u : lg_line - 1;
+  g.G = g.dense ? line_group(lg_line) : 1u << g.lgG;
+  g.rG = g.dense ? rcp_small(g.G) : 0.0f;
+  g.L = g.dense ? div_small((1u << lis) - 1u, g.rG) + 1u : (1u << lis) >> g.lgG;
+  g.U = g.dense ? line_unary_bits(g.G, rvs) : 128u;
+  return g;
+}
+__device__ __forceinline__ void line_locate(const LineGeo& g, uint32_t bucket, uint32_t lis, uint32_t& line,
+                                            uint32_t& j) {
+  if (g.dense) {
+    const uint32_t bo = bucket & ((1u << lis) - 1u), k = div_small(bo, g.rG);
+    line = (bucket >> lis) * g.L + k;
+    j = bo - k * g.G;
+  } else {
+    line = bucket >> g.lgG;
+    j = bucket & (g.G - 1u);
+  }
+}
+
+template <typename Bits64>
+__device__ __forceinline__ void dense_line_quarter(Bits64 bits64, uint32_t qq, uint32_t U, uint32_t ne, uint32_t n,
+                                                   uint32_t rvs, uint32_t ecode, uint32_t efield, uint64_t (&w)[2]) {
+  const uint32_t ue = min(U, ne);
+  const uint32_t fe = U + (rvs ? min(n, (512u - U) / rvs) * rvs : 0u);
+#pragma unroll
+  for (int h = 0; h < 2; h++) {
+    const uint32_t o = qq * 128 + h * 64;
+    uint64_t x = 0;
+    if (o < ue) x = bits64(ecode + o) & lowmask64(min(64u, ue - o));
+    const uint32_t lo = max(o, U), hi = min(o + 64u, fe);
+    if (lo < hi) x |= (bits64(efield + (lo - U)) & lowmask64(hi - lo)) << (lo - o);
+    w[h] = x;
+  }
+}
+
+template <typename Bits64>
+__device__ __forceinline__ void classic_line_quarter(Bits64 bits64, uint32_t qq, uint32_t ne, uint32_t n, uint32_t rvs,
+                                                     uint32_t ecode, uint32_t efield, uint64_t (&w)[2]) {
+  const bool ovf = ne > 128 || n * rvs > 384;
+#pragma unroll
+  for (int h = 0; h < 2; h++) {
+    const uint32_t o = qq * 128 + h * 64;
+    uint64_t x = 0;
+    if (ovf) {
+      x = o < 128 ? ~0ull : 0ull;
+    } else if (o < 128) {
+      const uint32_t hi = min(o + 64, ne);
+      if (o < hi) x = bits64(ecode + o) & lowmask64(hi - o);
+    } else {
+      const uint32_t ro = o - 128, hi = min(ro + 64, n * rvs);
+      if (ro < hi) x = bits64(efield + ro) & lowmask64(hi - ro);
+    }
+    w[h] = x;
+  }
+}
+template <typename Bits64>
+__device__ __forceinline__ void line_quarter(Bits64 bits64, const LineGeo& g, uint32_t qq, uint32_t ne, uint32_t n,
+                                             uint32_t rvs, uint32_t ecode, uint32_t efield, uint64_t (&w)[2]) {
+  if (g.dense) dense_line_quarter(bits64, qq, g.U, ne, n, rvs, ecode, efield, w);
+  else classic_line_quarter(bits64, qq, ne, n, rvs, ecode, efield, w);
+}
+
 __device__ __forceinline__ uint64_t lds_bits64(const uint32_t* s_pg, uint32_t bitpos) {
   const uint32_t w = bitpos >> 5, sh = bitpos & 31;
   const uint64_t lo = ((uint64_t)s_pg[w + 1] << 32) | s_pg[w];
   return (lo >> sh) | (sh ? (uint64_t)s_pg[w + 2] << (64 - sh) : 0ull);
 }
 
+template <bool DENSE>
 __global__ __launch_bounds__(ASM_NT) __attribute__((amdgpu_waves_per_eu(8))) void k_assemble(const FilterPlan* __restrict__ plans,
                                                      const uint32_t* __restrict__ pg_filter,
                                                      const uint32_t* __restrict__ idx_cnt,
@@ -2173,7 +2249,8 @@
     return;
   }
   const uint32_t IS = 1u << lis, rvs = P.rvs;
-  const uint32_t lgG = P.lines_asm ? P.lg_line - 1 : 0u, G = 1u << lgG, L = IS >> lgG;
+  const LineGeo lg = line_geo<DENSE>(P.lines_asm ? P.lg_line : 1u, rvs, lis);
+  const uint32_t G = lg.G, L = lg.L;
   const bool cut = P.lines_asm && !(P.lines_flag && nb * (L + 1) > ASM_GT);
   uint32_t cj[2], oj[2], sj[2], sum = 0;
   uint64_t sl[2];
@@ -2304,11 +2381,11 @@
     if (r != threadIdx.x) load_run(r, ev, pv);
     if (cut) {
       const uint32_t gb = j * (L + 1);
-      const uint32_t gp = k0 ? ((pv >> bsh) & bmask) >> lgG : 0u;
+      const uint32_t gp = k0 ? lg.group((pv >> bsh) & bmask) : 0u;
       uint32_t last = ev[0];
 #pragma unroll
       for (uint32_t i = 1; i < ASM_RUN; i++) last = i < len ? ev[i] : last;
-      const uint32_t gl = ((last >> bsh) & bmask) >> lgG;
+      const uint32_t gl = lg.group((last >> bsh) & bmask);
       const uint32_t hi = bsh + lis >= 32 ? 0u : ev[0] & ~((IS << bsh) - 1u);
 #pragma unroll 1
       for (uint32_t g = gp + 1; g <= gl; g++) {
@@ -2443,7 +2520,7 @@
     __syncthreads();
     if (it < nw) {
       const uint32_t ex = ex_all - s_wpre[j];
-      for (uint32_t k = (ex + G) >> lgG; k < L && k * G - 1 < ex + ones; k++)
+      for (uint32_t k = lg.group(ex + G); k < L && k * G - 1 < ex + ones; k++)
         s_gs[j * (L + 1) + k] = (uint16_t)(w * 64 + select64_fast(x, k * G - 1 - ex) + 1);
     }
     __syncthreads();
@@ -2451,29 +2528,16 @@
   }
   DBG_PHASE_K(3, 4);
   const uint32_t nt = nb * L * 4;
+  const float rL = rcp_small(L);
   for (uint32_t u = threadIdx.x; u < nt; u += ASM_NT) {
-    const uint32_t j = u >> (lis - lgG + 2), rest = u & (4 * L - 1), gl = rest >> 2, qq = rest & 3;
+    const uint32_t j = lg.dense ? div_small(u >> 2, rL) : u >> (lis - lg.lgG + 2);
+    const uint32_t gl = lg.dense ? (u >> 2) - j * L : (u & (4 * L - 1)) >> 2, qq = u & 3;
     const uint32_t c = s_c[j];
     const uint32_t ebit = (s_off[j] + 2) * 8, rbit = (s_off[j] + 2 + (c + IS - 1) / 8 + 4) * 8;
     const uint32_t a = s_gs[j * (L + 1) + gl], ne2 = s_gs[j * (L + 1) + gl + 1] - a;
-    const uint32_t n = ne2 - G, E = a - gl * G;
-    const bool ovf = ne2 > 128 || n * rvs > 384;
+    const uint32_t n = ne2 - (lg.dense ? min(G, IS - gl * G) : G), E = a - gl * G;
     uint64_t wv[2];
-#pragma unroll
-    for (int h = 0; h < 2; h++) {
-      const uint32_t o = qq * 128 + h * 64;
-      uint64_t x = 0;
-      if (ovf) {
-        x = o < 128 ? ~0ull : 0ull;
-      } else if (o < 128) {
-        const uint32_t hi = min(o + 64, ne2);
-        if (o < hi) x = lds_bits64(s_pg, ebit + a + o) & lowmask64(hi - o);
-      } else {
-        const uint32_t ro = o - 128, hi = min(ro + 64, n * rvs);
-        if (ro < hi) x = lds_bits64(s_pg, rbit + E * rvs + ro) & lowmask64(hi - ro);
-      }
-      wv[h] = x;
-    }
+    line_quarter([&](uint32_t bit) { return lds_bits64(s_pg, bit); }, lg, qq, ne2, n, rvs, ebit + a, rbit + E * rvs, wv);
     const uint64_t line = (uint64_t)P.line_base + (uint64_t)(b0 + j) * L + gl;
     lines[line * 4 + qq] = make_uint4((uint32_t)wv[0], (uint32_t)(wv[0] >> 32), (uint32_t)wv[1], (uint32_t)(wv[1] >> 32));
   }
@@ -3012,13 +3076,15 @@
   return x;
 }
 
+template <bool DENSE>
 __device__ __forceinline__ void plines_index(const FilterPlan& P, uint32_t g, const uint64_t* __restrict__ slots,
                                              const uint8_t* __restrict__ pages, uint4* __restrict__ lines,
                                              uint8_t* blk, uint32_t* s_a, uint32_t lane, uint32_t lis,
                                              uint32_t page_size) {
   constexpr uint32_t SLICE = MAX_PAGE + 64;
   const uint32_t IS = 1u << lis;
-  const uint32_t lgG = P.lg_line - 1, G = 1u << lgG, L = IS >> lgG;
+  const LineGeo lg = line_geo<DENSE>(P.lg_line, P.rvs, lis);
+  const uint32_t G = lg.G, L = lg.L;
   const uint8_t* pg = blk;
   const uint8_t* gp = pages + (uint64_t)P.page_base * page_size;
   const uint64_t rel_g = slots[g];
@@ -3048,7 +3114,7 @@
       }
       const uint32_t ones = __popcll(x);
       const uint32_t ex = wave_incl_scan(ones) - ones + ones_before;
-      for (uint32_t k = (ex + G) >> lgG; k < L && k * G - 1 < ex + ones; k++)
+      for (uint32_t k = lg.group(ex + G); k < L && k * G - 1 < ex + ones; k++)
         s_a[k] = b0 + select64_fast(x, k * G - 1 - ex) + 1;
       ones_before = __shfl(ex + ones, WAVE - 1, WAVE);
     }
@@ -3064,30 +3130,17 @@
   for (uint32_t u = lane; u < 4 * L; u += WAVE) {
     const uint32_t gl = u >> 2, qq = u & 3;
     const uint32_t a = s_a[gl], ne = s_a[gl + 1] - a;
-    const uint32_t n = ne - G, E = a - gl * G;
-    const bool ovf = ne > 128 || (uint64_t)n * rvs > 384;
+    const uint32_t n = ne - (lg.dense ? min(G, IS - gl * G) : G), E = a - gl * G;
     uint64_t w[2];
-#pragma unroll
-    for (int h = 0; h < 2; h++) {
-      const uint32_t o = qq * 128 + h * 64;
-      uint64_t x = 0;
-      if (ovf) {
-        x = o < 128 ? ~0ull : 0ull;
-      } else if (o < 128) {
-        const uint32_t hi = min(o + 64, ne);
-        if (o < hi) x = bits64_at(pg, ebit + a + o) & lowmask64(hi - o);
-      } else {
-        const uint32_t ro = o - 128, hi = min(ro + 64, n * rvs);
-        if (ro < hi) x = bits64_at(pg, rbit0 + (uint64_t)E * rvs + ro) & lowmask64(hi - ro);
-      }
-      w[h] = x;
-    }
+    line_quarter([&](uint32_t bit) { return bits64_at(pg, bit); }, lg, qq, ne, n, rvs, (uint32_t)ebit + a,
+                 (uint32_t)rbit0 + E * rvs, w);
     lines[(line0 + gl) * 4 + qq] =
         make_uint4((uint32_t)w[0], (uint32_t)(w[0] >> 32), (uint32_t)w[1], (uint32_t)(w[1] >> 32));
   }
 }
 
 
+template <bool DENSE>
 __global__ __launch_bounds__(256) void k_plines(const FilterPlan* __restrict__ plans,
                                                 const uint32_t* __restrict__ idx_filter,
                                                 const uint64_t* __restrict__ slots,
@@ -3106,9 +3159,10 @@
   const FilterPlan& P = plans[f];
   if (P.lg_line == 0 || (outs && outs[f].error) || g - P.idx_base >= P.num_indices) return;
   if (!force && P.lines_asm) return;
-  plines_index(P, g, slots, pages, lines, s_blk[wv], s_dyn + wv * (lmax + 1), lane, lis, page_size);
-}
-
+  plines_index<DENSE>(P, g, slots, pages, lines, s_blk[wv], s_dyn + wv * (lmax + 1), lane, lis, page_size);
+}
+
+template <bool DENSE>
 __global__ __launch_bounds__(256) void k_plines_list(const FilterPlan* __restrict__ plans,
                                                      const uint32_t* __restrict__ pg_filter,
                                                      const uint32_t* __restrict__ page_first,
@@ -3128,7 +3182,7 @@
     const uint32_t* pf = page_first + P.pf_base;
     const uint32_t p = slot - P.page_base, b1 = pf[p + 1];
     for (uint32_t b = pf[p] + wv; b < b1; b += 256 / WAVE)
-      plines_index(P, P.idx_base + b, slots, pages, lines, s_blk[wv], s_dyn + wv * (lmax + 1), lane, lis,
+      plines_index<DENSE>(P, P.idx_base + b, slots, pages, lines, s_blk[wv], s_dyn + wv * (lmax + 1), lane, lis,
                    page_size);
   }
 }
@@ -3234,6 +3288,63 @@
   return true;
 }
 
+struct FieldOnes {
+  uint64_t v[33];
+  constexpr FieldOnes() : v() {
+    for (uint32_t r = 1; r <= 32; r++) {
+      uint64_t L = 0;
+      for (uint32_t k = 0; k < 64; k += r) L |= 1ull << k;
+      v[r] = L;
+    }
+  }
+};
+__constant__ FieldOnes c_field_ones = FieldOnes();
+
+template <typename Dw>
+__device__ __forceinline__ bool line_decode_d(Dw dw, uint32_t U, uint32_t j, uint32_t remainder, uint32_t vs,
+                                              uint32_t rvs, uint64_t& found) {
+  auto cut = [&](uint32_t k) -> uint32_t {
+    return U >= 32 * k + 32 ? dw(k) : (U > 32 * k ? dw(k) & ((1u << (U - 32 * k)) - 1u) : 0u);
+  };
+  uint32_t p1 = 0;
+  if (j) {
+    const uint32_t d0 = cut(0), d1 = cut(1), d2 = cut(2), d3 = cut(3), d4 = cut(4);
+    const uint32_t r = j - 1, c0 = __popc(d0), c1 = c0 + __popc(d1), c2 = c1 + __popc(d2), c3 = c2 + __popc(d3);
+    if (r >= c3 + __popc(d4)) return false;
+    const uint32_t x = r >= c3 ? d4 : (r >= c2 ? d3 : (r >= c1 ? d2 : (r >= c0 ? d1 : d0)));
+    const uint32_t base = r >= c3 ? 128u : (r >= c2 ? 96u : (r >= c1 ? 64u : (r >= c0 ? 32u : 0u)));
+    const uint32_t before = r >= c3 ? c3 : (r >= c2 ? c2 : (r >= c1 ? c1 : (r >= c0 ? c0 : 0u)));
+    p1 = base + select32(x, r - before) + 1;
+  }
+  const uint32_t wi = p1 >> 5, sh = p1 & 31;
+  const uint32_t a0 = dw(wi), a1 = dw(wi + 1), a2 = dw(wi + 2);
+  const uint64_t y = ((uint64_t)__builtin_amdgcn_alignbit(a2, a1, sh) << 32 | __builtin_amdgcn_alignbit(a1, a0, sh)) &
+                     lowmask64(U - p1);
+  if (y == 0) return false;
+  const uint32_t c = (uint32_t)__builtin_ctzll(y);
+  found = 0;
+  if (c == 0) return true;
+  if (rvs == 0) {
+    found = 1;
+    return true;
+  }
+  const uint32_t b = U + (p1 - j) * rvs, nb = c * rvs, fi = b >> 5, off = b & 31;
+  if (b + nb > 512 || nb > 64) return false;
+  const uint32_t w0 = dw(fi), w1 = dw(fi + 1), w2 = dw(fi + 2);
+  const uint64_t W = (uint64_t)__builtin_amdgcn_alignbit(w2, w1, off) << 32 | __builtin_amdgcn_alignbit(w1, w0, off);
+  const uint64_t L = c_field_ones.v[rvs];
+  const uint64_t valid = nb == 64 ? ~0ull : (1ull << nb) - 1;
+  const uint64_t H = L << (rvs - 1);
+  uint64_t Z = H & valid;
+  if (rvs > vs) {
+    const uint64_t M = (L << rvs) - (L << vs), MH = M & ~H;
+    const uint64_t Y = (W ^ ((uint64_t)(remainder << vs) * L)) & M;
+    Z = H & valid & ~(((Y & MH) + MH) | Y);
+  }
+  found = emit_matches(Z, W, rvs, vs);
+  return true;
+}
+
 __device__ __forceinline__ bool line_decode(const v4u (&Q)[4], uint32_t j, uint32_t remainder, uint32_t vs,
                                             uint32_t rvs, uint64_t& found) {
   auto win = [&](uint32_t wi, uint32_t& w0, uint32_t& w1, uint32_t& w2) {
@@ -3305,14 +3416,22 @@
   remainder = fp & (rem >= 32 ? 0xffffffffu : ((1u << rem) - 1));
 }
 
+template <bool DENSE>
 __device__ __forceinline__ bool probe_line(const uint4 P, uint32_t h, const uint4* __restrict__ lines,
-                                           uint32_t fp_size, uint64_t& r) {
+                                           uint32_t fp_size, uint32_t lis, uint64_t& r) {
   const uint32_t vs = P.x & 0xff, rem = (P.x >> 8) & 0xff, rvs = (P.x >> 16) & 0xff, lgl = P.x >> 24;
   r = 0;
   if (P.w) return true;
   if (!lgl) return false;
   uint32_t bucket, remainder;
   split_fp(h, fp_size, rem, bucket, remainder);
+  if (DENSE && line_is_dense(lgl)) {
+    const LineGeo g = line_geo<true>(lgl, rvs, lis);
+    uint32_t line, j;
+    line_locate(g, bucket, lis, line, j);
+    const uint32_t* lw = reinterpret_cast<const uint32_t*>(lines + ((uint64_t)P.y + line) * 4);
+    return line_decode_d([&](uint32_t i) { return lw[i & 15u]; }, g.U, j, remainder, vs, rvs, r);
+  }
   const v4u* lp = reinterpret_cast<const v4u*>(lines + ((uint64_t)P.y + (bucket >> (lgl - 1))) * 4);
   v4u Q[4];
 #pragma unroll
@@ -3332,17 +3451,6 @@
   return probe_stream(bucket & ((1u << lis) - 1), remainder, vs, rvs, pg, hdr, lis);
 }
 
-struct FieldOnes {
-  uint64_t v[33];
-  constexpr FieldOnes() : v() {
-    for (uint32_t r = 1; r <= 32; r++) {
-      uint64_t L = 0;
-      for (uint32_t k = 0; k < 64; k += r) L |= 1ull << k;
-      v[r] = L;
-    }
-  }
-};
-__constant__ FieldOnes c_field_ones = FieldOnes();
 
 __device__ __forceinline__ uint32_t sload32(const void* p) {
 #if __HIP_DEVICE_COMPILE__
@@ -3426,7 +3534,7 @@
   quad_gather_k<3, STRIDE, ROT>(fb, lo, q, q16, sb);
 }
 
-template <int KIND>
+template <int KIND, bool DENSE>
 __device__ __forceinline__ bool probe_fast(const uint4* __restrict__ pplans, const FilterPlan* __restrict__ plans,
                                            const uint8_t* __restrict__ pages, const uint64_t* __restrict__ slots,
                                            const uint4* __restrict__ lines, const void* __restrict__ in0,
@@ -3455,25 +3563,33 @@
     wave_sync_lds();
     h = keys24_hash_lds(sw, lane, seed);
   }
-  const uint32_t lgG = lgl - 1;
+  const LineGeo g = line_geo<DENSE>(lgl, rvs, lis);
   const uint32_t fp = h >> (32 - fp_size);
   const uint32_t bucket = fp >> rem;
   const uint32_t remainder = fp & ((1u << rem) - 1);
   const uint8_t* fb = reinterpret_cast<const uint8_t*>(lines) + ((uint64_t)U.y << 6);
   uint8_t* sb = reinterpret_cast<uint8_t*>(sw);
-  quad_gather<FAST_KSTRIDE, false>(fb, (bucket >> lgG) << 6, lane & 3, sb);
+  uint32_t line, j;
+  line_locate(g, bucket, lis, line, j);
+  quad_gather<FAST_KSTRIDE, false>(fb, line << 6, lane & 3, sb);
   asm volatile("s_waitcnt vmcnt(0)" ::: "memory");
   wave_sync_lds();
   const uint32_t* Lw = reinterpret_cast<const uint32_t*>(sb + (lane & 3) * FAST_KSTRIDE + (lane >> 2) * 64);
-  const uint64_t L = sload64(&c_field_ones.v[rvs]);
   uint64_t r;
-  if (!line_decode_u(Lw, bucket & ((1u << lgG) - 1), remainder, vs, rvs, L, r))
+  bool ok;
+  if (g.dense) {
+    ok = line_decode_d([&](uint32_t i) { return Lw[i]; }, g.U, j, remainder, vs, rvs, r);
+  } else {
+    const uint64_t L = sload64(&c_field_ones.v[rvs]);
+    ok = line_decode_u(Lw, j, remainder, vs, rvs, L, r);
+  }
+  if (!ok)
     r = probe_walk(U, h, fs, plans, pages, slots, fp_size, lis, page_size);
   __builtin_nontemporal_store(r, found + wf + lane);
   return true;
 }
 
-template <int KIND>
+template <int KIND, bool DENSE>
 __global__ __launch_bounds__(probe_nt(KIND)) void k_probe(const uint4* __restrict__ pplans,
                                                     const FilterPlan* __restrict__ plans,
                                                     const uint8_t* __restrict__ pages,
@@ -3503,7 +3619,7 @@
     if (runs) {
       const uint32_t wv = __builtin_amdgcn_readfirstlane(threadIdx.x) / WAVE;
       const uint64_t wfs = (uint64_t)xcd_chunk(blockIdx.x, gridDim.x) * NT + wv * WAVE;
-      if (wfs < n && probe_fast<KIND>(pplans, plans, pages, slots, lines, in0, wave_tab, n, found, fp_size, seed,
+      if (wfs < n && probe_fast<KIND, DENSE>(pplans, plans, pages, slots, lines, in0, wave_tab, n, found, fp_size, seed,
                                       lis, page_size, num_filters, wfs, s_wbuf[wv]))
         return;
     }
@@ -3562,7 +3678,10 @@
       uint32_t bucket, remainder;
       split_fp(h, fp_size, rem, bucket, remainder);
       const uint8_t* fb = reinterpret_cast<const uint8_t*>(lines) + ((uint64_t)U.y << 6);
-      const uint32_t lo = (bucket >> (lgl - 1)) << 6;
+      const LineGeo g = line_geo<DENSE>(lgl, rvs, lis);
+      uint32_t line, j;
+      line_locate(g, bucket, lis, line, j);
+      const uint32_t lo = line << 6;
       v4u* sw;
       if constexpr (WAVE_VAR) sw = reinterpret_cast<v4u*>(s_vk[threadIdx.x / WAVE]);
       else sw = s_wbuf[threadIdx.x / WAVE];
@@ -3578,7 +3697,13 @@
         w2 = dw(6 + wi);
       };
       uint64_t r;
-      if (!line_decode_w(E, win, bucket & ((1u << (lgl - 1)) - 1), remainder, vs, rvs, r))
+      bool ok;
+      if (g.dense)
+        ok = line_decode_d([&](uint32_t d) { d &= 15u; return L32[(((d >> 2) - lane) & 3u) * 4 + (d & 3u)]; }, g.U, j,
+                           remainder, vs, rvs, r);
+      else
+        ok = line_decode_w(E, win, j, remainder, vs, rvs, r);
+      if (!ok)
         r = probe_walk(U, h, fs, plans, pages, slots, fp_size, lis, page_size);
       __builtin_nontemporal_store(r, found + i0);
       return;
@@ -3590,21 +3715,21 @@
   if (uniform) {
     const uint4 U = make_uint4(__builtin_amdgcn_readfirstlane(pp.x), __builtin_amdgcn_readfirstlane(pp.y),
                                __builtin_amdgcn_readfirstlane(pp.z), __builtin_amdgcn_readfirstlane(pp.w));
-    ok = probe_line(U, h, lines, fp_size, r);
+    ok = probe_line<DENSE>(U, h, lines, fp_size, lis, r);
   } else {
-    ok = probe_line(pp, h, lines, fp_size, r);
+    ok = probe_line<DENSE>(pp, h, lines, fp_size, lis, r);
   }
   if (!ok) r = probe_walk(pp, h, fid, plans, pages, slots, fp_size, lis, page_size);
   __builtin_nontemporal_store(r, found + i0);
 }
 
-template <int KIND>
+template <int KIND, bool DENSE>
 __global__ __launch_bounds__(probe_nt(KIND)) void k_probe_floor(const uint4* __restrict__ pplans,
                                                           const uint4* __restrict__ lines,
                                                           const void* __restrict__ in0,
                                                           const uint32_t* __restrict__ wave_tab, uint64_t n,
                                                           uint64_t* __restrict__ found, uint32_t fp_size,
-                                                          uint32_t nf) {
+                                                          uint32_t lis, uint32_t nf) {
   constexpr int NT = probe_nt(KIND);
   __shared__ v4u s_wbuf[NT / WAVE][FAST_WBUF];
   const uint32_t wv = __builtin_amdgcn_readfirstlane(threadIdx.x) / WAVE;
@@ -3621,11 +3746,12 @@
   }
   const uint32_t t = sload32(wave_tab + wf / WAVE);
   const uint32_t fs = t >> 7;
-  uint32_t lgl = 0, rem = 0, base = 0;
+  uint32_t lgl = 0, rem = 0, rvs = 0, base = 0;
   if ((t & 127u) == WAVE && fs < nf && full) {
     const uint32_t x = sload32(&pplans[fs].x);
     lgl = x >> 24;
     rem = (x >> 8) & 0xff;
+    rvs = (x >> 16) & 0xff;
     base = sload32(&pplans[fs].y);
   }
   if (!lgl || rem == 0 || rem >= 32) {
@@ -3645,7 +3771,9 @@
   const uint32_t bucket = (h >> (32 - fp_size)) >> rem;
   const uint8_t* fb = reinterpret_cast<const uint8_t*>(lines) + ((uint64_t)base << 6);
   uint8_t* sb = reinterpret_cast<uint8_t*>(sw);
-  quad_gather<FAST_KSTRIDE, false>(fb, (bucket >> (lgl - 1)) << 6, lane & 3, sb);
+  uint32_t line, j;
+  line_locate(line_geo<DENSE>(lgl, rvs, lis), bucket, lis, line, j);
+  quad_gather<FAST_KSTRIDE, false>(fb, line << 6, lane & 3, sb);
   asm volatile("s_waitcnt vmcnt(0)" ::: "memory");
   wave_sync_lds();
   const v4u E = *reinterpret_cast<const v4u*>(sb + (lane & 3) * FAST_KSTRIDE + (lane >> 2) * 64);
@@ -3656,7 +3784,7 @@
   const uint32_t fp_size = G.fpl & 0xff, lis = (G.fpl >> 8) & 0xff;
   const uint4 P = make_uint4(G.x, 0u, 0u, G.err);
   uint64_t r = 0;
-  if (!probe_line(P, h, G.lines, fp_size, r)) {
+  if (!probe_line<true>(P, h, G.lines, fp_size, lis, r)) {
     const uint32_t vs = G.x & 0xff, rem = (G.x >> 8) & 0xff, rvs = (G.x >> 16) & 0xff;
     uint32_t bucket, remainder;
     split_fp(h, fp_size, rem, bucket, remainder);
@@ -3756,7 +3884,7 @@
 }
 
 template <int KIND>
-__global__ __launch_bounds__(FAN_NT) void k_probe_fanout(const void* __restrict__ in0,
+__global__ __launch_bounds__(FAN_NT) __attribute__((amdgpu_waves_per_eu(5))) void k_probe_fanout(const void* __restrict__ in0,
                                                          const uint64_t* __restrict__ offs, uint32_t key_len,
                                                          uint32_t seed, const ProbeGroup* __restrict__ groups,
                                                          uint32_t ng, const uint32_t* __restrict__ member,
@@ -3816,7 +3944,7 @@
           pf[u] = G->fpl;
           pl[u] = (uint64_t)(uintptr_t)G->lines;
         }
-        st[u] = err ? 0u : ((px[u] >> 24) ? 1u : 2u);
+        st[u] = err ? 0u : ((px[u] >> 24) - 1u < LINE_DENSE - 1u ? 1u : 2u);
       }
 #pragma unroll
       for (int u = 0; u < FAN_U; u++) {
@@ -3847,7 +3975,7 @@
 }
 
 template <int KIND>
-__global__ __launch_bounds__(FAN_NT) void k_probe_fanout_ragged(const void* __restrict__ in0,
+__global__ __launch_bounds__(FAN_NT) __attribute__((amdgpu_waves_per_eu(5))) void k_probe_fanout_ragged(const void* __restrict__ in0,
                                                                 const uint64_t* __restrict__ offs,
                                                                 uint32_t key_len, uint32_t seed,
                                                                 const ProbeGroup* __restrict__ groups, uint32_t ng,
@@ -3910,7 +4038,7 @@
           pf[u] = G->fpl;
           pl[u] = (uint64_t)(uintptr_t)G->lines;
         }
-        st[u] = err ? 0u : ((px[u] >> 24) ? 1u : 2u);
+        st[u] = err ? 0u : ((px[u] >> 24) - 1u < LINE_DENSE - 1u ? 1u : 2u);
       }
 #pragma unroll
       for (int u = 0; u < FAN_U; u++) {
@@ -4352,8 +4480,9 @@
   if (!a.line_lmax || !a.num_page_slots) return 0;
   const size_t lds = 4ull * (256 / WAVE) * (a.line_lmax + 1);
   const uint32_t grid = a.num_page_slots < 1024 ? a.num_page_slots : 1024;
-  hipLaunchKernelGGL(k_plines_list, dim3(grid), dim3(256), lds, (hipStream_t)a.stream, a.plans, a.pg_filter,
-                     a.page_first, a.slots, a.pages, a.pg_noline, a.lines, a.line_lmax, a.lis, a.page_size);
+  hipLaunchKernelGGL(a.lines_dense ? k_plines_list<true> : k_plines_list<false>, dim3(grid), dim3(256), lds,
+                     (hipStream_t)a.stream, a.plans, a.pg_filter, a.page_first, a.slots, a.pages, a.pg_noline, a.lines,
+                     a.line_lmax, a.lis, a.page_size);
   CHECK_LAUNCH();
   return 0;
 }
@@ -4455,9 +4584,9 @@
     CHECK_LAUNCH();
   }
   REC(EV_B_LAYOUT);
-  hipLaunchKernelGGL(k_assemble, dim3(a.num_page_slots), dim3(ASM_NT), 0, (hipStream_t)a.stream, a.plans, a.pg_filter,
-                     a.idx_cnt, a.idx_start, a.sorted32, a.slots, a.page_first, a.outs, a.pages, a.lines,
-                     a.pg_noline, a.lis, a.page_size);
+  hipLaunchKernelGGL(a.lines_dense ? k_assemble<true> : k_assemble<false>, dim3(a.num_page_slots), dim3(ASM_NT), 0,
+                     (hipStream_t)a.stream, a.plans, a.pg_filter, a.idx_cnt, a.idx_start, a.sorted32, a.slots,
+                     a.page_first, a.outs, a.pages, a.lines, a.pg_noline, a.lis, a.page_size);
   CHECK_LAUNCH();
   if (a.plines_needed)
     if (int rc = launch_plines_list(a)) return rc;
@@ -4473,9 +4602,9 @@
   const LaunchArgs& a = *pa;
   if (!a.line_lmax) return 0;
   const size_t lds = 4ull * (256 / WAVE) * (a.line_lmax + 1);
-  hipLaunchKernelGGL(k_plines, dim3((a.num_idx + 3) / 4), dim3(256), lds, (hipStream_t)a.stream, a.plans,
-                     a.idx_filter, a.slots, a.pages, a.outs, a.lines, a.num_idx, a.line_lmax, a.lis,
-                     a.page_size, a.plines_force);
+  hipLaunchKernelGGL(a.lines_dense ? k_plines<true> : k_plines<false>, dim3((a.num_idx + 3) / 4), dim3(256), lds,
+                     (hipStream_t)a.stream, a.plans, a.idx_filter, a.slots, a.pages, a.outs, a.lines, a.num_idx,
+                     a.line_lmax, a.lis, a.page_size, a.plines_force);
   CHECK_LAUNCH();
   return 0;
 }
@@ -4533,12 +4662,10 @@
   if (!a.wave_tab || (kind != IN_KEYS24 && kind != IN_HASH)) return (int)hipErrorInvalidValue;
   const int nt = probe_nt(kind);
   dim3 g((uint32_t)((n + nt - 1) / nt)), b(nt);
-  if (kind == IN_KEYS24)
-    hipLaunchKernelGGL((k_probe_floor<IN_KEYS24>), g, b, 0, (hipStream_t)a.stream, a.pplans, a.lines, in0, a.wave_tab, n,
-                       found, a.fp_size, a.num_filters);
-  else
-    hipLaunchKernelGGL((k_probe_floor<IN_HASH>), g, b, 0, (hipStream_t)a.stream, a.pplans, a.lines, in0, a.wave_tab, n,
-                       found, a.fp_size, a.num_filters);
+  auto kern = kind == IN_KEYS24 ? (a.lines_dense ? k_probe_floor<IN_KEYS24, true> : k_probe_floor<IN_KEYS24, false>)
+                                : (a.lines_dense ? k_probe_floor<IN_HASH, true> : k_probe_floor<IN_HASH, false>);
+  hipLaunchKernelGGL(kern, g, b, 0, (hipStream_t)a.stream, a.pplans, a.lines, in0, a.wave_tab, n, found, a.fp_size,
+                     a.lis, a.num_filters);
   CHECK_LAUNCH();
   return 0;
 }
@@ -4550,7 +4677,10 @@
   const int nt = probe_nt(kind);
   dim3 g((uint32_t)((n + nt - 1) / nt)), b(nt);
   REC(EV_P_START);
-#define PK(K) hipLaunchKernelGGL((k_probe<K>), g, b, 0, (hipStream_t)a.stream, a.pplans, a.plans, a.pages, a.slots, a.lines, in0, offs, key_len, filter_id, a.probe_runs, a.wave_tab, n, found, a.fp_size, a.seed, a.lis, a.page_size, a.num_filters)
+#define PK(K)                                                                                                      \
+  hipLaunchKernelGGL((a.lines_dense ? k_probe<K, true> : k_probe<K, false>), g, b, 0, (hipStream_t)a.stream,        \
+                     a.pplans, a.plans, a.pages, a.slots, a.lines, in0, offs, key_len, filter_id, a.probe_runs,      \
+                     a.wave_tab, n, found, a.fp_size, a.seed, a.lis, a.page_size, a.num_filters)
   switch (kind) {
     KEY_KIND_CASES(PK)
     case IN_PAIR: PK(IN_PAIR); break;
diff --git a/splinterdb_amd/csrc/rf_plan.h b/splinterdb_amd/csrc/rf_plan.h
--- a/splinterdb_amd/csrc/rf_plan.h
+++ b/splinterdb_amd/csrc/rf_plan.h
@@ -79,6 +79,21 @@
   const uint32_t* old_idx_cnt;
   const FilterOut* old_out;
 };
+constexpr uint32_t LINE_DENSE = 0x80;
+constexpr uint32_t LINE_UNARY_MAX = 160;
+__host__ __device__ inline bool line_is_dense(uint32_t lg_line) { return (lg_line & LINE_DENSE) != 0; }
+__host__ __device__ inline uint32_t line_group(uint32_t lg_line) {
+  return line_is_dense(lg_line) ? (lg_line & 0x3fu) + 1u : 1u << (lg_line - 1);
+}
+__host__ __device__ inline uint32_t lines_per_index(uint32_t lis, uint32_t lg_line) {
+  const uint32_t IS = 1u << lis;
+  return line_is_dense(lg_line) ? (IS + line_group(lg_line) - 1) / line_group(lg_line) : IS >> (lg_line - 1);
+}
+__host__ __device__ inline uint32_t line_unary_bits(uint32_t G, uint32_t rvs) {
+  const uint32_t cap = (512u - G) / (1u + rvs), room = LINE_UNARY_MAX - G;
+  return G + (cap < room ? cap : room);
+}
+
 __host__ __device__ inline uint32_t old_error(const FilterPlan& P) { return P.old_out ? P.old_out->error : 0u; }
 
 constexpr uint32_t LAYOUT_SEG_MAX = 4096, LAYOUT_SEG_MIN = 256;
@@ -198,6 +213,7 @@
   uint32_t line_lmax;
   uint32_t plines_needed;
   uint32_t plines_force;
+  uint32_t lines_dense;
   const uint32_t* idx_filter;
   uint32_t num_idx;
   uint32_t* page_first;
diff --git a/splinterdb_amd/engine.py b/splinterdb_amd/engine.py
--- a/splinterdb_amd/engine.py
+++ b/splinterdb_amd/engine.py
@@ -49,6 +49,7 @@
     "rf_amd_found_compact_scratch_bytes", "rf_amd_found_compact",
     "rf_amd_filter_set_probe_var_keys", "rf_amd_batch_probe_var_keys_runs", "rf_amd_filter_lookup_var_keys",
     "rf_amd_diag_fanout_max_blocks", "rf_amd_diag_lookup_paths", "rf_amd_diag_part16_builds",
+    "rf_amd_diag_dense_line_filters",
     "rf_amd_filter_set_probe_keys_ragged", "rf_amd_filter_set_probe_var_keys_ragged",
     "rf_amd_filter_set_probe_hashes_ragged",
     "rf_amd_filter_set_create_cap", "rf_amd_filter_set_capacity", "rf_amd_filter_set_update",
@@ -161,6 +162,8 @@
     L.rf_amd_diag_lookup_ring.argtypes = [vp]
     L.rf_amd_diag_k4_bitmap_builds.argtypes = []
     L.rf_amd_diag_k4_bitmap_builds.restype = u64
+    L.rf_amd_diag_dense_line_filters.argtypes = []
+    L.rf_amd_diag_dense_line_filters.restype = u64
     L.rf_amd_diag_part16_builds.argtypes = []
     L.rf_amd_diag_part16_builds.restype = u64
     L.rf_amd_batch_num_filters.argtypes = [vp]
```

New measurement: 47240 Mkeys/s (median of 6 runs). 2.9% higher.
